# namada-net/masp

Measured on AMD Instinct MI355X. Metric: Spend proofs/sec, higher is better.
Workload: dtype u32; 1 GPU; BASELINE.json configs[3]: batch of 256 distinct Spend proofs per step on one MI355X (throughput mode); proofs_per_gpu=4352, distinct_witnesses_per_gpu=256, ntt_log2=17, batch_cap=256, slots=4, calls_in_flight=4, hw_queues=4, parallelism=proofs sharded over 1 GPU(s), no data-path collective, gather of the proofs

## Files before the change

include/masp_hip.h:

```cpp
#ifndef MASP_HIP_H
#define MASP_HIP_H
#include <stddef.h>
#include <stdint.h>

#ifdef __cplusplus
extern "C" {
#endif

#define MASP_HIP_OK 0
#define MASP_HIP_E_INVALID_ARG 1
#define MASP_HIP_E_PARAMS_FORMAT 2
#define MASP_HIP_E_PARAMS_SHAPE 3
#define MASP_HIP_E_NO_DEVICE 4
#define MASP_HIP_E_HIP 5
#define MASP_HIP_E_UNEXPECTED_IDENTITY 6
#define MASP_HIP_E_NOT_LOADED 7
#define MASP_HIP_E_SCALAR_RANGE 8
#define MASP_HIP_E_POINT_ENCODING 9
#define MASP_HIP_E_CAPACITY 10

#define MASP_HIP_MAX_CIRCUITS 8
#define MASP_HIP_SPEND 0
#define MASP_HIP_OUTPUT 1
#define MASP_HIP_CONVERT 2

typedef struct masp_hip_ctx masp_hip_ctx;

typedef struct {
    uint32_t n_inputs, n_aux, n_constraints;
    const uint32_t* a_rowptr; const uint32_t* a_col; const uint8_t* a_coef;
    const uint32_t* b_rowptr; const uint32_t* b_col; const uint8_t* b_coef;
    const uint32_t* c_rowptr; const uint32_t* c_col; const uint8_t* c_coef;
} masp_hip_r1cs;

typedef struct {
    uint32_t circuit;
    const uint8_t* inputs;
    const uint8_t* aux;
    const uint8_t* a;
    const uint8_t* b;
    const uint8_t* c;
    uint8_t r[32], s[32];
    uint32_t aux_form;
    uint32_t reserved;
} masp_hip_job;
#define MASP_HIP_AUX_CANONICAL 0
#define MASP_HIP_AUX_MONTGOMERY 1

int masp_hip_device_count(void);
int masp_hip_device_pci_bus_id(int device, char* out, size_t cap);

typedef struct {
    uint32_t struct_size;
    int32_t slots;
    int32_t batch_cap;
    int32_t ntt_sub_batch;
    int32_t window_bits_h;
    int32_t window_bits_la;
    int32_t window_bits_b;
    int32_t window_bits_b2_lone;
    int32_t witness_nontrivial_percent;
    int32_t bucket_tree_levels;
    int32_t bucket_tree_sub_batch;
    int32_t bucket_tree_levels_g2;
    int32_t bucket_tree_scratch_mb;
    int32_t bucket_tree_fallback_proofs;
    int32_t lone_proof_graph;
    int32_t hw_queues;
    int32_t window_bits_h_lone;
    int32_t digit_recoding;
    int32_t window_bits_b2;
} masp_hip_options;
void masp_hip_options_default(masp_hip_options* opt);
#define MASP_HIP_MAX_USEFUL_HW_QUEUES 20
int masp_hip_runtime_prepare(int hw_queues, int overwrite);

int masp_hip_ctx_create(int device, masp_hip_ctx** out);
int masp_hip_ctx_create_ex(const int* devices, int n_devices, const masp_hip_options* opt, masp_hip_ctx** out);
int masp_hip_ctx_get_options(const masp_hip_ctx* ctx, masp_hip_options* out);
int masp_hip_ctx_create_multi(const int* devices, int n_devices, masp_hip_ctx** out);
int masp_hip_ctx_set_boolean_block_bits(masp_hip_ctx* ctx, int32_t bits);
int masp_hip_ctx_get_boolean_block_bits(const masp_hip_ctx* ctx, int32_t* out);
int masp_hip_ctx_device_count(const masp_hip_ctx* ctx);
int masp_hip_ctx_device_proofs(const masp_hip_ctx* ctx, uint64_t* counts, int cap);
int masp_hip_ctx_device_status(const masp_hip_ctx* ctx, int32_t* status, int cap, uint64_t* requeued);
int masp_hip_ctx_inject_fault(masp_hip_ctx* ctx, int device, uint32_t nth);
int masp_hip_ctx_stream_concurrency(masp_hip_ctx* ctx, int mains_only, int* n_streams, int* concurrent);
int masp_hip_ctx_lone_graph_launches(const masp_hip_ctx* ctx, uint64_t* out);
void masp_hip_ctx_destroy(masp_hip_ctx* ctx);
const char* masp_hip_strerror(int code);
const char* masp_hip_last_error(const masp_hip_ctx* ctx);

int masp_hip_circuit_load(masp_hip_ctx* ctx, uint32_t slot, const uint8_t* params, size_t params_len, const masp_hip_r1cs* cs);
#define MASP_HIP_CIRCUIT_G1_ENDOMORPHISM 1u
int masp_hip_circuit_flags(const masp_hip_ctx* ctx, uint32_t slot, uint32_t* flags);

int masp_hip_prove(masp_hip_ctx* ctx, uint32_t slot, const uint8_t* inputs, const uint8_t* aux, const uint8_t* a,
                   const uint8_t* b, const uint8_t* c, const uint8_t r[32], const uint8_t s[32], uint8_t proof_out[192]);
int masp_hip_prove_batch(masp_hip_ctx* ctx, size_t n, const masp_hip_job* jobs, uint8_t* proofs_out);

int masp_hip_generate_parameters(masp_hip_ctx* ctx, const masp_hip_r1cs* cs, const uint8_t toxic[160], uint8_t* out, size_t cap,
                                 size_t* out_len);
size_t masp_hip_parameters_max_size(const masp_hip_r1cs* cs);

int masp_hip_msm_g1(masp_hip_ctx* ctx, const uint8_t* bases, const uint8_t* scalars, size_t n, uint8_t out[96]);
int masp_hip_msm_g2(masp_hip_ctx* ctx, const uint8_t* bases, const uint8_t* scalars, size_t n, uint8_t out[192]);
int masp_hip_msm_g1_multi(masp_hip_ctx* ctx, const uint8_t* bases, size_t n, const uint8_t* scalars, size_t np, int window_bits,
                          uint8_t* out);
int masp_hip_msm_g2_multi(masp_hip_ctx* ctx, const uint8_t* bases, size_t n, const uint8_t* scalars, size_t np, int window_bits,
                          uint8_t* out);
int masp_hip_msm_g1_multi_ex(masp_hip_ctx* ctx, const uint8_t* bases, size_t n, const uint8_t* scalars, size_t np, int window_bits,
                             int block_bits, size_t sub_lo, size_t sub_hi, uint8_t* out, uint32_t* bucket0_entries);
int masp_hip_msm_g2_multi_ex(masp_hip_ctx* ctx, const uint8_t* bases, size_t n, const uint8_t* scalars, size_t np, int window_bits,
                             int block_bits, size_t sub_lo, size_t sub_hi, uint8_t* out, uint32_t* bucket0_entries);
int masp_hip_quotient_h(masp_hip_ctx* ctx, const uint8_t* a, const uint8_t* b, const uint8_t* c, size_t nrows,
                        uint32_t logm, uint8_t* h_out);
int masp_hip_ntt(masp_hip_ctx* ctx, uint8_t* data, uint32_t logm, int inverse);

typedef struct masp_hip_vk masp_hip_vk;
int masp_hip_vk_prepare(masp_hip_ctx* ctx, const uint8_t* params, size_t params_len, masp_hip_vk** out);
void masp_hip_vk_free(masp_hip_vk* vk);
int masp_hip_verify_batch(masp_hip_ctx* ctx, masp_hip_vk* vk, size_t n, const uint8_t* proofs, const uint8_t* public_inputs,
                          uint32_t n_public, const uint8_t* z, int* all_valid);

int masp_hip_jubjub_msm(masp_hip_ctx* ctx, size_t n, const uint8_t* points, const uint8_t* scalars, uint8_t out32[32], int64_t* bad_index);
int masp_hip_redjubjub_verify_batch(masp_hip_ctx* ctx, size_t n, const uint8_t* vks, const uint8_t* sigs, const uint8_t* sighashes,
                                    const uint8_t* kinds, const uint8_t* z, int* all_valid);

int masp_hip_sapling_trial_decrypt(masp_hip_ctx* ctx, size_t n_ivk, const uint8_t* ivks, size_t n_out, const uint8_t* epks,
                                   const uint8_t* enc_ciphertexts, uint8_t* epk_status, size_t hit_capacity, uint32_t* hit_output,
                                   uint32_t* hit_ivk, uint8_t* hit_keys, size_t* n_hits);
int masp_hip_note_scan_configure(masp_hip_ctx* ctx, int signed_digits, int inversion);
int masp_hip_note_scan_last_timing(masp_hip_ctx* ctx, double ms[2]);

int masp_hip_sapling_compact_trial_decrypt(masp_hip_ctx* ctx, size_t n_ivk, const uint8_t* ivks, size_t n_out, const uint8_t* epks,
                                           const uint8_t* cmus, const uint8_t* enc_compact, int lead_byte, uint8_t* epk_status,
                                           size_t hit_capacity, uint32_t* hit_output, uint32_t* hit_ivk, uint8_t* hit_plaintexts,
                                           uint8_t* hit_pk_d, size_t* n_hits, size_t* n_candidates);
int masp_hip_note_scan_compact_last_timing(masp_hip_ctx* ctx, double ms[3]);

int masp_hip_sapling_output_recovery_scan(masp_hip_ctx* ctx, size_t n_ovk, const uint8_t* ovks, size_t n_out, const uint8_t* cvs,
                                          const uint8_t* epks, const uint8_t* cmus, const uint8_t* out_ciphertexts, size_t hit_capacity,
                                          uint32_t* hit_output, uint32_t* hit_ovk, uint8_t* hit_ocks, size_t* n_hits);
int masp_hip_out_recovery_last_timing(masp_hip_ctx* ctx, double ms[2]);

int masp_hip_merkle_tree_complete(masp_hip_ctx* ctx, unsigned height0, size_t n, const uint8_t* row, uint8_t* nodes_out, size_t nodes_capacity,
                                  size_t* n_nodes, uint8_t root32[32], size_t n_paths, const uint64_t* positions, uint8_t* paths_out,
                                  int64_t* bad_index);
int masp_hip_merkle_last_timing(masp_hip_ctx* ctx, double ms[3]);
int masp_hip_merkle_tree_append(masp_hip_ctx* ctx, uint64_t start, const uint8_t frontier[32 * 32], size_t n, const uint8_t* row,
                                uint8_t* nodes_out, size_t nodes_capacity, size_t* n_nodes, int64_t* bad_index);

int masp_hip_batch_upload(masp_hip_ctx* ctx, size_t n, const masp_hip_job* jobs);
int masp_hip_batch_prove_resident(masp_hip_ctx* ctx, int handle, uint8_t* proofs_out, float* elapsed_ms);
int masp_hip_batch_prove_resident_steps(masp_hip_ctx* ctx, int handle, size_t steps, const uint8_t* rs, uint8_t* proofs_out,
                                        float* elapsed_ms);
int masp_hip_batch_free(masp_hip_ctx* ctx, int handle);
int masp_hip_bench_msm(masp_hip_ctx* ctx, int handle, size_t job, int which, int iters, float* avg_ms, uint32_t* n_bases);

int masp_hip_profile_enable(masp_hip_ctx* ctx, int on);
int masp_hip_profile_read(masp_hip_ctx* ctx, double* total_ms, uint64_t* launches, uint64_t* alg_bytes);
int masp_hip_profile_read_split(masp_hip_ctx* ctx, double ms[8]);
int masp_hip_profile_read_lone(masp_hip_ctx* ctx, double ms[12]);
void* masp_hip_host_alloc(masp_hip_ctx* ctx, size_t bytes);
void masp_hip_host_free(masp_hip_ctx* ctx, void* ptr);
int masp_hip_sync(masp_hip_ctx* ctx);

#ifdef __cplusplus
}
#endif

#if defined(__cplusplus) && __cplusplus >= 201103L
#define MASP_HIP_STATIC_ASSERT(c, m) static_assert(c, m)
#elif defined(__STDC_VERSION__) && __STDC_VERSION__ >= 201112L
#define MASP_HIP_STATIC_ASSERT(c, m) _Static_assert(c, m)
#else
#define MASP_HIP_SA_CAT2(a, b) a##b
#define MASP_HIP_SA_CAT(a, b) MASP_HIP_SA_CAT2(a, b)
#define MASP_HIP_STATIC_ASSERT(c, m) typedef char MASP_HIP_SA_CAT(masp_hip_static_assert_, __LINE__)[(c) ? 1 : -1]
#endif
#if defined(__LP64__) || defined(_LP64)
MASP_HIP_STATIC_ASSERT(sizeof(masp_hip_job) == 120, "masp_hip_job: 4 + 4 pad + 5 pointers + r[32] + s[32] + aux_form + reserved");
MASP_HIP_STATIC_ASSERT(offsetof(masp_hip_job, inputs) == 8 && offsetof(masp_hip_job, c) == 40, "masp_hip_job pointers");
MASP_HIP_STATIC_ASSERT(offsetof(masp_hip_job, r) == 48 && offsetof(masp_hip_job, s) == 80, "masp_hip_job r | s");
MASP_HIP_STATIC_ASSERT(offsetof(masp_hip_job, aux_form) == 112 && offsetof(masp_hip_job, reserved) == 116, "masp_hip_job tail");
MASP_HIP_STATIC_ASSERT(sizeof(masp_hip_r1cs) == 88 && offsetof(masp_hip_r1cs, a_rowptr) == 16 && offsetof(masp_hip_r1cs, c_coef) == 80,
                       "masp_hip_r1cs: three counts + 4 pad + nine pointers");
MASP_HIP_STATIC_ASSERT(sizeof(masp_hip_options) == 76 && offsetof(masp_hip_options, window_bits_b2) == 72,
                       "masp_hip_options: struct_size + 18 int32 fields (appended-only: struct_size versions it)");
MASP_HIP_STATIC_ASSERT(offsetof(masp_hip_options, hw_queues) == 60 && offsetof(masp_hip_options, digit_recoding) == 68, "masp_hip_options tail");
#endif
#endif
```

masp_amd/csrc/device/ntt.hpp:

```cpp
#pragma once
#include <hip/hip_runtime.h>

#include "field.hpp"
#include "fr_io.hpp"
#include "ntt_geom.h"

namespace masp {


__device__ __forceinline__ uint32_t bitrev(uint32_t k, uint32_t logm) { return __brev(k) >> (32 - logm); }

__global__ void k_fr_powers(Fr* __restrict__ table, uint32_t n, Fr base, Fr scale, int plain) {
    uint32_t k = blockIdx.x * blockDim.x + threadIdx.x;
    if (k >= n) return;
    uint32_t e[1] = {k};
    Fr r = fe_mul(fe_pow(base, e, 1), scale);
    if (plain) r = fe_from_mont(r);
    fr_store(table + k, r);
}

#define NTT_P (blockIdx.y)

__global__ void k_ntt_load_bitrev(const Fr* __restrict__ x, size_t x_stride, uint32_t nrows, Fr* __restrict__ y, uint32_t logm) {
    uint32_t k = blockIdx.x * blockDim.x + threadIdx.x;
    if (k >= (1u << logm)) return;
    x += NTT_P * x_stride;
    y += (size_t)NTT_P << logm;
    Fr v = fe_zero<FrCfg>();
    if (k < nrows) v = fe_to_mont(fr_load(x + k));
    fr_store(y + bitrev(k, logm), v);
}
__global__ void k_ntt_copy_bitrev(const Fr* __restrict__ x, size_t x_stride, uint32_t nrows, Fr* __restrict__ y, uint32_t logm) {
    uint32_t k = blockIdx.x * blockDim.x + threadIdx.x;
    if (k >= (1u << logm)) return;
    x += NTT_P * x_stride;
    y += (size_t)NTT_P << logm;
    Fr v = fe_zero<FrCfg>();
    if (k < nrows) v = fr_load(x + k);
    fr_store(y + bitrev(k, logm), v);
}
__global__ void k_ntt_scale_bitrev(const Fr* __restrict__ x, const Fr* __restrict__ scale, Fr* __restrict__ y, uint32_t logm) {
    uint32_t k = blockIdx.x * blockDim.x + threadIdx.x;
    if (k >= (1u << logm)) return;
    x += (size_t)NTT_P << logm;
    y += (size_t)NTT_P << logm;
    fr_store(y + bitrev(k, logm), fe_mul(fr_load(x + k), fr_load(scale + k)));
}
__global__ void k_ntt_ab_bitrev(const Fr* __restrict__ a, const Fr* __restrict__ b, Fr* __restrict__ y, uint32_t logm) {
    uint32_t k = blockIdx.x * blockDim.x + threadIdx.x;
    if (k >= (1u << logm)) return;
    a += (size_t)NTT_P << logm;
    b += (size_t)NTT_P << logm;
    y += (size_t)NTT_P << logm;
    fr_store(y + bitrev(k, logm), fe_mul(fr_load(a + k), fr_load(b + k)));
}
__global__ void k_fr_scale_sub(const Fr* __restrict__ x, const Fr* __restrict__ scale, const Fr* __restrict__ c, Fr cscale, Fr* __restrict__ y,
                               uint32_t n, size_t y_stride) {
    uint32_t k = blockIdx.x * blockDim.x + threadIdx.x;
    if (k >= n) return;
    x += (size_t)NTT_P * n;
    c += (size_t)NTT_P * n;
    y += (size_t)NTT_P * y_stride;
    fr_store(y + k, fe_sub(fe_mul(fr_load(x + k), fr_load(scale + k)), fe_mul(fr_load(c + k), cscale)));
}
__global__ void k_fr_scale(const Fr* __restrict__ x, const Fr* __restrict__ scale, Fr* __restrict__ y, uint32_t n, size_t y_stride) {
    uint32_t k = blockIdx.x * blockDim.x + threadIdx.x;
    if (k >= n) return;
    x += (size_t)NTT_P * n;
    y += (size_t)NTT_P * y_stride;
    fr_store(y + k, fe_mul(fr_load(x + k), fr_load(scale + k)));
}
__global__ void k_fr_from_mont(const Fr* __restrict__ x, Fr* __restrict__ y, uint32_t n) {
    uint32_t k = blockIdx.x * blockDim.x + threadIdx.x;
    if (k >= n) return;
    fr_store(y + k, fe_from_mont(fr_load(x + k)));
}

__global__ void __launch_bounds__(256) k_ntt_pass(Fr* __restrict__ data, const Fr* __restrict__ tw, uint32_t logm, uint32_t s0,
                                                  uint32_t nst) {
    __shared__ uint4 tile[2 << NTT_LT];
    const uint32_t lt = nst + (NTT_LT - nst < logm - nst ? NTT_LT - nst : logm - nst);
    const uint32_t cols_log = lt - nst;
    const uint32_t cols = 1u << cols_log;
    const uint32_t tsize = 1u << lt;
    const uint32_t col0 = blockIdx.x << cols_log;
    const uint32_t lomask = (1u << s0) - 1u;
    data += (size_t)NTT_P << logm;
    for (uint32_t L = threadIdx.x; L < tsize; L += blockDim.x) {
        uint32_t h = L >> cols_log, col = col0 + (L & (cols - 1));
        uint32_t idx = ((col >> s0) << (s0 + nst)) | (h << s0) | (col & lomask);
        const uint4* q = reinterpret_cast<const uint4*>(data + idx);
        tile[L] = q[0];
        tile[tsize + L] = q[1];
    }
    __syncthreads();
    auto ld = [&](uint32_t L) {
        Fr r;
        uint4 a0 = tile[L], a1 = tile[tsize + L];
        r.v[0] = a0.x; r.v[1] = a0.y; r.v[2] = a0.z; r.v[3] = a0.w; r.v[4] = a1.x; r.v[5] = a1.y; r.v[6] = a1.z; r.v[7] = a1.w;
        return r;
    };
    auto st = [&](uint32_t L, const Fr& x) {
        tile[L] = make_uint4(x.v[0], x.v[1], x.v[2], x.v[3]);
        tile[tsize + L] = make_uint4(x.v[4], x.v[5], x.v[6], x.v[7]);
    };
    uint32_t q = 0;
    for (; q + 1 < nst; q += 2) {
        const uint32_t s = s0 + q;
        for (uint32_t gidx = threadIdx.x; gidx < (tsize >> 2); gidx += blockDim.x) {
            const uint32_t cl = gidx & (cols - 1), r = gidx >> cols_log;
            const uint32_t hj = r & ((1u << q) - 1u), hg = r >> q;
            const uint32_t h00 = (hg << (q + 2)) | hj;
            const uint32_t L0 = (h00 << cols_log) | cl, d = cols << q;
            const uint32_t lo = (col0 + cl) & lomask;
            const uint32_t j1 = (hj << s0) | lo;
            const uint32_t j2a = j1, j2b = ((hj | (1u << q)) << s0) | lo;
            Fr x0 = ld(L0), x1 = ld(L0 + d), x2 = ld(L0 + 2 * d), x3 = ld(L0 + 3 * d);
            if (s == 0) {
                const Fr y0 = fe_add(x0, x1), y1 = fe_sub(x0, x1), y2 = fe_add(x2, x3), y3 = fe_sub(x2, x3);
                st(L0, fe_add(y0, y2));
                st(L0 + 2 * d, fe_sub(y0, y2));
                const Fr t = fe_mul(y3, fr_load(tw + ((size_t)1 << (logm - 2))));
                st(L0 + d, fe_add(y1, t));
                st(L0 + 3 * d, fe_sub(y1, t));
                continue;
            }
            const Fr w1 = fr_load(tw + ((size_t)j1 << (logm - s - 1)));
            const Fr w2a = fr_load(tw + ((size_t)j2a << (logm - s - 2)));
            const Fr w2b = fr_load(tw + ((size_t)j2b << (logm - s - 2)));
            Fr t = fe_mul(x1, w1);
            Fr y0 = fe_add(x0, t), y1 = fe_sub(x0, t);
            t = fe_mul(x3, w1);
            Fr y2 = fe_add(x2, t), y3 = fe_sub(x2, t);
            t = fe_mul(y2, w2a);
            st(L0, fe_add(y0, t));
            st(L0 + 2 * d, fe_sub(y0, t));
            t = fe_mul(y3, w2b);
            st(L0 + d, fe_add(y1, t));
            st(L0 + 3 * d, fe_sub(y1, t));
        }
        __syncthreads();
    }
    for (; q < nst; ++q) {
        const uint32_t s = s0 + q;
        for (uint32_t b = threadIdx.x; b < (tsize >> 1); b += blockDim.x) {
            uint32_t cl = b & (cols - 1), hb = b >> cols_log;
            uint32_t hj = hb & ((1u << q) - 1u), hg = hb >> q;
            uint32_t L0 = (((hg << (q + 1)) | hj) << cols_log) | cl;
            uint32_t L1 = L0 + (cols << q);
            uint32_t col = col0 + cl;
            uint32_t jglob = (hj << s0) | (col & lomask);
            Fr w = fr_load(tw + ((size_t)jglob << (logm - s - 1)));
            Fr u = ld(L0), v = fe_mul(ld(L1), w);
            st(L0, fe_add(u, v));
            st(L1, fe_sub(u, v));
        }
        __syncthreads();
    }
    for (uint32_t L = threadIdx.x; L < tsize; L += blockDim.x) {
        uint32_t h = L >> cols_log, col = col0 + (L & (cols - 1));
        uint32_t idx = ((col >> s0) << (s0 + nst)) | (h << s0) | (col & lomask);
        uint4* q = reinterpret_cast<uint4*>(data + idx);
        q[0] = tile[L];
        q[1] = tile[tsize + L];
    }
}

}
```

masp_amd/csrc/device/r1cs.hpp:

```cpp
#pragma once
#include <hip/hip_runtime.h>

#include "../launch.h"
#include "fr_io.hpp"

namespace masp {

__global__ void k_fr_to_mont(const Fr* __restrict__ x, size_t x_stride, Fr* __restrict__ y, uint32_t n, int* __restrict__ range_err) {
    uint32_t k = blockIdx.x * blockDim.x + threadIdx.x;
    if (k >= n) return;
    x += blockIdx.y * x_stride;
    y += (size_t)blockIdx.y * n;
    Fr v = fr_load(x + k);
    if (fe_canonical_ge_mod(v)) atomicOr(range_err, 1);
    fr_store(y + k, fe_to_mont(v));
}
__global__ void k_fr_split_forms(Fr* __restrict__ x, size_t x_stride, Fr* __restrict__ y, uint32_t n, uint32_t mont_from, int* __restrict__ range_err) {
    uint32_t k = blockIdx.x * blockDim.x + threadIdx.x;
    if (k >= n) return;
    x += blockIdx.y * x_stride;
    y += (size_t)blockIdx.y * n;
    Fr v = fr_load(x + k);
    if (fe_canonical_ge_mod(v)) atomicOr(range_err, 1);
    if (k < mont_from) {
        fr_store(y + k, fe_to_mont(v));
    } else {
        fr_store(y + k, v);
        fr_store(x + k, fe_from_mont(v));
    }
}

__global__ void k_r1cs_eval(R1csMatrices M, const Fr* __restrict__ w, uint32_t n_vars, uint32_t n_constraints, uint32_t n_inputs) {
    const int which = blockIdx.z;
    const uint32_t v = blockIdx.x * blockDim.x + threadIdx.x, nl = M.n_long[which];
    const uint32_t* __restrict__ rowptr = M.rowptr[which];
    const uint32_t* __restrict__ order = M.order[which];
    const uint32_t* __restrict__ col = M.col[which];
    const Fr* __restrict__ coef = M.coef[which];
    Fr* __restrict__ out = M.out[which];
    w += (size_t)blockIdx.y * n_vars;
    out += (size_t)blockIdx.y * (n_constraints + n_inputs);
    if (v < nl * 64u) {
        const uint32_t row = order[v >> 6], lane = v & 63u;
        const uint32_t lo = rowptr[row], hi = rowptr[row + 1];
        Fr acc = fe_zero<FrCfg>();
        for (uint32_t t = lo + lane; t < hi; t += 64) acc = fe_add(acc, fe_mul(fr_load(coef + t), fr_load(w + col[t])));
        for (int d = 32; d >= 1; d >>= 1) {
            Fr other;
#pragma unroll
            for (int i = 0; i < 8; ++i) other.v[i] = (uint32_t)__shfl_down((int)acc.v[i], d, 64);
            acc = fe_add(acc, other);
        }
        if (lane == 0) fr_store(out + row, acc);
        return;
    }
    uint32_t row = v - nl * 64u + nl;
    if (row >= n_constraints + n_inputs) return;
    Fr acc = fe_zero<FrCfg>();
    if (row < n_constraints) {
        row = order[row];
        uint32_t lo = rowptr[row], hi = rowptr[row + 1];
        for (uint32_t t = lo; t < hi; ++t) acc = fe_add(acc, fe_mul(fr_load(coef + t), fr_load(w + col[t])));
    } else if (which == 0) {
        acc = fr_load(w + (row - n_constraints));
    }
    fr_store(out + row, acc);
}

__global__ void k_gather_scalars(const Fr* __restrict__ src, size_t src_stride, const uint32_t* __restrict__ idx, uint32_t n,
                                 Fr* __restrict__ dst) {
    uint32_t k = blockIdx.x * blockDim.x + threadIdx.x;
    if (k >= n) return;
    src += blockIdx.y * src_stride;
    dst += (size_t)blockIdx.y * n;
    fr_store(dst + k, fr_load(src + idx[k]));
}

}
```

masp_amd/csrc/device/setup.hpp:

```cpp
#pragma once
#include <hip/hip_runtime.h>

#include "curve.hpp"
#include "fr_io.hpp"
#include "io.hpp"

namespace masp {

__global__ void k_setup_lagrange(Fr* __restrict__ lag, uint32_t nrows, Fr omega, Fr tau, Fr z_over_m) {
    uint32_t k = blockIdx.x * blockDim.x + threadIdx.x;
    if (k >= nrows) return;
    uint32_t e[1] = {k};
    Fr wk = fe_pow(omega, e, 1);
    Fr den = fe_inv(fe_sub(tau, wk));
    fr_store(lag + k, fe_mul(fe_mul(z_over_m, wk), den));
}
__global__ void k_setup_qap(const uint32_t* __restrict__ colptr, const uint32_t* __restrict__ rowidx, const Fr* __restrict__ coef,
                            const Fr* __restrict__ lag, uint32_t nv, uint32_t n_inputs, uint32_t n_constraints, int is_a,
                            Fr* __restrict__ out) {
    uint32_t v = blockIdx.x * blockDim.x + threadIdx.x;
    if (v >= nv) return;
    Fr acc = fe_zero<FrCfg>();
    for (uint32_t t = colptr[v]; t < colptr[v + 1]; ++t) acc = fe_add(acc, fe_mul(fr_load(coef + t), fr_load(lag + rowidx[t])));
    if (is_a && v < n_inputs) acc = fe_add(acc, fr_load(lag + n_constraints + v));
    fr_store(out + v, acc);
}
__global__ void k_setup_lc(const Fr* __restrict__ at, const Fr* __restrict__ bt, const Fr* __restrict__ ct, uint32_t n, Fr alpha, Fr beta,
                           Fr scale, Fr* __restrict__ out) {
    uint32_t v = blockIdx.x * blockDim.x + threadIdx.x;
    if (v >= n) return;
    Fr x = fe_add(fe_add(fe_mul(beta, fr_load(at + v)), fe_mul(alpha, fr_load(bt + v))), fr_load(ct + v));
    fr_store(out + v, fe_mul(x, scale));
}
__global__ void k_setup_nonzero(const Fr* __restrict__ x, uint32_t n, uint8_t* __restrict__ flags) {
    uint32_t v = blockIdx.x * blockDim.x + threadIdx.x;
    if (v >= n) return;
    flags[v] = fe_is_zero(fr_load(x + v)) ? 0 : 1;
}

template <class O>
__global__ void k_setup_fixed_table(Affine<O> gen, Affine<O>* __restrict__ tab) {
    uint32_t w = blockIdx.x * blockDim.x + threadIdx.x;
    if (w >= 32) return;
    Xyzz<O> base = xyzz_from_affine(gen);
    for (uint32_t k = 0; k < 8 * w; ++k) base = xyzz_dbl(base);
    Affine<O> b = xyzz_to_affine(base);
    Xyzz<O> cur = xyzz_from_affine(b);
    for (uint32_t d = 1; d <= 255; ++d) {
        tab[w * 255 + d - 1] = xyzz_to_affine(cur);
        xyzz_madd_nc(cur, b, false);
    }
}
template <class O, int BYTES>
__global__ void __launch_bounds__(64) k_setup_fixed_mul(const Affine<O>* __restrict__ tab, const Fr* __restrict__ scalars, uint32_t n, int mont,
                                                        uint8_t* __restrict__ out) {
    uint32_t i = blockIdx.x * blockDim.x + threadIdx.x;
    if (i >= n) return;
    Fr k = fr_load(scalars + i);
    if (mont) k = fe_from_mont(k);
    Xyzz<O> acc = xyzz_inf<O>();
    for (int w = 0; w < 32; ++w) {
        uint32_t d = (k.v[w >> 2] >> (8 * (w & 3))) & 0xffu;
        if (d) xyzz_madd_nc(acc, tab[w * 255 + d - 1], false);
    }
    Affine<O> p = xyzz_to_affine(acc);
    if constexpr (BYTES == 96)
        g1_write_uncompressed(p, out + (size_t)i * 96);
    else
        g2_write_uncompressed(p, out + (size_t)i * 192);
}
__global__ void k_setup_gather(const Fr* __restrict__ src, const uint32_t* __restrict__ idx, uint32_t n, Fr* __restrict__ dst) {
    uint32_t k = blockIdx.x * blockDim.x + threadIdx.x;
    if (k >= n) return;
    fr_store(dst + k, fr_load(src + idx[k]));
}
__global__ void k_setup_h_scalars(Fr tau, Fr c, uint32_t n, Fr* __restrict__ out) {
    uint32_t i = blockIdx.x * blockDim.x + threadIdx.x;
    if (i >= n) return;
    uint32_t e[1] = {i};
    fr_store(out + i, fe_mul(fe_pow(tau, e, 1), c));
}

}
```

masp_amd/csrc/internal.h:

```cpp
#pragma once
#include <hip/hip_runtime.h>

#include <algorithm>
#include <array>
#include <condition_variable>
#include <cstring>
#include <deque>
#include <map>
#include <memory>
#include <mutex>
#include <shared_mutex>
#include <string>
#include <thread>
#include <vector>

#include "chunk_pipeline.h"
#include "device/io.hpp"
#include "device/ntt_geom.h"
#include "launch.h"
#include "msm_host.h"
#include <atomic>
#include "util.h"

#ifndef MASP_SUBSET_BITS
#define MASP_SUBSET_BITS 2
#endif
static_assert(MASP_SUBSET_BITS == 0 || MASP_SUBSET_BITS == 2 || MASP_SUBSET_BITS == 3, "subset blocks are 4 or 8 bases wide");


namespace masp {

template <class T>
struct DevBuf {
    T* p = nullptr;
    size_t cap = 0;
    ~DevBuf() { release(); }
    void release() {
        if (p) dev_free(p);
        p = nullptr;
        cap = 0;
    }
    int reserve(size_t n) {
        if (n <= cap) return MASP_HIP_OK;
        release();
        HIP_TRY(dev_malloc(&p, sizeof(T) * std::max<size_t>(n, 1)));
        cap = n;
        return MASP_HIP_OK;
    }
    int upload(const T* h, size_t n, hipStream_t s) {
        int rc = reserve(n);
        if (rc) return rc;
        if (n) HIP_TRY(hipMemcpyAsync(p, h, sizeof(T) * n, hipMemcpyHostToDevice, s));
        return MASP_HIP_OK;
    }
};

static inline Fr fr_from_u64_mont(uint64_t x) {
    Fr v = fe_zero<FrCfg>();
    v.v[0] = (uint32_t)x;
    v.v[1] = (uint32_t)(x >> 32);
    return fe_to_mont(v);
}
static inline Fr fr_const(const uint32_t* limbs) {
    Fr v;
    for (int i = 0; i < 8; ++i) v.v[i] = limbs[i];
    return v;
}

struct NttDomain {
    uint32_t logm = 0;
    size_t m = 0;
    DevBuf<Fr> tw_fwd, tw_inv, coset_scale, h_scale;
    Fr c_scale;
    int init(uint32_t logm_, hipStream_t s) {
        logm = logm_;
        m = (size_t)1 << logm;
        Fr omega = fr_const(FrCfg::ROOT_OF_UNITY);
        for (uint32_t i = logm; i < 32; ++i) omega = fe_sqr(omega);
        Fr omega_inv = fe_inv(omega);
        Fr minv = fe_inv(fr_from_u64_mont(m));
        Fr g = fr_const(FrCfg::GEN), ginv = fr_const(FrCfg::GEN_INV);
        uint32_t e[2] = {(uint32_t)m, (uint32_t)((uint64_t)m >> 32)};
        const Fr zinv = fe_inv(fe_sub(fe_pow(g, e, 2), fe_one<FrCfg>()));
        const Fr mzinv = fe_mul(minv, zinv);
        c_scale = fe_from_mont(mzinv);
        Fr one = fe_one<FrCfg>();
        size_t half = std::max<size_t>(m / 2, 1);
        int rc;
        if ((rc = tw_fwd.reserve(half)) || (rc = tw_inv.reserve(half)) || (rc = coset_scale.reserve(m)) || (rc = h_scale.reserve(m))) return rc;
        launch_fr_powers(s, tw_fwd.p, (uint32_t)half, omega, one, 0);
        launch_fr_powers(s, tw_inv.p, (uint32_t)half, omega_inv, one, 0);
        launch_fr_powers(s, coset_scale.p, (uint32_t)m, g, minv, 0);
        launch_fr_powers(s, h_scale.p, (uint32_t)m, ginv, mzinv, 1);
        HIP_TRY(hipStreamSynchronize(s));
        return MASP_HIP_OK;
    }
    void passes(hipStream_t s, Fr* data, const Fr* tw, uint32_t np = 1) const {
        for (uint32_t s0 = 0; s0 < logm;) {
            uint32_t nst = std::min<uint32_t>(NTT_LT, logm - s0);
            launch_ntt_pass(s, data, tw, logm, s0, nst, np);
            s0 += nst;
        }
    }
};

struct Circuit {
    uint32_t n_inputs = 0, n_aux = 0, n_constraints = 0, nrows = 0, logm = 0;
    size_t m = 0;
    DevBuf<uint32_t> rowptr[3], col[3];
    DevBuf<uint32_t> row_order[3];
    uint32_t n_long_rows[3] = {0, 0, 0};
    DevBuf<Fr> coef[3];
    DevBuf<uint32_t> a_var, b_var;
    uint32_t na = 0, nbq = 0;
    DevBuf<VkDevice> vk;
    DevBuf<G1Xyzz> fb1;
    DevBuf<G2Xyzz> fb2;
    BasesG1 h, l, a, b1;
    BasesG1 hl;
    BasesG2 b2;
    BasesG2 b2_lone;
    bool g1_endo = false;
    NttDomain* dom = nullptr;
};

struct Slot {
    hipStream_t stream = nullptr;
    hipEvent_t done = nullptr;
    MsmWorkspace<FpOps> ws1;
    MsmWorkspace<Fp2Ops> ws2;
    static constexpr int N_AUX = 4;
    hipStream_t aux[N_AUX] = {nullptr, nullptr, nullptr, nullptr};
    hipEvent_t ev_fork = nullptr, ev_sort_b = nullptr, ev_fixed = nullptr, ev_join[N_AUX] = {nullptr, nullptr, nullptr, nullptr};
    hipEvent_t ev_uploaded = nullptr;
    MsmWorkspace<FpOps> ws_l, ws_a, ws_b;
    DevBuf<Fr> w, inp, abc, wm, ev[3], x0, x1, h, hl, sa, sb;
    DevBuf<G1Xyzz> res1, asm1;
    DevBuf<G2Xyzz> res2, asm2;
    DevBuf<uint32_t> rs;
    DevBuf<uint8_t> proof;
    DevBuf<int> flags;
    MsmProfile prof;
    bool profiling = false;
    static constexpr int N_LONE_MARKS = 12;
    hipEvent_t ev_lone[N_LONE_MARKS] = {};
    bool lone_marked = false;
    void lone_mark(hipStream_t st, int id) {
        if (!profiling) return;
        if (!ev_lone[id] && hipEventCreate(&ev_lone[id]) != hipSuccess) return;
        (void)hipEventRecord(ev_lone[id], st);
        if (id == N_LONE_MARKS - 1) lone_marked = true;
    }
    uint32_t ntt_sub = 8;
    uint8_t* h_stage = nullptr;
    size_t h_stage_cap = 0;
    uint8_t* h_proof = nullptr;
    size_t h_proof_cap = 0;
    int* h_flags = nullptr;
    struct LoneGraph {
        const void *circuit, *w, *abc, *rs, *proof;
        size_t w_stride;
        uint32_t np;
        bool mont;
        int runs;
        bool dead;
        hipGraphExec_t exec;
    };
    std::vector<LoneGraph> graphs;
    uint64_t graph_epoch = 0;
    bool lone_graph = false;
    std::atomic<uint64_t> graph_launches{0};
    void drop_graphs() {
        for (auto& g : graphs)
            if (g.exec) hipGraphExecDestroy(g.exec);
        graphs.clear();
    }
    ~Slot() {
        drop_graphs();
        if (done) hipEventDestroy(done);
        for (hipEvent_t e : ev_join)
            if (e) hipEventDestroy(e);
        for (hipEvent_t e : ev_lone)
            if (e) hipEventDestroy(e);
        if (ev_fork) hipEventDestroy(ev_fork);
        if (ev_uploaded) hipEventDestroy(ev_uploaded);
        if (ev_sort_b) hipEventDestroy(ev_sort_b);
        if (ev_fixed) hipEventDestroy(ev_fixed);
        if (h_stage) hipHostFree(h_stage);
        if (h_proof) hipHostFree(h_proof);
        if (h_flags) hipHostFree(h_flags);
    }
    void configure(const masp_hip_options& o) {
        ntt_sub = (uint32_t)o.ntt_sub_batch;
        ws1.tree_levels = o.bucket_tree_levels;
        ws2.tree_levels = o.bucket_tree_levels_g2;
        ws1.tree_levels_shared = o.bucket_tree_levels_g2;
        ws1.tree_sub = ws2.tree_sub = (uint32_t)o.bucket_tree_sub_batch;
        ws2.tree.arena = &ws1.tree.own;
        ws1.tree.own.limit = (size_t)o.bucket_tree_scratch_mb << 20;
        lone_graph = o.lone_proof_graph > 0;
    }
    int init(const std::array<hipStream_t, 5>& streams) {
        stream = streams[0];
        for (int i = 0; i < N_AUX; ++i) aux[i] = streams[1 + i];
        HIP_TRY(hipEventCreateWithFlags(&done, hipEventDisableTiming));
        HIP_TRY(hipEventCreateWithFlags(&ev_fork, hipEventDisableTiming));
        HIP_TRY(hipEventCreateWithFlags(&ev_uploaded, hipEventDisableTiming));
        HIP_TRY(hipEventCreateWithFlags(&ev_sort_b, hipEventDisableTiming));
        HIP_TRY(hipEventCreateWithFlags(&ev_fixed, hipEventDisableTiming));
        for (hipEvent_t& e : ev_join) HIP_TRY(hipEventCreateWithFlags(&e, hipEventDisableTiming));
        HIP_TRY(hipHostMalloc(&h_flags, sizeof(int)));
        int rc;
        if ((rc = flags.reserve(1))) return rc;
        return reserve_batch(1);
    }
    int reserve_batch(size_t np) {
        int rc;
        if ((rc = res1.reserve(4 * np)) || (rc = res2.reserve(np)) || (rc = asm1.reserve(6 * np)) || (rc = asm2.reserve(np)) || (rc = rs.reserve(16 * np)) || (rc = proof.reserve(192 * np))) return rc;
        if (np > h_proof_cap) {
            if (h_proof) hipHostFree(h_proof);
            h_proof = nullptr;
            HIP_TRY(hipHostMalloc(&h_proof, 192 * np));
            h_proof_cap = np;
        }
        return MASP_HIP_OK;
    }
    int stage_reserve(size_t bytes) {
        if (bytes <= h_stage_cap) return MASP_HIP_OK;
        if (h_stage) hipHostFree(h_stage);
        h_stage = nullptr;
        HIP_TRY(hipHostMalloc(&h_stage, bytes));
        h_stage_cap = bytes;
        return MASP_HIP_OK;
    }
};

struct ResidentBatch {
    size_t n = 0;
    std::vector<uint32_t> circuit;
    std::vector<size_t> order;
    std::vector<size_t> w_off;
    DevBuf<Fr> w;
    DevBuf<uint32_t> rs;
};

struct StreamTable {
    hipStream_t main = nullptr;
    std::vector<std::array<hipStream_t, 5>> slot;
    hipStream_t vk[2] = {nullptr, nullptr};
    std::vector<hipStream_t> distinct() const {
        std::vector<hipStream_t> out;
        auto add = [&](hipStream_t s) {
            if (s && std::find(out.begin(), out.end(), s) == out.end()) out.push_back(s);
        };
        add(main);
        for (const auto& row : slot)
            for (hipStream_t s : row) add(s);
        for (hipStream_t s : vk) add(s);
        return out;
    }
    ~StreamTable() {
        for (hipStream_t s : distinct()) (void)hipStreamDestroy(s);
    }
};

}

using masp::Circuit;
using masp::DevBuf;
using masp::Fr;
using masp::G1Affine;
using masp::G1Xyzz;
using masp::G2Affine;
using masp::G2Xyzz;
using masp::NttDomain;
using masp::ResidentBatch;
using masp::Slot;

struct masp_hip_ctx {
    static constexpr size_t MAX_SLOTS = 64;
    int device = 0;
    std::vector<masp_hip_ctx*> children;
    masp_hip_options opt{};
    int boolean_block_bits = MASP_SUBSET_BITS;
    int n_slots = 4;
    size_t batch_cap = 256;
    std::shared_mutex mu;
    mutable std::mutex slot_mu;
    std::condition_variable slot_cv;
    std::vector<char> slot_busy;
    std::string err;
    masp::StreamTable streams;
    std::unique_ptr<Circuit> circ[MASP_HIP_MAX_CIRCUITS];
    std::map<uint32_t, std::unique_ptr<NttDomain>> domains;
    std::vector<std::unique_ptr<Slot>> slots;
    std::vector<std::unique_ptr<ResidentBatch>> batches;
    bool profiling = false;
    std::atomic<uint64_t> proofs_done{0};
    std::unique_ptr<std::atomic<int>[]> dev_status;
    std::atomic<uint64_t> requeued{0};
    std::atomic<uint32_t> fault_countdown{0};
    std::atomic<unsigned> vk_next{0};
    int main_streams_concurrent = 0;
    std::mutex upload_mu;
    hipEvent_t upload_tail = nullptr;
    std::atomic<uint64_t> block_tree_fallbacks{0};
    std::atomic<uint32_t> block_tree_sub{0xffffffffu};
    DevBuf<Fr> tmp_scalars;
    DevBuf<uint8_t> tmp_out;
    DevBuf<G1Xyzz> tmp_g1;
    DevBuf<G2Xyzz> tmp_g2;
    DevBuf<G1Affine> fb_g1;
    DevBuf<G2Affine> fb_g2;
    std::mutex jj_mu;
    DevBuf<uint8_t> jj_points, jj_scalars, jj_partial;
    DevBuf<int> jj_status;
    DevBuf<uint32_t> jj_out;
    struct NoteScanSet {
        DevBuf<uint8_t> epk, raw, ct, pts, status, hit_keys;
        DevBuf<uint32_t> count, hit_idx;
    };
    std::mutex ns_mu;
    NoteScanSet ns[2];
    DevBuf<uint32_t> ns_digits;
    std::atomic<int> ns_signed_digits{1}, ns_inversion{0};
    double ns_last_ms[2] = {0, 0};
    struct NoteScanCompactSet {
        DevBuf<uint8_t> cmu, enc, cand, state, hit_idx, hit_data;
        DevBuf<uint32_t> count, list;
    };
    NoteScanCompactSet nsc[2];
    DevBuf<uint8_t> nsc_ivks;
    DevBuf<uint8_t> nsc_table;
    double nsc_last_ms[3] = {0, 0, 0};
    struct OutRecoverySet {
        DevBuf<uint8_t> cv, cmu, epk, cout, cols, hit_ocks;
        DevBuf<uint32_t> count, hit_idx;
    };
    OutRecoverySet orc[2];
    DevBuf<uint32_t> orc_ovks;
    double orc_last_ms[2] = {0, 0};
    DevBuf<uint32_t> mt_nodes, mt_bad, mt_paths, mt_empties;
    DevBuf<uint64_t> mt_pos;
    double mt_last_ms[3] = {0, 0, 0};
};

namespace masp {

static inline int fail(masp_hip_ctx* ctx, int rc) {
    if (rc == MASP_HIP_E_HIP) {
        std::lock_guard<std::mutex> g(ctx->slot_mu);
        ctx->err = last_hip_error();
    }
    return rc;
}

#define FIRST_DEVICE(ctx) ((ctx) && !(ctx)->children.empty() ? (ctx)->children[0] : (ctx))

static inline int get_domain(masp_hip_ctx* ctx, uint32_t logm, NttDomain** out) {
    auto it = ctx->domains.find(logm);
    if (it == ctx->domains.end()) {
        std::unique_ptr<NttDomain> d(new NttDomain);
        int rc = d->init(logm, ctx->streams.main);
        if (rc) return rc;
        it = ctx->domains.emplace(logm, std::move(d)).first;
    }
    *out = it->second.get();
    return MASP_HIP_OK;
}

constexpr size_t NS_MAX_IVKS = 4096;
constexpr size_t NS_MAX_OUTPUTS = (size_t)1 << 26;
int ns_recode_ivks(std::vector<uint32_t>& digits, size_t n_ivk, const uint8_t* ivks, bool signed_digits);
void launch_ns_decode(hipStream_t s, const uint8_t* epks, uint32_t n, uint8_t* status, uint8_t* pts);

static inline uint32_t log2_ceil(uint32_t n) {
    uint32_t k = 0;
    while ((1ull << k) < n) ++k;
    return k;
}

}
```

masp_amd/csrc/k_ntt.hip:

```cpp
#include <algorithm>
#include "device/ntt.hpp"
#include "device/r1cs.hpp"
#include "launch.h"
#include "util.h"

namespace masp {

void launch_fr_powers(hipStream_t s, Fr* table, uint32_t n, const Fr& base, const Fr& scale, int plain) {
    MASP_LAUNCH(k_fr_powers, dim3((n + 255) / 256), dim3(256), 0, s, table, n, base, scale, plain);
}
void launch_ntt_pass(hipStream_t s, Fr* data, const Fr* tw, uint32_t logm, uint32_t s0, uint32_t nst, uint32_t np) {
    const uint32_t lt = (uint32_t)NTT_LT < logm ? (uint32_t)NTT_LT : logm;
    MASP_LAUNCH(k_ntt_pass, dim3(1u << (logm - lt), np), dim3(256), 0, s, data, tw, logm, s0, nst);
}
void launch_ntt_load_bitrev(hipStream_t s, const Fr* x, size_t x_stride, uint32_t nrows, Fr* y, uint32_t logm, uint32_t np) {
    MASP_LAUNCH(k_ntt_load_bitrev, dim3(((1u << logm) + 255) / 256, np), dim3(256), 0, s, x, x_stride, nrows, y, logm);
}
void launch_ntt_copy_bitrev(hipStream_t s, const Fr* x, size_t x_stride, uint32_t nrows, Fr* y, uint32_t logm, uint32_t np) {
    MASP_LAUNCH(k_ntt_copy_bitrev, dim3(((1u << logm) + 255) / 256, np), dim3(256), 0, s, x, x_stride, nrows, y, logm);
}
void launch_ntt_scale_bitrev(hipStream_t s, const Fr* x, const Fr* scale, Fr* y, uint32_t logm, uint32_t np) {
    MASP_LAUNCH(k_ntt_scale_bitrev, dim3(((1u << logm) + 255) / 256, np), dim3(256), 0, s, x, scale, y, logm);
}
void launch_ntt_ab_bitrev(hipStream_t s, const Fr* a, const Fr* b, Fr* y, uint32_t logm, uint32_t np) {
    MASP_LAUNCH(k_ntt_ab_bitrev, dim3(((1u << logm) + 255) / 256, np), dim3(256), 0, s, a, b, y, logm);
}
void launch_fr_scale_sub(hipStream_t s, const Fr* x, const Fr* scale, const Fr* c, const Fr& cscale, Fr* y, uint32_t n, uint32_t np, size_t y_stride) {
    MASP_LAUNCH(k_fr_scale_sub, dim3((n + 255) / 256, np), dim3(256), 0, s, x, scale, c, cscale, y, n, y_stride ? y_stride : (size_t)n);
}
void launch_fr_scale(hipStream_t s, const Fr* x, const Fr* scale, Fr* y, uint32_t n, uint32_t np, size_t y_stride) {
    MASP_LAUNCH(k_fr_scale, dim3((n + 255) / 256, np), dim3(256), 0, s, x, scale, y, n, y_stride ? y_stride : (size_t)n);
}
void launch_fr_from_mont(hipStream_t s, const Fr* x, Fr* y, uint32_t n) {
    MASP_LAUNCH(k_fr_from_mont, dim3((n + 255) / 256), dim3(256), 0, s, x, y, n);
}
void launch_fr_to_mont(hipStream_t s, const Fr* x, size_t x_stride, Fr* y, uint32_t n, uint32_t np, int* range_err) {
    MASP_LAUNCH(k_fr_to_mont, dim3((n + 255) / 256, np), dim3(256), 0, s, x, x_stride, y, n, range_err);
}
void launch_fr_split_forms(hipStream_t s, Fr* x, size_t x_stride, Fr* y, uint32_t n, uint32_t mont_from, uint32_t np, int* range_err) {
    MASP_LAUNCH(k_fr_split_forms, dim3((n + 255) / 256, np), dim3(256), 0, s, x, x_stride, y, n, mont_from, range_err);
}
void launch_r1cs_eval(hipStream_t s, const R1csMatrices& M, const Fr* w, uint32_t n_vars, uint32_t n_constraints, uint32_t n_inputs, uint32_t np) {
    const uint32_t nl = std::max(M.n_long[0], std::max(M.n_long[1], M.n_long[2])), lanes = n_constraints + n_inputs + nl * 63u;
    MASP_LAUNCH(k_r1cs_eval, dim3((lanes + 127) / 128, np, 3), dim3(128), 0, s, M, w, n_vars, n_constraints, n_inputs);
}
void launch_gather_scalars(hipStream_t s, const Fr* src, size_t src_stride, const uint32_t* idx, uint32_t n, Fr* dst, uint32_t np) {
    MASP_LAUNCH(k_gather_scalars, dim3((n + 255) / 256, np), dim3(256), 0, s, src, src_stride, idx, n, dst);
}

}
```

masp_amd/csrc/k_setup.hip:

```cpp
#include "device/setup.hpp"
#include "internal.h"

using namespace masp;

extern "C" {

size_t masp_hip_parameters_max_size(const masp_hip_r1cs* cs) {
    if (!cs) return 0;
    size_t nv = (size_t)cs->n_inputs + cs->n_aux;
    size_t m = (size_t)1 << log2_ceil(cs->n_constraints + cs->n_inputs);
    return 864 + 6 * 4 + 96 * ((size_t)cs->n_inputs + (m - 1) + cs->n_aux + 2 * nv) + 192 * nv;
}

int masp_hip_generate_parameters(masp_hip_ctx* ctx, const masp_hip_r1cs* cs, const uint8_t toxic[160], uint8_t* out, size_t cap,
                                 size_t* out_len) {
    if (!ctx || !cs || !toxic || !out_len || cs->n_inputs == 0) return MASP_HIP_E_INVALID_ARG;
    const ApiLaunchScope api_scope;
    ctx = FIRST_DEVICE(ctx);
    std::unique_lock<std::shared_mutex> lock(ctx->mu);
    hipSetDevice(ctx->device);
    hipStream_t s = ctx->streams.main;
    Fr tw[5];
    for (int i = 0; i < 5; ++i) {
        Fr v = fe_load_le<FrCfg>(toxic + 32 * i);
        if (fe_canonical_ge_mod(v)) return MASP_HIP_E_SCALAR_RANGE;
        tw[i] = fe_to_mont(v);
    }
    const Fr tau = tw[0], alpha = tw[1], beta = tw[2], gamma = tw[3], delta = tw[4];
    if (fe_is_zero(gamma) || fe_is_zero(delta)) return MASP_HIP_E_UNEXPECTED_IDENTITY;
    const uint32_t n_in = cs->n_inputs, n_aux = cs->n_aux, nc = cs->n_constraints, nv = n_in + n_aux;
    const uint32_t nrows = nc + n_in, logm = log2_ceil(nrows);
    const size_t m = (size_t)1 << logm;
    Fr omega = fr_const(FrCfg::ROOT_OF_UNITY);
    for (uint32_t i = logm; i < 32; ++i) omega = fe_sqr(omega);
    uint32_t em[2] = {(uint32_t)m, (uint32_t)((uint64_t)m >> 32)};
    Fr z = fe_sub(fe_pow(tau, em, 2), fe_one<FrCfg>());
    Fr z_over_m = fe_mul(z, fe_inv(fr_from_u64_mont(m)));
    Fr dinv = fe_inv(delta), ginv = fe_inv(gamma);
    int rc;
    if (!ctx->fb_g1.p) {
        if ((rc = ctx->fb_g1.reserve(32 * 255)) || (rc = ctx->fb_g2.reserve(32 * 255))) return fail(ctx, rc);
        G1Affine g1;
        G2Affine g2;
        for (int i = 0; i < 12; ++i) {
            g1.x.v[i] = FpCfg::G1_X[i];
            g1.y.v[i] = FpCfg::G1_Y[i];
            g2.x.c0.v[i] = FpCfg::G2_X0[i];
            g2.x.c1.v[i] = FpCfg::G2_X1[i];
            g2.y.c0.v[i] = FpCfg::G2_Y0[i];
            g2.y.c1.v[i] = FpCfg::G2_Y1[i];
        }
        MASP_LAUNCH((k_setup_fixed_table<FpOps>), dim3(1), dim3(64), 0, s, g1, ctx->fb_g1.p);
        MASP_LAUNCH((k_setup_fixed_table<Fp2Ops>), dim3(1), dim3(64), 0, s, g2, ctx->fb_g2.p);
    }
    DevBuf<Fr> lag, qt[3];
    if ((rc = lag.reserve(nrows))) return fail(ctx, rc);
    MASP_LAUNCH(k_setup_lagrange, dim3((nrows + 127) / 128), dim3(128), 0, s, lag.p, nrows, omega, tau, z_over_m);
    const uint32_t* rp[3] = {cs->a_rowptr, cs->b_rowptr, cs->c_rowptr};
    const uint32_t* cl[3] = {cs->a_col, cs->b_col, cs->c_col};
    const uint8_t* cf[3] = {cs->a_coef, cs->b_coef, cs->c_coef};
    DevBuf<int> d_flag;
    if ((rc = d_flag.reserve(1))) return fail(ctx, rc);
    hipMemsetAsync(d_flag.p, 0, sizeof(int), s);
    for (int mi = 0; mi < 3; ++mi) {
        const uint32_t nnz = rp[mi][nc];
        std::vector<uint32_t> colptr(nv + 1, 0), rowidx(nnz);
        std::vector<Fr> coefs(nnz);
        for (uint32_t t = 0; t < nnz; ++t) {
            if (cl[mi][t] >= nv) return MASP_HIP_E_INVALID_ARG;
            ++colptr[cl[mi][t] + 1];
        }
        for (uint32_t v = 0; v < nv; ++v) colptr[v + 1] += colptr[v];
        std::vector<uint32_t> fill(colptr.begin(), colptr.end() - 1);
        for (uint32_t row = 0; row < nc; ++row)
            for (uint32_t t = rp[mi][row]; t < rp[mi][row + 1]; ++t) {
                uint32_t pos = fill[cl[mi][t]]++;
                rowidx[pos] = row;
                memcpy(&coefs[pos], cf[mi] + 32 * (size_t)t, 32);
            }
        DevBuf<uint32_t> d_colptr, d_rowidx;
        DevBuf<Fr> d_raw, d_coef;
        if ((rc = d_colptr.upload(colptr.data(), nv + 1, s)) || (rc = d_rowidx.upload(rowidx.data(), nnz, s)) ||
            (rc = d_raw.upload(coefs.data(), nnz, s)) || (rc = d_coef.reserve(nnz)) || (rc = qt[mi].reserve(nv)))
            return fail(ctx, rc);
        if (nnz) launch_fr_to_mont(s, d_raw.p, (size_t)0, d_coef.p, nnz, 1, d_flag.p);
        MASP_LAUNCH(k_setup_qap, dim3((nv + 127) / 128), dim3(128), 0, s, d_colptr.p, d_rowidx.p, d_coef.p, lag.p, nv, n_in, nc,
                           mi == 0 ? 1 : 0, qt[mi].p);
        if (hipStreamSynchronize(s) != hipSuccess) {
            last_hip_error() = std::string("qap evaluation failed: ") + hipGetErrorString(hipGetLastError());
            return fail(ctx, MASP_HIP_E_HIP);
        }
    }
    DevBuf<uint8_t> d_nz;
    if ((rc = d_nz.reserve(2 * (size_t)nv))) return fail(ctx, rc);
    MASP_LAUNCH(k_setup_nonzero, dim3((nv + 255) / 256), dim3(256), 0, s, qt[0].p, nv, d_nz.p);
    MASP_LAUNCH(k_setup_nonzero, dim3((nv + 255) / 256), dim3(256), 0, s, qt[1].p, nv, d_nz.p + nv);
    std::vector<uint8_t> nz(2 * (size_t)nv);
    int hflag = 0;
    if (hipMemcpyAsync(nz.data(), d_nz.p, nz.size(), hipMemcpyDeviceToHost, s) != hipSuccess ||
        hipMemcpyAsync(&hflag, d_flag.p, sizeof(int), hipMemcpyDeviceToHost, s) != hipSuccess || hipStreamSynchronize(s) != hipSuccess)
        return fail(ctx, MASP_HIP_E_HIP);
    if (hflag) return MASP_HIP_E_SCALAR_RANGE;
    std::vector<uint32_t> a_list, b_list;
    for (uint32_t v = 0; v < nv; ++v) {
        if (nz[v]) a_list.push_back(v);
        if (nz[nv + v]) b_list.push_back(v);
    }
    const size_t n_h = m - 1, n_a = a_list.size(), n_b = b_list.size();
    const size_t o_ic = 3, o_h = o_ic + n_in, o_l = o_h + n_h, o_a = o_l + n_aux, o_b = o_a + n_a, n_g1 = o_b + n_b;
    const size_t n_g2 = 3 + n_b;
    const size_t total = 864 + 6 * 4 + 96 * (n_g1 - 3) + 192 * n_b;
    *out_len = total;
    if (!out || cap < total) return MASP_HIP_E_INVALID_ARG;
    DevBuf<Fr> k1, k2, lc;
    DevBuf<uint32_t> d_alist, d_blist;
    if ((rc = k1.reserve(n_g1)) || (rc = k2.reserve(n_g2)) || (rc = lc.reserve(nv)) || (rc = d_alist.upload(a_list.data(), n_a, s)) ||
        (rc = d_blist.upload(b_list.data(), n_b, s)))
        return fail(ctx, rc);
    Fr head1[3] = {alpha, beta, delta}, head2[3] = {beta, gamma, delta};
    if (hipMemcpyAsync(k1.p, head1, sizeof(head1), hipMemcpyHostToDevice, s) != hipSuccess ||
        hipMemcpyAsync(k2.p, head2, sizeof(head2), hipMemcpyHostToDevice, s) != hipSuccess)
        return fail(ctx, MASP_HIP_E_HIP);
    MASP_LAUNCH(k_setup_lc, dim3((n_in + 255) / 256), dim3(256), 0, s, qt[0].p, qt[1].p, qt[2].p, n_in, alpha, beta, ginv, k1.p + o_ic);
    if (n_aux)
        MASP_LAUNCH(k_setup_lc, dim3((n_aux + 255) / 256), dim3(256), 0, s, qt[0].p + n_in, qt[1].p + n_in, qt[2].p + n_in, n_aux, alpha,
                           beta, dinv, k1.p + o_l);
    MASP_LAUNCH(k_setup_h_scalars, dim3((n_h + 255) / 256), dim3(256), 0, s, tau, fe_mul(z, dinv), (uint32_t)n_h, k1.p + o_h);
    if (n_a) MASP_LAUNCH(k_setup_gather, dim3((n_a + 255) / 256), dim3(256), 0, s, qt[0].p, d_alist.p, (uint32_t)n_a, k1.p + o_a);
    if (n_b) {
        MASP_LAUNCH(k_setup_gather, dim3((n_b + 255) / 256), dim3(256), 0, s, qt[1].p, d_blist.p, (uint32_t)n_b, k1.p + o_b);
        MASP_LAUNCH(k_setup_gather, dim3((n_b + 255) / 256), dim3(256), 0, s, qt[1].p, d_blist.p, (uint32_t)n_b, k2.p + 3);
    }
    DevBuf<uint8_t> p1, p2;
    if ((rc = p1.reserve(96 * n_g1)) || (rc = p2.reserve(192 * n_g2))) return fail(ctx, rc);
    MASP_LAUNCH((k_setup_fixed_mul<FpOps, 96>), dim3((n_g1 + 63) / 64), dim3(64), 0, s, ctx->fb_g1.p, k1.p, (uint32_t)n_g1, 1, p1.p);
    MASP_LAUNCH((k_setup_fixed_mul<Fp2Ops, 192>), dim3((n_g2 + 63) / 64), dim3(64), 0, s, ctx->fb_g2.p, k2.p, (uint32_t)n_g2, 1, p2.p);
    std::vector<uint8_t> h1(96 * n_g1), h2(192 * n_g2);
    if (hipMemcpyAsync(h1.data(), p1.p, h1.size(), hipMemcpyDeviceToHost, s) != hipSuccess ||
        hipMemcpyAsync(h2.data(), p2.p, h2.size(), hipMemcpyDeviceToHost, s) != hipSuccess || hipStreamSynchronize(s) != hipSuccess) {
        last_hip_error() = std::string("parameter generation failed: ") + hipGetErrorString(hipGetLastError());
        return fail(ctx, MASP_HIP_E_HIP);
    }
    uint8_t* w = out;
    auto put = [&](const uint8_t* src, size_t n) {
        memcpy(w, src, n);
        w += n;
    };
    auto put_len = [&](size_t n) {
        uint8_t b[4] = {(uint8_t)(n >> 24), (uint8_t)(n >> 16), (uint8_t)(n >> 8), (uint8_t)n};
        put(b, 4);
    };
    put(&h1[0], 96);
    put(&h1[96], 96);
    put(&h2[0], 192);
    put(&h2[192], 192);
    put(&h1[192], 96);
    put(&h2[384], 192);
    put_len(n_in);
    put(&h1[96 * o_ic], 96 * (size_t)n_in);
    put_len(n_h);
    put(&h1[96 * o_h], 96 * n_h);
    put_len(n_aux);
    put(&h1[96 * o_l], 96 * (size_t)n_aux);
    put_len(n_a);
    put(&h1[96 * o_a], 96 * n_a);
    put_len(n_b);
    put(&h1[96 * o_b], 96 * n_b);
    put_len(n_b);
    put(&h2[192 * 3], 192 * n_b);
    if (launch_status() != MASP_HIP_OK) return fail(ctx, MASP_HIP_E_HIP);
    return (size_t)(w - out) == total ? MASP_HIP_OK : MASP_HIP_E_INVALID_ARG;
}

}
```

masp_amd/csrc/launch.h:

```cpp
#pragma once
#include <hip/hip_runtime.h>

#include "device/curve.hpp"

namespace masp {

void launch_fr_powers(hipStream_t s, Fr* table, uint32_t n, const Fr& base, const Fr& scale, int plain);
void launch_ntt_pass(hipStream_t s, Fr* data, const Fr* tw, uint32_t logm, uint32_t s0, uint32_t nst, uint32_t np);
void launch_ntt_load_bitrev(hipStream_t s, const Fr* x, size_t x_stride, uint32_t nrows, Fr* y, uint32_t logm, uint32_t np);
void launch_ntt_copy_bitrev(hipStream_t s, const Fr* x, size_t x_stride, uint32_t nrows, Fr* y, uint32_t logm, uint32_t np);
void launch_ntt_scale_bitrev(hipStream_t s, const Fr* x, const Fr* scale, Fr* y, uint32_t logm, uint32_t np);
void launch_ntt_ab_bitrev(hipStream_t s, const Fr* a, const Fr* b, Fr* y, uint32_t logm, uint32_t np);
void launch_fr_scale_sub(hipStream_t s, const Fr* x, const Fr* scale, const Fr* c, const Fr& cscale, Fr* y, uint32_t n, uint32_t np, size_t y_stride = 0);
void launch_fr_scale(hipStream_t s, const Fr* x, const Fr* scale, Fr* y, uint32_t n, uint32_t np, size_t y_stride = 0);
void launch_fr_from_mont(hipStream_t s, const Fr* x, Fr* y, uint32_t n);
void launch_fr_to_mont(hipStream_t s, const Fr* x, size_t x_stride, Fr* y, uint32_t n, uint32_t np, int* range_err);
void launch_fr_split_forms(hipStream_t s, Fr* x, size_t x_stride, Fr* y, uint32_t n, uint32_t mont_from, uint32_t np, int* range_err);
struct R1csMatrices {
    const uint32_t* rowptr[3];
    const uint32_t* order[3];
    const uint32_t* col[3];
    const Fr* coef[3];
    Fr* out[3];
    uint32_t n_long[3];
};
static constexpr uint32_t R1CS_LONG_ROW = 64;
void launch_r1cs_eval(hipStream_t s, const R1csMatrices& M, const Fr* w, uint32_t n_vars, uint32_t n_constraints, uint32_t n_inputs, uint32_t np);
void launch_gather_scalars(hipStream_t s, const Fr* src, size_t src_stride, const uint32_t* idx, uint32_t n, Fr* dst, uint32_t np);

void launch_groth16_fixed_g1(hipStream_t s, const G1Xyzz* fb1, const uint32_t* rs, size_t rs_stride, G1Xyzz* part, uint32_t np);
void launch_groth16_fixed_g2(hipStream_t s, const G2Xyzz* fb2, const uint32_t* rs, size_t rs_stride, G2Xyzz* part2, uint32_t np);
void launch_groth16_var_mul(hipStream_t s, int which, const G1Xyzz* msm_g1, const uint32_t* rs, size_t rs_stride, G1Xyzz* part, uint32_t np, bool endo);
void launch_g1_subgroup_flag(hipStream_t s, const void* pts, size_t stride_bytes, uint32_t n, int* flag);
void launch_groth16_finish_b(hipStream_t s, const VkDevice* vk, const G2Xyzz* part2, const G2Xyzz* msm_g2, uint8_t* proof, uint32_t np);
void launch_groth16_finish_ac(hipStream_t s, const VkDevice* vk, const G1Xyzz* part, const G1Xyzz* msm_g1, uint8_t* proof, uint32_t np);
void launch_groth16_finish_ac_early(hipStream_t s, const VkDevice* vk, G1Xyzz* part, const G1Xyzz* msm_g1, uint8_t* proof, uint32_t np);
void launch_groth16_finish_c_late(hipStream_t s, const G1Xyzz* part, const G1Xyzz* msm_g1, uint8_t* proof, uint32_t np);
void launch_g1_export(hipStream_t s, const G1Xyzz* p, uint8_t* out);
void launch_g2_export(hipStream_t s, const G2Xyzz* p, uint8_t* out);
void launch_g1_import_one(hipStream_t s, const uint8_t* raw, G1Affine* out, int* status);
void launch_g2_import_one(hipStream_t s, const uint8_t* raw, G2Affine* out, int* status);
void launch_fixed_table_g1(hipStream_t s, const G1Affine* pts, G1Xyzz* tabs, uint32_t npts);
void launch_fixed_table_g2(hipStream_t s, const G2Affine* pts, G2Xyzz* tabs, uint32_t npts);

}
```

masp_amd/csrc/prover.hip:

```cpp
#include <hip/hip_runtime.h>

#include <chrono>
#include <cstring>
#include <map>
#include <memory>
#include <algorithm>
#include <condition_variable>
#include <deque>
#include <mutex>
#include <shared_mutex>
#include <string>
#include <thread>
#include <vector>

#include "internal.h"

using namespace masp;

#ifndef MASP_UPLOAD_CHAIN
#define MASP_UPLOAD_CHAIN 1
#endif

namespace {

static masp_hip_options resolve_options(const masp_hip_options* in) {
    masp_hip_options o;
    memset(&o, 0, sizeof o);
    if (in) memcpy(&o, in, std::min<size_t>(in->struct_size ? in->struct_size : sizeof o, sizeof o));
    o.struct_size = sizeof o;
    o.slots = o.slots > 0 ? std::min<int>(o.slots, (int)masp_hip_ctx::MAX_SLOTS) : 4;
    o.batch_cap = o.batch_cap > 0 ? std::min<int>(o.batch_cap, 256) : 256;
    o.ntt_sub_batch = o.ntt_sub_batch > 0 ? o.ntt_sub_batch : o.ntt_sub_batch < 0 ? 0 : 8;
    o.window_bits_b2_lone = o.window_bits_b2_lone > 0 ? o.window_bits_b2_lone : o.window_bits_b2_lone < 0 ? 0 : 8;
    o.witness_nontrivial_percent = o.witness_nontrivial_percent > 0 ? std::min<int>(o.witness_nontrivial_percent, 100) : 30;
    o.bucket_tree_levels = o.bucket_tree_levels > 0 ? std::min<int>(o.bucket_tree_levels, 12) : o.bucket_tree_levels < 0 ? -1 : 0;
    o.bucket_tree_sub_batch = o.bucket_tree_sub_batch > 0 ? std::min<int>(o.bucket_tree_sub_batch, 256) : 86;
    o.bucket_tree_levels_g2 = o.bucket_tree_levels_g2 > 0 ? std::min<int>(o.bucket_tree_levels_g2, 12) : o.bucket_tree_levels_g2 < 0 ? -1 : o.bucket_tree_levels;
    o.bucket_tree_scratch_mb = std::max(o.bucket_tree_scratch_mb, 0);
    o.bucket_tree_fallback_proofs = 0;
    o.hw_queues = 0;
    o.window_bits_h_lone = o.window_bits_h_lone > 0 ? std::min<int>(o.window_bits_h_lone, 16) : 0;
    o.lone_proof_graph = o.lone_proof_graph > 0 ? 1 : 0;
    o.digit_recoding = 0;
    o.window_bits_b2 = o.window_bits_b2 > 0 ? std::max(2, std::min<int>(o.window_bits_b2, 16)) : o.window_bits_b2 < 0 ? -1 : 0;
    return o;
}
static std::vector<std::pair<size_t, size_t>> even_groups(size_t n, size_t cap) {
    std::vector<std::pair<size_t, size_t>> out;
    if (!n) return out;
    const size_t g = (n + cap - 1) / cap, base = n / g, extra = n % g;
    size_t lo = 0;
    for (size_t i = 0; i < g; ++i) {
        size_t cnt = base + (i < extra ? 1 : 0);
        out.push_back({lo, cnt});
        lo += cnt;
    }
    return out;
}

static int add_slot(masp_hip_ctx* ctx, char busy) {
    std::unique_ptr<Slot> s(new Slot);
    int rc = s->init(ctx->streams.slot[ctx->slots.size()]);
    if (rc) return rc;
    s->profiling = ctx->profiling;
    s->configure(ctx->opt);
    ctx->slots.push_back(std::move(s));
    ctx->slot_busy.push_back(busy);
    return MASP_HIP_OK;
}
static int ensure_slots(masp_hip_ctx* ctx, size_t want) {
    std::lock_guard<std::mutex> g(ctx->slot_mu);
    want = std::min(want, ctx->streams.slot.size());
    while (ctx->slots.size() < want)
        if (int rc = add_slot(ctx, 0)) return rc;
    for (auto& sl : ctx->slots) sl->profiling = ctx->profiling;
    return MASP_HIP_OK;
}
static int slot_try_acquire(masp_hip_ctx* ctx, size_t* si) {
    std::lock_guard<std::mutex> g(ctx->slot_mu);
    for (size_t i = 0; i < ctx->slots.size(); ++i)
        if (!ctx->slot_busy[i]) {
            ctx->slot_busy[i] = 1;
            *si = i;
            return MASP_HIP_OK;
        }
    if (ctx->slots.size() >= (size_t)ctx->n_slots) return -1;
    if (int rc = add_slot(ctx, 1)) return rc;
    *si = ctx->slots.size() - 1;
    return MASP_HIP_OK;
}
static size_t slot_acquire_blocking(masp_hip_ctx* ctx) {
    std::unique_lock<std::mutex> g(ctx->slot_mu);
    size_t found = 0;
    ctx->slot_cv.wait(g, [&] {
        for (size_t i = 0; i < ctx->slots.size(); ++i)
            if (!ctx->slot_busy[i]) {
                found = i;
                return true;
            }
        return false;
    });
    ctx->slot_busy[found] = 1;
    return found;
}
static void slot_release(masp_hip_ctx* ctx, size_t si) {
    bool idle = true;
    {
        std::lock_guard<std::mutex> g(ctx->slot_mu);
        ctx->slot_busy[si] = 0;
        for (char b : ctx->slot_busy) idle = idle && !b;
    }
    ctx->slot_cv.notify_one();
    if (idle) dev_free_drain();
}
static int enqueue_quotient(Slot& sl, const NttDomain& D, const Fr* const in[3], size_t in_stride, uint32_t nrows, bool mont_in, uint32_t np,
                            Fr* h_out = nullptr, size_t h_stride = 0) {
    hipStream_t s = sl.stream;
    const uint32_t m = (uint32_t)D.m, logm = D.logm;
    const uint32_t sub_max = sl.ntt_sub;
    const uint32_t sub = sub_max ? std::min(sub_max, np) : np;
    int rc;
    if ((rc = sl.x0.reserve((size_t)3 * m * sub)) || (rc = sl.x1.reserve((size_t)2 * m * sub))) return rc;
    if (!h_out) {
        if ((rc = sl.h.reserve((size_t)m * np))) return rc;
        h_out = sl.h.p;
        h_stride = m;
    }
    Fr *x0 = sl.x0.p, *x1 = sl.x1.p;
    for (uint32_t p0 = 0; p0 < np; p0 += sub) {
        const uint32_t q = std::min(sub, np - p0);
        const size_t part = (size_t)q * m;
        for (int i = 0; i < 3; ++i) {
            const Fr* src = in[i] + (size_t)p0 * in_stride;
            if (mont_in)
                launch_ntt_copy_bitrev(s, src, in_stride, nrows, x0 + i * part, logm, q);
            else
                launch_ntt_load_bitrev(s, src, in_stride, nrows, x0 + i * part, logm, q);
        }
        D.passes(s, x0, D.tw_inv.p, 3 * q);
        launch_ntt_scale_bitrev(s, x0, D.coset_scale.p, x1, logm, 2 * q);
        D.passes(s, x1, D.tw_fwd.p, 2 * q);
        launch_ntt_ab_bitrev(s, x1, x1 + part, x0, logm, q);
        D.passes(s, x0, D.tw_inv.p, q);
        launch_fr_scale_sub(s, x0, D.h_scale.p, x0 + 2 * part, D.c_scale, h_out + (size_t)p0 * h_stride, m, q, h_stride);
    }
    return MASP_HIP_OK;
}

static int enqueue_proofs(Slot& sl, Circuit& C, uint32_t np, const Fr* d_w, size_t w_stride, const Fr* const d_abc[3], const uint32_t* d_rs,
                          uint8_t* d_proof, bool aux_montgomery = false) {
    hipStream_t s = sl.stream;
    const uint32_t nv = C.n_inputs + C.n_aux;
    int rc;
    if ((rc = sl.reserve_batch(np))) return rc;
    if ((rc = sl.wm.reserve((size_t)nv * np))) return rc;
    const bool lone = np < 8;
    if (aux_montgomery) launch_fr_split_forms(s, const_cast<Fr*>(d_w), w_stride, sl.wm.p, nv, C.n_inputs, np, sl.flags.p);
    if (lone) {
        sl.lone_mark(s, 0);
        HIP_TRY(hipEventRecord(sl.ev_fork, s));
        for (int i = 0; i < Slot::N_AUX; ++i) HIP_TRY(hipStreamWaitEvent(sl.aux[i], sl.ev_fork, 0));
    }
    if (!aux_montgomery) launch_fr_to_mont(s, d_w, w_stride, sl.wm.p, nv, np, sl.flags.p);
    const Fr* in[3];
    bool mont_in;
    if (d_abc[0]) {
        in[0] = d_abc[0];
        in[1] = d_abc[1];
        in[2] = d_abc[2];
        mont_in = false;
    } else {
        R1csMatrices M;
        for (int i = 0; i < 3; ++i) {
            if ((rc = sl.ev[i].reserve((size_t)C.nrows * np))) return rc;
            M.rowptr[i] = C.rowptr[i].p;
            M.order[i] = C.row_order[i].p;
            M.n_long[i] = C.n_long_rows[i];
            M.col[i] = C.col[i].p;
            M.coef[i] = C.coef[i].p;
            M.out[i] = sl.ev[i].p;
            in[i] = sl.ev[i].p;
        }
        launch_r1cs_eval(s, M, sl.wm.p, nv, C.n_constraints, C.n_inputs, np);
        mont_in = true;
    }
    if ((rc = sl.sa.reserve((size_t)C.na * np)) || (rc = sl.sb.reserve((size_t)C.nbq * np))) return rc;
    MsmProfile* prof = sl.profiling ? &sl.prof : nullptr;
    const size_t m8 = C.m * 8;
    const bool share_b = C.nbq && msm_same_sort(C.b1, C.b2);
    if (lone) {
        launch_groth16_fixed_g1(sl.aux[0], C.fb1.p, d_rs, 16, sl.asm1.p, np);
        launch_groth16_fixed_g2(sl.aux[0], C.fb2.p, d_rs, 16, sl.asm2.p, np);
        HIP_TRY(hipEventRecord(sl.ev_fixed, sl.aux[0]));
        const bool own_b2 = C.b2_lone.n != 0;
        auto chain_a = [&]() -> int {
            int r;
            if (C.na) launch_gather_scalars(sl.aux[1], d_w, w_stride, C.a_var.p, C.na, sl.sa.p, np);
            if ((r = msm_enqueue(sl.aux[1], C.a, sl.ws_a, (const uint32_t*)sl.sa.p, (size_t)C.na * 8, sl.res1.p + 2, 4, np))) return r;
            sl.lone_mark(sl.aux[1], 1);
            launch_groth16_var_mul(sl.aux[1], 0, sl.res1.p, d_rs, 16, sl.asm1.p, np, C.g1_endo);
            sl.lone_mark(sl.aux[1], 2);
            return MASP_HIP_OK;
        };
        auto chain_b = [&]() -> int {
            int r;
            if (C.nbq) launch_gather_scalars(sl.aux[2], d_w, w_stride, C.b_var.p, C.nbq, sl.sb.p, np);
            HIP_TRY(hipEventRecord(sl.ev_sort_b, sl.aux[2]));
            if (share_b) {
                if ((r = msm_sort_enqueue(sl.aux[2], C.b1.n, C.b1.g, sl.ws_b.sort, (const uint32_t*)sl.sb.p, (size_t)C.nbq * 8, np, 0, C.b1.subset()))) return r;
                if (!own_b2) HIP_TRY(hipEventRecord(sl.ev_sort_b, sl.aux[2]));
                if ((r = msm_reduce_enqueue(sl.aux[2], C.b1, sl.ws_b.sort, sl.ws_b, sl.res1.p + 3, 4))) return r;
            } else if ((r = msm_enqueue(sl.aux[2], C.b1, sl.ws_b, (const uint32_t*)sl.sb.p, (size_t)C.nbq * 8, sl.res1.p + 3, 4, np))) {
                return r;
            }
            sl.lone_mark(sl.aux[2], 3);
            launch_groth16_var_mul(sl.aux[2], 1, sl.res1.p, d_rs, 16, sl.asm1.p, np, C.g1_endo);
            sl.lone_mark(sl.aux[2], 4);
            HIP_TRY(hipStreamWaitEvent(sl.aux[3], sl.ev_sort_b, 0));
            if (own_b2) {
                if ((r = msm_enqueue(sl.aux[3], C.b2_lone, sl.ws2, (const uint32_t*)sl.sb.p, (size_t)C.nbq * 8, sl.res2.p, 1, np))) return r;
            } else if (share_b) {
                if ((r = msm_reduce_enqueue(sl.aux[3], C.b2, sl.ws_b.sort, sl.ws2, sl.res2.p, 1))) return r;
            } else if ((r = msm_enqueue(sl.aux[3], C.b2, sl.ws2, (const uint32_t*)sl.sb.p, (size_t)C.nbq * 8, sl.res2.p, 1, np))) {
                return r;
            }
            sl.lone_mark(sl.aux[3], 5);
            HIP_TRY(hipStreamWaitEvent(sl.aux[3], sl.ev_fixed, 0));
            launch_groth16_finish_b(sl.aux[3], C.vk.p, sl.asm2.p, sl.res2.p, d_proof, np);
            sl.lone_mark(sl.aux[3], 6);
            return MASP_HIP_OK;
        };
        auto chain_l = [&]() -> int {
            return msm_enqueue(sl.aux[0], C.l, sl.ws_l, (const uint32_t*)(d_w + C.n_inputs), w_stride * 8, sl.res1.p + 1, 4, np);
        };
        if ((rc = chain_a()) || (rc = chain_b())) return rc;
        if ((rc = enqueue_quotient(sl, *C.dom, in, C.nrows, C.nrows, mont_in, np))) return rc;
        sl.lone_mark(s, 7);
        if ((rc = msm_enqueue(s, C.h, sl.ws1, (const uint32_t*)sl.h.p, m8, sl.res1.p + 0, 4, np, prof))) return rc;
        sl.lone_mark(s, 8);
        if ((rc = chain_l())) return rc;
        sl.lone_mark(sl.aux[0], 9);
        for (int i = 1; i < Slot::N_AUX - 1; ++i) {
            HIP_TRY(hipEventRecord(sl.ev_join[i], sl.aux[i]));
            HIP_TRY(hipStreamWaitEvent(sl.aux[0], sl.ev_join[i], 0));
        }
        launch_groth16_finish_ac_early(sl.aux[0], C.vk.p, sl.asm1.p, sl.res1.p, d_proof, np);
        HIP_TRY(hipEventRecord(sl.ev_join[0], sl.aux[0]));
        HIP_TRY(hipStreamWaitEvent(s, sl.ev_join[0], 0));
    } else {
        const size_t hl_stride = C.hl.n;
        if ((rc = sl.hl.reserve(hl_stride * np + 1))) return rc;
        if ((rc = enqueue_quotient(sl, *C.dom, in, C.nrows, C.nrows, mont_in, np, sl.hl.p, hl_stride))) return rc;
        HIP_TRY(hipMemcpy2DAsync(sl.hl.p + (C.m - 1), hl_stride * sizeof(Fr), d_w + C.n_inputs, w_stride * sizeof(Fr), (size_t)C.n_aux * sizeof(Fr), np,
                                 hipMemcpyDeviceToDevice, s));
        if (C.na) launch_gather_scalars(s, d_w, w_stride, C.a_var.p, C.na, sl.sa.p, np);
        if (C.nbq) launch_gather_scalars(s, d_w, w_stride, C.b_var.p, C.nbq, sl.sb.p, np);
        if ((rc = msm_enqueue(s, C.hl, sl.ws1, (const uint32_t*)sl.hl.p, hl_stride * 8, sl.res1.p + 0, 4, np, prof))) return rc;
        HIP_TRY(hipMemset2DAsync(sl.res1.p + 1, 4 * sizeof(G1Xyzz), 0, sizeof(G1Xyzz), np, s));
        const BasesG1 &Aq = C.a, &B1q = C.b1;
        const BasesG2& B2q = C.b2;
        const bool share_bq = share_b;
        if ((rc = msm_enqueue(s, Aq, sl.ws1, (const uint32_t*)sl.sa.p, (size_t)C.na * 8, sl.res1.p + 2, 4, np, prof))) return rc;
        if ((rc = msm_enqueue(s, B1q, sl.ws1, (const uint32_t*)sl.sb.p, (size_t)C.nbq * 8, sl.res1.p + 3, 4, np, prof))) return rc;
        if (share_bq) {
            if ((rc = msm_reduce_enqueue(s, B2q, sl.ws1.sort, sl.ws2, sl.res2.p, 1))) return rc;
        } else if ((rc = msm_enqueue(s, B2q, sl.ws2, (const uint32_t*)sl.sb.p, (size_t)C.nbq * 8, sl.res2.p, 1, np))) {
            return rc;
        }
    }
    if (!lone) {
        launch_groth16_fixed_g1(s, C.fb1.p, d_rs, 16, sl.asm1.p, np);
        launch_groth16_fixed_g2(s, C.fb2.p, d_rs, 16, sl.asm2.p, np);
                launch_groth16_var_mul(s, 2, sl.res1.p, d_rs, 16, sl.asm1.p, np, C.g1_endo);
        launch_groth16_finish_b(s, C.vk.p, sl.asm2.p, sl.res2.p, d_proof, np);
    }
    if (lone)
        launch_groth16_finish_c_late(s, sl.asm1.p, sl.res1.p, d_proof, np);
    else
        launch_groth16_finish_ac(s, C.vk.p, sl.asm1.p, sl.res1.p, d_proof, np);
    if (lone) {
        sl.lone_mark(s, 10);
        HIP_TRY(hipEventRecord(sl.ev_join[Slot::N_AUX - 1], sl.aux[Slot::N_AUX - 1]));
        HIP_TRY(hipStreamWaitEvent(s, sl.ev_join[Slot::N_AUX - 1], 0));
        sl.lone_mark(s, 11);
    }
    return MASP_HIP_OK;
}

static int enqueue_proofs_graphed(Slot& sl, Circuit& C, uint32_t np, const Fr* d_w, size_t w_stride, const Fr* const d_abc[3], const uint32_t* d_rs,
                                  uint8_t* d_proof, bool aux_montgomery) {
    if (np >= 8 || !sl.lone_graph || sl.profiling) return enqueue_proofs(sl, C, np, d_w, w_stride, d_abc, d_rs, d_proof, aux_montgomery);
    const uint64_t epoch = device_alloc_epoch().load(std::memory_order_relaxed);
    if (epoch != sl.graph_epoch) {
        sl.drop_graphs();
        sl.graph_epoch = epoch;
    }
    Slot::LoneGraph* e = nullptr;
    for (auto& g : sl.graphs)
        if (g.circuit == &C && g.np == np && g.w == d_w && g.w_stride == w_stride && g.abc == d_abc[0] && g.rs == d_rs && g.proof == d_proof &&
            g.mont == aux_montgomery)
            e = &g;
    if (!e) {
        if (sl.graphs.size() >= 16) sl.drop_graphs();
        sl.graphs.push_back(Slot::LoneGraph{&C, d_w, d_abc[0], d_rs, d_proof, w_stride, np, aux_montgomery, 0, false, nullptr});
        e = &sl.graphs.back();
    }
    if (e->exec) {
        HIP_TRY(hipGraphLaunch(e->exec, sl.stream));
        ++sl.graph_launches;
        return MASP_HIP_OK;
    }
    if (e->dead || e->runs == 0) {
        ++e->runs;
        return enqueue_proofs(sl, C, np, d_w, w_stride, d_abc, d_rs, d_proof, aux_montgomery);
    }
    bool ok = hipStreamBeginCapture(sl.stream, hipStreamCaptureModeThreadLocal) == hipSuccess;
    if (ok) {
        const int rc = enqueue_proofs(sl, C, np, d_w, w_stride, d_abc, d_rs, d_proof, aux_montgomery);
        hipGraph_t g = nullptr;
        const hipError_t ce = hipStreamEndCapture(sl.stream, &g);
        ok = rc == MASP_HIP_OK && ce == hipSuccess && g != nullptr && device_alloc_epoch().load(std::memory_order_relaxed) == epoch;
        if (ok) ok = hipGraphInstantiate(&e->exec, g, nullptr, nullptr, 0) == hipSuccess && e->exec != nullptr;
        if (g) hipGraphDestroy(g);
    }
    if (!ok) {
        (void)hipGetLastError();
        launch_error().clear();
        e->exec = nullptr;
        e->dead = true;
        sl.graph_epoch = device_alloc_epoch().load(std::memory_order_relaxed);
        return enqueue_proofs(sl, C, np, d_w, w_stride, d_abc, d_rs, d_proof, aux_montgomery);
    }
    HIP_TRY(hipGraphLaunch(e->exec, sl.stream));
    ++sl.graph_launches;
    return MASP_HIP_OK;
}

static bool rs_in_range(const uint8_t* x) {
    Fr v = fe_load_le<FrCfg>(x);
    return !fe_canonical_ge_mod(v);
}

struct ParamsLayout {
    const uint8_t *alpha_g1, *beta_g1, *beta_g2, *gamma_g2, *delta_g1, *delta_g2;
    const uint8_t *ic, *h, *l, *a, *b_g1, *b_g2;
    uint32_t n_ic, n_h, n_l, n_a, n_b1, n_b2;
};
static bool read_u32be(const uint8_t*& p, const uint8_t* end, uint32_t& v) {
    if (end - p < 4) return false;
    v = ((uint32_t)p[0] << 24) | ((uint32_t)p[1] << 16) | ((uint32_t)p[2] << 8) | p[3];
    p += 4;
    return true;
}
static bool parse_params(const uint8_t* buf, size_t len, ParamsLayout& L) {
    const uint8_t *p = buf, *end = buf + len;
    if (len < 864) return false;
    L.alpha_g1 = p; p += 96;
    L.beta_g1 = p;  p += 96;
    L.beta_g2 = p;  p += 192;
    L.gamma_g2 = p; p += 192;
    L.delta_g1 = p; p += 96;
    L.delta_g2 = p; p += 192;
    struct { const uint8_t** ptr; uint32_t* n; size_t sz; } secs[6] = {
        {&L.ic, &L.n_ic, 96}, {&L.h, &L.n_h, 96}, {&L.l, &L.n_l, 96}, {&L.a, &L.n_a, 96}, {&L.b_g1, &L.n_b1, 96}, {&L.b_g2, &L.n_b2, 192}};
    for (auto& sec : secs) {
        if (!read_u32be(p, end, *sec.n)) return false;
        if ((size_t)(end - p) < (size_t)*sec.n * sec.sz) return false;
        *sec.ptr = p;
        p += (size_t)*sec.n * sec.sz;
    }
    return true;
}

}

extern "C" {

const char* masp_hip_strerror(int code) {
    switch (code) {
        case MASP_HIP_OK: return "ok";
        case MASP_HIP_E_INVALID_ARG: return "invalid argument";
        case MASP_HIP_E_PARAMS_FORMAT: return "Parameters bytes are malformed";
        case MASP_HIP_E_PARAMS_SHAPE: return "Parameters do not match the circuit shape";
        case MASP_HIP_E_NO_DEVICE: return "no usable HIP device (there is no CPU fallback)";
        case MASP_HIP_E_HIP: return "HIP runtime error";
        case MASP_HIP_E_UNEXPECTED_IDENTITY: return "delta is the identity (UnexpectedIdentity)";
        case MASP_HIP_E_NOT_LOADED: return "circuit slot is empty";
        case MASP_HIP_E_SCALAR_RANGE: return "scalar is not a canonical field element";
        case MASP_HIP_E_POINT_ENCODING: return "a Jubjub point encoding does not decode";
        case MASP_HIP_E_CAPACITY: return "an output buffer is too small";
        default: return "unknown error";
    }
}

const char* masp_hip_last_error(const masp_hip_ctx* ctx) {
    static thread_local std::string copy;
    if (!ctx) return "";
    if (!ctx->children.empty()) {
        for (const masp_hip_ctx* ch : ctx->children) {
            const char* e = masp_hip_last_error(ch);
            if (e[0]) return e;
        }
        return "";
    }
    std::lock_guard<std::mutex> g(ctx->slot_mu);
    copy = ctx->err;
    return copy.c_str();
}

int masp_hip_device_count(void) {
    int count = 0;
    return hipGetDeviceCount(&count) == hipSuccess && count > 0 ? count : 0;
}

int masp_hip_device_pci_bus_id(int device, char* out, size_t cap) {
    if (!out || cap < 13) return MASP_HIP_E_INVALID_ARG;
    int count = 0;
    if (hipGetDeviceCount(&count) != hipSuccess || device < 0 || device >= count) return MASP_HIP_E_NO_DEVICE;
    return hipDeviceGetPCIBusId(out, (int)std::min<size_t>(cap, 64), device) == hipSuccess ? MASP_HIP_OK : MASP_HIP_E_HIP;
}

int masp_hip_runtime_prepare(int hw_queues, int overwrite) {
    char v[16];
    snprintf(v, sizeof v, "%d", hw_queues > 0 ? std::min(hw_queues, (int)MASP_HIP_MAX_USEFUL_HW_QUEUES) : 16);
    setenv("GPU_MAX_HW_QUEUES", v, overwrite ? 1 : 0);
    const char* e = getenv("GPU_MAX_HW_QUEUES");
    return e ? atoi(e) : 0;
}
__attribute__((constructor)) static void masp_hip_on_load() { setenv("GPU_MAX_HW_QUEUES", "16", 0); }

void masp_hip_options_default(masp_hip_options* opt) {
    if (!opt) return;
    memset(opt, 0, sizeof *opt);
    opt->struct_size = sizeof *opt;
}

static __global__ void k_hwq_spin(unsigned long long* out, int idx, long long ticks) {
    const long long t0 = wall_clock64();
    for (int it = 0; it < (1 << 22) && wall_clock64() - t0 < ticks; ++it) {
    }
    out[2 * idx] = (unsigned long long)t0;
    out[2 * idx + 1] = (unsigned long long)wall_clock64();
}
static long long wall_clock_per_ms() {
    int dev = 0, khz = 0;
    if (hipGetDevice(&dev) != hipSuccess || hipDeviceGetAttribute(&khz, hipDeviceAttributeWallClockRate, dev) != hipSuccess) return 0;
    return khz;
}
static int measure_streams(const std::vector<hipStream_t>& ss, int* concurrent, std::vector<unsigned long long>* intervals = nullptr) {
    const int n = (int)ss.size();
    const long long ms = wall_clock_per_ms();
    unsigned long long* d = nullptr;
    HIP_TRY(dev_malloc(&d, 16 * n));
    (void)hipGetLastError();
    bool ok = ms > 0;
    for (int r = 0; r < 2 && ok; ++r) {
        for (int i = 0; i < n; ++i) hipLaunchKernelGGL(k_hwq_spin, dim3(1), dim3(64), 0, ss[i], d, i, r ? 2 * ms : ms / 100);
        for (int i = 0; i < n; ++i) ok = hipStreamSynchronize(ss[i]) == hipSuccess && ok;
    }
    std::vector<unsigned long long> h(2 * n);
    ok = ok && hipGetLastError() == hipSuccess && hipMemcpyAsync(h.data(), d, 16 * n, hipMemcpyDeviceToHost, ss[0]) == hipSuccess &&
         hipStreamSynchronize(ss[0]) == hipSuccess;
    (void)dev_free(d);
    if (!ok) {
        last_hip_error() = "stream concurrency probe failed";
        return MASP_HIP_E_HIP;
    }
    int best = 0;
    for (int i = 0; i < n; ++i) {
        int c = 0;
        for (int j = 0; j < n; ++j) c += h[2 * j] <= h[2 * i] && h[2 * i] < h[2 * j + 1];
        best = std::max(best, c);
    }
    *concurrent = best;
    if (intervals) *intervals = std::move(h);
    return MASP_HIP_OK;
}
static int measure_hw_queues(int device, int streams) {
    static std::mutex mu;
    static std::map<int, int> known;
    std::lock_guard<std::mutex> lock(mu);
    auto it = known.find(device);
    if (it != known.end()) return it->second;
    const int n = std::max(1, std::min(streams, (int)MASP_HIP_MAX_USEFUL_HW_QUEUES + 1));
    std::vector<hipStream_t> ss;
    for (int i = 0; i < n; ++i) {
        hipStream_t s = nullptr;
        if (hipStreamCreateWithFlags(&s, hipStreamNonBlocking) != hipSuccess) break;
        ss.push_back(s);
    }
    int best = 0;
    if ((int)ss.size() == n) (void)measure_streams(ss, &best);
    for (hipStream_t s : ss) (void)hipStreamDestroy(s);
    (void)hipGetLastError();
    if (best > 0) known[device] = best;
    return best;
}

static std::vector<hipStream_t*> main_streams_of(StreamTable& t) {
    std::vector<hipStream_t*> at{&t.main};
    for (auto& row : t.slot) at.push_back(&row[0]);
    for (hipStream_t& v : t.vk) at.push_back(&v);
    return at;
}
static int measure_own_streams(masp_hip_ctx* ctx, bool mains_only, int* n_streams, int* concurrent) {
    std::vector<hipStream_t> ss;
    if (mains_only)
        for (hipStream_t* p : main_streams_of(ctx->streams)) ss.push_back(*p);
    else
        ss = ctx->streams.distinct();
    const int rc = measure_streams(ss, concurrent);
    if (rc == MASP_HIP_OK) *n_streams = (int)ss.size();
    return rc;
}

static int separate_main_streams(masp_hip_ctx* ctx) {
    const unsigned long long ms = (unsigned long long)wall_clock_per_ms();
    for (int attempt = 0; attempt < 8; ++attempt) {
        const std::vector<hipStream_t*> at = main_streams_of(ctx->streams);
        std::vector<hipStream_t> ss;
        for (hipStream_t* p : at) ss.push_back(*p);
        const int n = (int)ss.size();
        int conc = 0;
        std::vector<unsigned long long> h;
        if (int rc = measure_streams(ss, &conc, &h)) return rc;
        ctx->main_streams_concurrent = conc;
        if (conc >= n) return MASP_HIP_OK;
        unsigned long long t0 = ~0ull;
        for (int i = 0; i < n; ++i) t0 = std::min(t0, h[2 * i]);
        bool replaced = false;
        for (int i = 0; i < n; ++i) {
            if (h[2 * i] - t0 < ms) continue;
            int partner = -1;
            unsigned long long bestd = ~0ull;
            for (int j = 0; j < n; ++j) {
                if (j == i) continue;
                const unsigned long long d = h[2 * j + 1] > h[2 * i] ? h[2 * j + 1] - h[2 * i] : h[2 * i] - h[2 * j + 1];
                if (d < bestd) bestd = d, partner = j;
            }
            const int victim = i == 1 && partner >= 0 ? partner : i;
            if (victim == 1) continue;
            hipStream_t fresh = nullptr;
            if (hipStreamCreateWithFlags(&fresh, hipStreamNonBlocking) != hipSuccess) return MASP_HIP_E_HIP;
            (void)hipStreamDestroy(*at[victim]);
            *at[victim] = fresh;
            replaced = true;
        }
        if (!replaced) return MASP_HIP_OK;
    }
    return MASP_HIP_OK;
}

static int create_single(int device, const masp_hip_options& opt, masp_hip_ctx** out) {
    *out = nullptr;
    int count = 0;
    if (hipGetDeviceCount(&count) != hipSuccess || count <= 0 || device < 0 || device >= count) return MASP_HIP_E_NO_DEVICE;
    if (hipSetDevice(device) != hipSuccess) return MASP_HIP_E_NO_DEVICE;
    std::unique_ptr<masp_hip_ctx> ctx(new masp_hip_ctx);
    ctx->device = device;
    ctx->opt = opt;
    ctx->n_slots = opt.slots;
    ctx->batch_cap = (size_t)opt.batch_cap;
    ctx->slots.reserve(masp_hip_ctx::MAX_SLOTS);
    ctx->slot_busy.reserve(masp_hip_ctx::MAX_SLOTS);
    ctx->opt.hw_queues = measure_hw_queues(device, 5 * opt.slots);
    StreamTable& t = ctx->streams;
    bool ok = hipStreamCreateWithFlags(&t.main, hipStreamNonBlocking) == hipSuccess;
    t.slot.assign((size_t)opt.slots, std::array<hipStream_t, 5>{});
    for (size_t si = 0; si < t.slot.size(); ++si)
        for (int j = 0; j < 5; ++j) {
            if (j > 0 && si >= 2 && !opt.lone_proof_graph)
                t.slot[si][j] = t.slot[1][j];
            else
                ok = ok && hipStreamCreateWithFlags(&t.slot[si][j], hipStreamNonBlocking) == hipSuccess;
        }
    for (hipStream_t& v : t.vk) ok = ok && hipStreamCreateWithFlags(&v, hipStreamNonBlocking) == hipSuccess;
    if (!ok || separate_main_streams(ctx.get()) != MASP_HIP_OK) return MASP_HIP_E_NO_DEVICE;
    *out = ctx.release();
    return MASP_HIP_OK;
}

static int create_front(const int* devices, int n_devices, const masp_hip_options& opt, masp_hip_ctx** out) {
    std::unique_ptr<masp_hip_ctx> front(new masp_hip_ctx);
    front->device = devices[0];
    front->opt = opt;
    front->n_slots = opt.slots;
    front->batch_cap = (size_t)opt.batch_cap;
    for (int i = 0; i < n_devices; ++i) {
        masp_hip_ctx* ch = nullptr;
        if (int rc = create_single(devices[i], opt, &ch)) {
            for (masp_hip_ctx* c : front->children) masp_hip_ctx_destroy(c);
            return rc;
        }
        front->children.push_back(ch);
    }
    front->dev_status.reset(new std::atomic<int>[n_devices]);
    for (int i = 0; i < n_devices; ++i) front->dev_status[i] = MASP_HIP_OK;
    *out = front.release();
    return MASP_HIP_OK;
}

int masp_hip_ctx_create_ex(const int* devices, int n_devices, const masp_hip_options* opt_in, masp_hip_ctx** out) {
    if (!out || !devices || n_devices <= 0 || n_devices > 64) return MASP_HIP_E_INVALID_ARG;
    if (opt_in && opt_in->struct_size != 0 && opt_in->struct_size < 4 * sizeof(int32_t)) return MASP_HIP_E_INVALID_ARG;
    *out = nullptr;
    const masp_hip_options opt = resolve_options(opt_in);
    return n_devices == 1 ? create_single(devices[0], opt, out) : create_front(devices, n_devices, opt, out);
}

int masp_hip_ctx_get_options(const masp_hip_ctx* ctx, masp_hip_options* out) {
    if (!ctx || !out) return MASP_HIP_E_INVALID_ARG;
    const masp_hip_ctx* c = ctx->children.empty() ? ctx : ctx->children[0];
    const size_t room = out->struct_size ? std::min<size_t>(out->struct_size, sizeof(masp_hip_options)) : sizeof(masp_hip_options);
    if (room < 4 * sizeof(int32_t)) return MASP_HIP_E_INVALID_ARG;
    masp_hip_options full = c->opt, *const caller_out = out;
    out = &full;
    uint64_t fb = 0;
    int sub = out->bucket_tree_sub_batch;
    auto scan = [&](const masp_hip_ctx* d) {
        std::lock_guard<std::mutex> g(d->slot_mu);
        for (const auto& sl : d->slots) {
            fb += sl->ws1.tree_fallbacks + sl->ws2.tree_fallbacks;
            sub = std::min<int>(sub, (int)std::min(sl->ws1.tree_sub, sl->ws2.tree_sub));
        }
    };
    if (ctx->children.empty())
        scan(ctx);
    else
        for (const masp_hip_ctx* d : ctx->children) scan(d);
    fb += c->block_tree_fallbacks.load();
    if (c->block_tree_sub.load() != 0xffffffffu) sub = std::min<int>(sub, (int)c->block_tree_sub.load());
    out->bucket_tree_sub_batch = sub;
    out->bucket_tree_fallback_proofs = (int32_t)std::min<uint64_t>(fb, 0x7fffffff);
    full.struct_size = (uint32_t)room;
    memcpy(caller_out, &full, room);
    return MASP_HIP_OK;
}

int masp_hip_ctx_set_boolean_block_bits(masp_hip_ctx* ctx, int32_t bits) {
    if (!ctx || (bits != 0 && bits != -1 && bits != 2 && bits != 3)) return MASP_HIP_E_INVALID_ARG;
    const int resolved = bits == 0 ? (int)(MASP_SUBSET_BITS) : bits < 0 ? 0 : bits;
    auto set = [&](masp_hip_ctx* c) {
        std::unique_lock<std::shared_mutex> lock(c->mu);
        c->boolean_block_bits = resolved;
    };
    set(ctx);
    for (masp_hip_ctx* c : ctx->children) set(c);
    return MASP_HIP_OK;
}
int masp_hip_ctx_get_boolean_block_bits(const masp_hip_ctx* ctx, int32_t* out) {
    if (!ctx || !out) return MASP_HIP_E_INVALID_ARG;
    *out = (ctx->children.empty() ? ctx : ctx->children[0])->boolean_block_bits;
    return MASP_HIP_OK;
}

int masp_hip_ctx_create(int device, masp_hip_ctx** out) {
    if (!out) return MASP_HIP_E_INVALID_ARG;
    return masp_hip_ctx_create_ex(&device, 1, nullptr, out);
}

int masp_hip_ctx_create_multi(const int* devices, int n_devices, masp_hip_ctx** out) {
    if (!out || !devices || n_devices <= 0 || n_devices > 64) return MASP_HIP_E_INVALID_ARG;
    *out = nullptr;
    return create_front(devices, n_devices, resolve_options(nullptr), out);
}

int masp_hip_ctx_device_proofs(const masp_hip_ctx* ctx, uint64_t* counts, int cap) {
    if (!ctx || !counts || cap < 0) return MASP_HIP_E_INVALID_ARG;
    if (ctx->children.empty()) {
        if (cap >= 1) counts[0] = ctx->proofs_done.load();
        return MASP_HIP_OK;
    }
    for (size_t d = 0; d < ctx->children.size() && (int)d < cap; ++d) counts[d] = ctx->children[d]->proofs_done.load();
    return MASP_HIP_OK;
}
int masp_hip_ctx_device_status(const masp_hip_ctx* ctx, int32_t* status, int cap, uint64_t* requeued) {
    if (!ctx || !status || cap < 0) return MASP_HIP_E_INVALID_ARG;
    if (requeued) *requeued = ctx->requeued.load();
    if (ctx->children.empty()) {
        if (cap >= 1) status[0] = MASP_HIP_OK;
        return MASP_HIP_OK;
    }
    for (size_t d = 0; d < ctx->children.size() && (int)d < cap; ++d) status[d] = ctx->dev_status[d].load();
    return MASP_HIP_OK;
}
int masp_hip_ctx_inject_fault(masp_hip_ctx* ctx, int device, uint32_t nth) {
    if (!ctx || device < 0) return MASP_HIP_E_INVALID_ARG;
    if (ctx->children.empty()) {
        if (device != 0) return MASP_HIP_E_INVALID_ARG;
        ctx->fault_countdown = nth;
        return MASP_HIP_OK;
    }
    if ((size_t)device >= ctx->children.size()) return MASP_HIP_E_INVALID_ARG;
    ctx->children[device]->fault_countdown = nth;
    return MASP_HIP_OK;
}
int masp_hip_ctx_stream_concurrency(masp_hip_ctx* ctx, int mains_only, int* n_streams, int* concurrent) {
    if (!ctx || !n_streams || !concurrent) return MASP_HIP_E_INVALID_ARG;
    if (!ctx->children.empty()) ctx = ctx->children[0];
    std::unique_lock<std::shared_mutex> lock(ctx->mu);
    hipSetDevice(ctx->device);
    if (hipDeviceSynchronize() != hipSuccess) return fail(ctx, MASP_HIP_E_HIP);
    return fail(ctx, measure_own_streams(ctx, mains_only != 0, n_streams, concurrent));
}
int masp_hip_ctx_lone_graph_launches(const masp_hip_ctx* ctx, uint64_t* out) {
    if (!ctx || !out) return MASP_HIP_E_INVALID_ARG;
    *out = 0;
    if (!ctx->children.empty()) {
        for (const masp_hip_ctx* ch : ctx->children) {
            uint64_t v = 0;
            masp_hip_ctx_lone_graph_launches(ch, &v);
            *out += v;
        }
        return MASP_HIP_OK;
    }
    std::lock_guard<std::mutex> g(ctx->slot_mu);
    for (const auto& sl : ctx->slots) *out += sl->graph_launches.load();
    return MASP_HIP_OK;
}
int masp_hip_ctx_device_count(const masp_hip_ctx* ctx) { return !ctx ? 0 : ctx->children.empty() ? 1 : (int)ctx->children.size(); }

void masp_hip_ctx_destroy(masp_hip_ctx* ctx) {
    if (!ctx) return;
    if (!ctx->children.empty()) {
        for (masp_hip_ctx* c : ctx->children) masp_hip_ctx_destroy(c);
        delete ctx;
        return;
    }
    hipSetDevice(ctx->device);
    hipDeviceSynchronize();
    ctx->batches.clear();
    ctx->slots.clear();
    for (auto& c : ctx->circ) c.reset();
    ctx->domains.clear();
    delete ctx;
    dev_free_drain();
}

int masp_hip_circuit_load(masp_hip_ctx* ctx, uint32_t slot, const uint8_t* params, size_t params_len, const masp_hip_r1cs* cs) {
    const ApiLaunchScope api_scope;
    if (!ctx || !params || !cs || slot >= MASP_HIP_MAX_CIRCUITS || cs->n_inputs == 0) return MASP_HIP_E_INVALID_ARG;
    if (!ctx->children.empty()) {
        std::vector<int> rcs(ctx->children.size(), MASP_HIP_OK);
        std::vector<std::thread> th;
        for (size_t d = 0; d < ctx->children.size(); ++d)
            th.emplace_back([&, d] { rcs[d] = masp_hip_circuit_load(ctx->children[d], slot, params, params_len, cs); });
        for (auto& t : th) t.join();
        for (int rc : rcs)
            if (rc) return rc;
        return MASP_HIP_OK;
    }
    std::unique_lock<std::shared_mutex> lock(ctx->mu);
    hipSetDevice(ctx->device);
    hipStream_t s = ctx->streams.main;
    ParamsLayout L;
    if (!parse_params(params, params_len, L)) return MASP_HIP_E_PARAMS_FORMAT;
    std::unique_ptr<Circuit> C(new Circuit);
    C->n_inputs = cs->n_inputs;
    C->n_aux = cs->n_aux;
    C->n_constraints = cs->n_constraints;
    C->nrows = cs->n_constraints + cs->n_inputs;
    C->logm = log2_ceil(C->nrows);
    C->m = (size_t)1 << C->logm;
    const uint32_t nv = cs->n_inputs + cs->n_aux;
    std::vector<uint8_t> a_dense(nv, 0), b_dense(nv, 0);
    const uint32_t* rp[3] = {cs->a_rowptr, cs->b_rowptr, cs->c_rowptr};
    const uint32_t* cl[3] = {cs->a_col, cs->b_col, cs->c_col};
    const uint8_t* cf[3] = {cs->a_coef, cs->b_coef, cs->c_coef};
    for (int mi = 0; mi < 3; ++mi) {
        uint32_t nnz = rp[mi][cs->n_constraints];
        for (uint32_t t = 0; t < nnz; ++t) {
            if (cl[mi][t] >= nv) return MASP_HIP_E_INVALID_ARG;
            if (mi == 0) a_dense[cl[mi][t]] = 1;
            if (mi == 1) b_dense[cl[mi][t]] = 1;
        }
    }
    std::vector<uint32_t> a_var, b_var;
    for (uint32_t i = 0; i < cs->n_inputs; ++i) a_var.push_back(i);
    for (uint32_t v = cs->n_inputs; v < nv; ++v)
        if (a_dense[v]) a_var.push_back(v);
    for (uint32_t v = 0; v < nv; ++v)
        if (b_dense[v]) b_var.push_back(v);
    C->na = a_var.size();
    C->nbq = b_var.size();
    if (L.n_ic != cs->n_inputs || L.n_h < C->m - 1 || L.n_l != cs->n_aux || L.n_a != C->na || L.n_b1 != C->nbq || L.n_b2 != C->nbq)
        return MASP_HIP_E_PARAMS_SHAPE;
    int rc;
    if ((rc = C->a_var.upload(a_var.data(), a_var.size(), s)) || (rc = C->b_var.upload(b_var.data(), b_var.size(), s))) return fail(ctx, rc);
    DevBuf<int> d_flag;
    if ((rc = d_flag.reserve(1))) return fail(ctx, rc);
    hipMemsetAsync(d_flag.p, 0, sizeof(int), s);
    for (int mi = 0; mi < 3; ++mi) {
        uint32_t nnz = rp[mi][cs->n_constraints];
        DevBuf<Fr> raw;
        std::vector<uint32_t> order(cs->n_constraints);
        for (uint32_t r = 0; r < cs->n_constraints; ++r) order[r] = r;
        std::stable_sort(order.begin(), order.end(),
                         [&](uint32_t x, uint32_t y) { return rp[mi][x + 1] - rp[mi][x] > rp[mi][y + 1] - rp[mi][y]; });
        if ((rc = C->row_order[mi].upload(order.data(), order.size(), s))) return fail(ctx, rc);
        C->n_long_rows[mi] = 0;
        for (uint32_t r : order) {
            if (rp[mi][r + 1] - rp[mi][r] < R1CS_LONG_ROW) break;
            ++C->n_long_rows[mi];
        }
        if ((rc = C->rowptr[mi].upload(rp[mi], cs->n_constraints + 1, s)) || (rc = C->col[mi].upload(cl[mi], nnz, s)) ||
            (rc = raw.upload((const Fr*)cf[mi], nnz, s)) || (rc = C->coef[mi].reserve(nnz)))
            return fail(ctx, rc);
        if (nnz) launch_fr_to_mont(s, raw.p, (size_t)0, C->coef[mi].p, nnz, 1, d_flag.p);
        if (hipStreamSynchronize(s) != hipSuccess) return fail(ctx, MASP_HIP_E_HIP);
    }
    if ((rc = C->vk.reserve(1))) return fail(ctx, rc);
    {
        DevBuf<uint8_t> raw;
        if ((rc = raw.upload(params, 864, s))) return fail(ctx, rc);
        DevBuf<int> st;
        if ((rc = st.reserve(1))) return fail(ctx, rc);
        hipMemsetAsync(st.p, 0, sizeof(int), s);
        VkDevice* v = C->vk.p;
        launch_g1_import_one(s, raw.p + 0, &v->alpha_g1, st.p);
        launch_g1_import_one(s, raw.p + 96, &v->beta_g1, st.p);
        launch_g2_import_one(s, raw.p + 192, &v->beta_g2, st.p);
        launch_g1_import_one(s, raw.p + 576, &v->delta_g1, st.p);
        launch_g2_import_one(s, raw.p + 672, &v->delta_g2, st.p);
        int hst = 0, hflag = 0;
        if (hipMemcpyAsync(&hst, st.p, sizeof(int), hipMemcpyDeviceToHost, s) != hipSuccess ||
            hipMemcpyAsync(&hflag, d_flag.p, sizeof(int), hipMemcpyDeviceToHost, s) != hipSuccess || hipStreamSynchronize(s) != hipSuccess) {
            last_hip_error() = "vk import failed";
            return fail(ctx, MASP_HIP_E_HIP);
        }
        if (hflag) return MASP_HIP_E_SCALAR_RANGE;
        if (hst & (PT_BAD_FLAGS | PT_NOT_CANONICAL)) return MASP_HIP_E_PARAMS_FORMAT;
        DevBuf<G1Affine> p1;
        DevBuf<G2Affine> p2;
        if ((rc = p1.reserve(3)) || (rc = p2.reserve(1)) || (rc = C->fb1.reserve(3 * 32 * 255)) || (rc = C->fb2.reserve(32 * 255))) return fail(ctx, rc);
        hipMemcpyAsync(p1.p + 0, &v->delta_g1, sizeof(G1Affine), hipMemcpyDeviceToDevice, s);
        hipMemcpyAsync(p1.p + 1, &v->alpha_g1, sizeof(G1Affine), hipMemcpyDeviceToDevice, s);
        hipMemcpyAsync(p1.p + 2, &v->beta_g1, sizeof(G1Affine), hipMemcpyDeviceToDevice, s);
        hipMemcpyAsync(p2.p, &v->delta_g2, sizeof(G2Affine), hipMemcpyDeviceToDevice, s);
        launch_fixed_table_g1(s, p1.p, C->fb1.p, 3);
        launch_fixed_table_g2(s, p2.p, C->fb2.p, 1);
        if (hipStreamSynchronize(s) != hipSuccess) {
            last_hip_error() = std::string("fixed-base tables failed: ") + hipGetErrorString(hipGetLastError());
            return fail(ctx, MASP_HIP_E_HIP);
        }
        if ((params[576] & 0x40) || (params[672] & 0x40)) return MASP_HIP_E_UNEXPECTED_IDENTITY;
    }
    const uint32_t pct = (uint32_t)ctx->opt.witness_nontrivial_percent;
    auto eff = [&](uint32_t n) { return (uint32_t)((uint64_t)n * pct / 100); };
    const int c_la = ctx->opt.window_bits_la, c_b = ctx->opt.window_bits_b;
    const int c_b2 = ctx->opt.window_bits_b2 > 0 ? ctx->opt.window_bits_b2 : c_b;
    const uint32_t n_h = (uint32_t)(C->m - 1);
    const int c_h = ctx->opt.window_bits_h ? ctx->opt.window_bits_h : n_h >= 49152 ? 16 : n_h >= 16384 ? 15 : 0;
    const int c_h_lone = ctx->opt.window_bits_h_lone ? ctx->opt.window_bits_h_lone : c_h;
    const int sub_bits = ctx->boolean_block_bits;
    if ((rc = C->h.load_host(L.h, (uint32_t)(C->m - 1), s, 0xffffffffu, c_h_lone)) || (rc = C->l.load_host(L.l, L.n_l, s, eff(L.n_l), c_la)) ||
        (rc = C->a.load_host(L.a, L.n_a, s, eff(L.n_a), c_la, sub_bits)) || (rc = C->b1.load_host(L.b_g1, L.n_b1, s, eff(L.n_b1), c_b, sub_bits)) ||
        (rc = C->b2.load_host(L.b_g2, L.n_b2, s, eff(L.n_b2), c_b2, sub_bits)))
        return fail(ctx, rc);
    if (C->b1.sub.bits && C->b2.sub.bits && msm_same_sort(C->b1, C->b2)) {
        const uint32_t words = C->b1.sub.bad_words();
        std::vector<uint32_t> w1(words), w2(words);
        if (hipMemcpyAsync(w1.data(), C->b1.sub.bad, 4 * (size_t)words, hipMemcpyDeviceToHost, s) != hipSuccess ||
            hipMemcpyAsync(w2.data(), C->b2.sub.bad, 4 * (size_t)words, hipMemcpyDeviceToHost, s) != hipSuccess || hipStreamSynchronize(s) != hipSuccess)
            return fail(ctx, MASP_HIP_E_HIP);
        for (uint32_t i = 0; i < words; ++i) w1[i] |= w2[i];
        if (hipMemcpyAsync(C->b1.sub.bad, w1.data(), 4 * (size_t)words, hipMemcpyHostToDevice, s) != hipSuccess ||
            hipMemcpyAsync(C->b2.sub.bad, w1.data(), 4 * (size_t)words, hipMemcpyHostToDevice, s) != hipSuccess || hipStreamSynchronize(s) != hipSuccess)
            return fail(ctx, MASP_HIP_E_HIP);
    }
    {
        const int c_lone = ctx->opt.window_bits_b2_lone;
        if (c_lone > 0 && L.n_b2 && (rc = C->b2_lone.load_host(L.b_g2, L.n_b2, s, eff(L.n_b2), c_lone))) return fail(ctx, rc);
    }
    {
        const size_t nh = C->m - 1;
        std::vector<uint8_t> cat(96 * (nh + L.n_l));
        memcpy(cat.data(), L.h, 96 * nh);
        memcpy(cat.data() + 96 * nh, L.l, 96 * (size_t)L.n_l);
        const int c_hl = c_h ? c_h : ctx->opt.window_bits_h_lone ? 0 : C->h.g.c;
        if ((rc = C->hl.load_host(cat.data(), (uint32_t)(nh + L.n_l), s, 0xffffffffu, c_hl, sub_bits, (uint32_t)nh))) return fail(ctx, rc);
    }
    int st = C->h.import_status | C->l.import_status | C->a.import_status | C->b1.import_status | C->b2.import_status;
    if (st) return MASP_HIP_E_PARAMS_FORMAT;
    {
        DevBuf<int> out;
        if ((rc = out.reserve(1))) return fail(ctx, rc);
        hipMemsetAsync(out.p, 0, sizeof(int), s);
        launch_g1_subgroup_flag(s, C->a.tab, sizeof(*C->a.tab), C->a.n, out.p);
        launch_g1_subgroup_flag(s, C->b1.tab, sizeof(*C->b1.tab), C->b1.n, out.p);
        launch_g1_subgroup_flag(s, &C->vk.p->alpha_g1, 0, 1, out.p);
        launch_g1_subgroup_flag(s, &C->vk.p->beta_g1, 0, 1, out.p);
        launch_g1_subgroup_flag(s, &C->vk.p->delta_g1, 0, 1, out.p);
        int outside = 1;
        if (hipMemcpyAsync(&outside, out.p, sizeof(int), hipMemcpyDeviceToHost, s) != hipSuccess || hipStreamSynchronize(s) != hipSuccess ||
            launch_status() != MASP_HIP_OK)
            return fail(ctx, MASP_HIP_E_HIP);
        C->g1_endo = outside == 0;
    }
    if ((rc = get_domain(ctx, C->logm, &C->dom))) return fail(ctx, rc);
    ctx->circ[slot] = std::move(C);
    return MASP_HIP_OK;
}

int masp_hip_circuit_flags(const masp_hip_ctx* ctx, uint32_t slot, uint32_t* flags) {
    if (!ctx || !flags) return MASP_HIP_E_INVALID_ARG;
    if (!ctx->children.empty()) return masp_hip_circuit_flags(ctx->children[0], slot, flags);
    std::shared_lock<std::shared_mutex> lock(const_cast<masp_hip_ctx*>(ctx)->mu);
    if (slot >= MASP_HIP_MAX_CIRCUITS || !ctx->circ[slot]) return MASP_HIP_E_NOT_LOADED;
    *flags = ctx->circ[slot]->g1_endo ? MASP_HIP_CIRCUIT_G1_ENDOMORPHISM : 0u;
    return MASP_HIP_OK;
}

static int validate_jobs(const masp_hip_ctx* dev_ctx, size_t n, const masp_hip_job* jobs) {
    for (size_t j = 0; j < n; ++j) {
        const masp_hip_job& J = jobs[j];
        if (J.circuit >= MASP_HIP_MAX_CIRCUITS || !J.inputs || !J.aux) return MASP_HIP_E_INVALID_ARG;
        if (!dev_ctx->circ[J.circuit]) return MASP_HIP_E_NOT_LOADED;
        if ((J.a || J.b || J.c) && !(J.a && J.b && J.c)) return MASP_HIP_E_INVALID_ARG;
        if (J.reserved != 0) return MASP_HIP_E_INVALID_ARG;
        if (J.aux_form > MASP_HIP_AUX_MONTGOMERY || (J.aux_form && J.a)) return MASP_HIP_E_INVALID_ARG;
        if (!rs_in_range(J.r) || !rs_in_range(J.s)) return MASP_HIP_E_SCALAR_RANGE;
    }
    return MASP_HIP_OK;
}

static int prove_batch_multi(masp_hip_ctx* ctx, size_t n, const masp_hip_job* jobs, uint8_t* proofs_out) {
    const size_t nd = ctx->children.size();
    auto alive = [&](size_t d) { return ctx->dev_status[d].load() == MASP_HIP_OK; };
    size_t n_alive = 0, first_alive = nd;
    for (size_t d = 0; d < nd; ++d)
        if (alive(d)) {
            ++n_alive;
            if (first_alive == nd) first_alive = d;
        }
    if (!n_alive) return MASP_HIP_E_HIP;
    {
        std::shared_lock<std::shared_mutex> lock(ctx->children[first_alive]->mu);
        if (int rc = validate_jobs(ctx->children[first_alive], n, jobs)) return rc;
    }
    struct Block {
        std::vector<size_t> idx;
        uint64_t cost;
    };
    std::deque<Block> queue;
    {
        std::map<std::pair<uint32_t, bool>, std::vector<size_t>> by_kind;
        for (size_t j = 0; j < n; ++j) by_kind[{jobs[j].circuit | (jobs[j].aux_form ? 0x100u : 0u), jobs[j].a != nullptr}].push_back(j);
        std::vector<Block> blocks;
        for (auto& kv : by_kind) {
            const size_t cap = std::min(ctx->batch_cap, std::max<size_t>((kv.second.size() + n_alive - 1) / n_alive, 8));
            const Circuit& C = *ctx->children[first_alive]->circ[kv.first.first & 0xffu];
            for (auto& g : even_groups(kv.second.size(), cap)) {
                Block b;
                b.idx.assign(kv.second.begin() + g.first, kv.second.begin() + g.first + g.second);
                b.cost = (uint64_t)C.nrows * g.second;
                blocks.push_back(std::move(b));
            }
        }
        std::stable_sort(blocks.begin(), blocks.end(), [](const Block& x, const Block& y) { return x.cost > y.cost; });
        for (auto& b : blocks) queue.push_back(std::move(b));
    }
    std::mutex mu;
    std::condition_variable cv;
    size_t pending = queue.size();
    int fatal = MASP_HIP_OK;
    auto worker = [&](size_t d) {
        masp_hip_ctx* ch = ctx->children[d];
        std::vector<masp_hip_job> mine;
        std::vector<uint8_t> out;
        for (;;) {
            Block b;
            {
                std::unique_lock<std::mutex> g(mu);
                cv.wait(g, [&] { return !queue.empty() || pending == 0 || fatal || !alive(d); });
                if (pending == 0 || fatal || !alive(d)) return;
                b = std::move(queue.front());
                queue.pop_front();
            }
            mine.resize(b.idx.size());
            for (size_t k = 0; k < mine.size(); ++k) mine[k] = jobs[b.idx[k]];
            out.resize(192 * mine.size());
            const int rc = masp_hip_prove_batch(ch, mine.size(), mine.data(), out.data());
            std::unique_lock<std::mutex> g(mu);
            if (rc == MASP_HIP_OK) {
                for (size_t k = 0; k < b.idx.size(); ++k) memcpy(proofs_out + 192 * b.idx[k], out.data() + 192 * k, 192);
                --pending;
            } else if (rc == MASP_HIP_E_HIP || rc == MASP_HIP_E_NO_DEVICE) {
                int ok = MASP_HIP_OK;
                ctx->dev_status[d].compare_exchange_strong(ok, rc);
                ctx->requeued += b.idx.size();
                queue.push_front(std::move(b));
                bool any = false;
                for (size_t e = 0; e < nd; ++e) any = any || alive(e);
                if (!any) fatal = rc;
            } else {
                fatal = rc;
            }
            cv.notify_all();
            if (rc != MASP_HIP_OK) return;
        }
    };
    std::vector<std::thread> th;
    for (size_t d = 0; d < nd; ++d) {
        if (!alive(d)) continue;
        const size_t w = std::min<size_t>(std::max(ctx->children[d]->n_slots, 1), std::max<size_t>((queue.size() + n_alive - 1) / n_alive, 1));
        for (size_t k = 0; k < w; ++k) th.emplace_back(worker, d);
    }
    for (auto& t : th) t.join();
    if (fatal) return fatal;
    return pending == 0 ? MASP_HIP_OK : MASP_HIP_E_HIP;
}

int masp_hip_prove_batch(masp_hip_ctx* ctx, size_t n, const masp_hip_job* jobs, uint8_t* proofs_out) {
    const ApiLaunchScope api_scope;
    if (!ctx || (n && (!jobs || !proofs_out))) return MASP_HIP_E_INVALID_ARG;
    if (!ctx->children.empty()) return prove_batch_multi(ctx, n, jobs, proofs_out);
    std::shared_lock<std::shared_mutex> lock(ctx->mu);
    if (int rc = validate_jobs(ctx, n, jobs)) return rc;
    for (uint32_t left = ctx->fault_countdown.load(); left != 0;) {
        if (!ctx->fault_countdown.compare_exchange_weak(left, left - 1)) continue;
        if (left == 1) {
            last_hip_error() = "injected fault (masp_hip_ctx_inject_fault): this device context's call fails as a lost GPU's would";
            return fail(ctx, MASP_HIP_E_HIP);
        }
        break;
    }
    hipSetDevice(ctx->device);
    struct Group {
        std::vector<size_t> idx;
    };
    std::vector<Group> groups;
    {
        std::map<std::pair<uint32_t, bool>, std::vector<size_t>> by_kind;
        for (size_t j = 0; j < n; ++j) by_kind[{jobs[j].circuit | (jobs[j].aux_form ? 0x100u : 0u), jobs[j].a != nullptr}].push_back(j);
        for (auto& kv : by_kind)
            for (auto& eg : even_groups(kv.second.size(), ctx->batch_cap)) {
                Group g;
                g.idx.assign(kv.second.begin() + eg.first, kv.second.begin() + eg.first + eg.second);
                groups.push_back(std::move(g));
            }
    }
    struct Owned {
        size_t si, gi;
    };
    std::deque<Owned> owned;
    int result = MASP_HIP_OK, rc;
    auto retire_oldest = [&]() -> size_t {
        Owned o = owned.front();
        owned.pop_front();
        Slot& sl = *ctx->slots[o.si];
        const Group& G = groups[o.gi];
        if (hipEventSynchronize(sl.done) != hipSuccess) {
            last_hip_error() = "event sync failed";
            result = fail(ctx, MASP_HIP_E_HIP);
        } else if (*sl.h_flags) {
            result = MASP_HIP_E_SCALAR_RANGE;
        } else if (result == MASP_HIP_OK) {
            for (size_t p = 0; p < G.idx.size(); ++p) memcpy(proofs_out + 192 * G.idx[p], sl.h_proof + 192 * p, 192);
        }
        return o.si;
    };
#ifdef MASP_ENQ_TIMING
    const auto tcall = std::chrono::steady_clock::now();
    auto ms_since = [&](std::chrono::steady_clock::time_point t0) { return std::chrono::duration<double, std::milli>(std::chrono::steady_clock::now() - t0).count(); };
#endif
    for (size_t gi = 0; gi < groups.size() && result == MASP_HIP_OK; ++gi) {
        size_t si = 0;
#ifdef MASP_ENQ_TIMING
        const auto tg0 = std::chrono::steady_clock::now();
#endif
        rc = slot_try_acquire(ctx, &si);
        if (rc > 0) {
            result = fail(ctx, rc);
            break;
        }
        if (rc < 0) si = owned.empty() ? slot_acquire_blocking(ctx) : retire_oldest();
        if (result) {
            slot_release(ctx, si);
            break;
        }
        const Group& G = groups[gi];
        Slot& sl = *ctx->slots[si];
        Circuit& C = *ctx->circ[jobs[G.idx[0]].circuit];
        const size_t nv = (size_t)C.n_inputs + C.n_aux, np = G.idx.size();
        const bool has_abc = jobs[G.idx[0]].a != nullptr;
#ifdef MASP_ENQ_TIMING
        const double t_wait = ms_since(tg0);
        const auto tg1 = std::chrono::steady_clock::now();
#endif
        const size_t w_bytes = 32 * nv * np, abc_bytes = has_abc ? 3 * 32 * (size_t)C.nrows * np : 0, rs_bytes = 64 * np;
        const size_t in_bytes = 32 * (size_t)C.n_inputs * np;
        bool ok = true;
        if ((rc = sl.stage_reserve(w_bytes + abc_bytes + rs_bytes + in_bytes)) || (rc = sl.w.reserve(nv * np)) || (rc = sl.inp.reserve((size_t)C.n_inputs * np)) ||
            (rc = sl.abc.reserve(has_abc ? 3 * (size_t)C.nrows * np : 1)) || (rc = sl.reserve_batch(np))) {
            result = fail(ctx, rc);
            ok = false;
        }
        if (ok) {
            uint8_t* hs = sl.h_stage;
            std::vector<char> direct(np, 0);
            bool any_staged = false;
            for (size_t p = 0; p < np; ++p) {
                hipPointerAttribute_t attr;
                direct[p] = hipPointerGetAttributes(&attr, jobs[G.idx[p]].aux) == hipSuccess && attr.type == hipMemoryTypeHost;
                any_staged = any_staged || !direct[p];
            }
            (void)hipGetLastError();
            for (size_t p = 0; p < np; ++p) {
                const masp_hip_job& J = jobs[G.idx[p]];
                memcpy(hs + 32 * nv * p, J.inputs, 32 * (size_t)C.n_inputs);
                memcpy(hs + w_bytes + abc_bytes + rs_bytes + 32 * (size_t)C.n_inputs * p, J.inputs, 32 * (size_t)C.n_inputs);
                if (!direct[p]) memcpy(hs + 32 * nv * p + 32 * (size_t)C.n_inputs, J.aux, 32 * (size_t)C.n_aux);
                if (has_abc) {
                    const uint8_t* src[3] = {J.a, J.b, J.c};
                    for (int i = 0; i < 3; ++i) memcpy(hs + w_bytes + 32 * (size_t)C.nrows * (np * i + p), src[i], 32 * (size_t)C.nrows);
                }
                memcpy(hs + w_bytes + abc_bytes + 64 * p, J.r, 32);
                memcpy(hs + w_bytes + abc_bytes + 64 * p + 32, J.s, 32);
            }
            hipStream_t s = sl.stream;
#if MASP_UPLOAD_CHAIN
            const bool chain = ctx->opt.lone_proof_graph == 0;
            std::unique_lock<std::mutex> upload_turn(ctx->upload_mu, std::defer_lock);
            if (chain) upload_turn.lock();
            if (chain && ctx->upload_tail && ctx->upload_tail != sl.ev_uploaded) ok = hipStreamWaitEvent(s, ctx->upload_tail, 0) == hipSuccess;
#endif
            if (!ok) {
            } else if (any_staged) {
                ok = hipMemcpyAsync(sl.w.p, hs, w_bytes, hipMemcpyHostToDevice, s) == hipSuccess;
            } else {
                ok = hipMemcpyAsync(sl.inp.p, hs + w_bytes + abc_bytes + rs_bytes, in_bytes, hipMemcpyHostToDevice, s) == hipSuccess &&
                     hipMemcpy2DAsync(sl.w.p, 32 * nv, sl.inp.p, 32 * (size_t)C.n_inputs, 32 * (size_t)C.n_inputs, np, hipMemcpyDeviceToDevice, s) ==
                         hipSuccess;
            }
            for (size_t p = 0; p < np && ok; ++p)
                if (direct[p])
                    ok = hipMemcpyAsync(sl.w.p + nv * p + C.n_inputs, jobs[G.idx[p]].aux, 32 * (size_t)C.n_aux, hipMemcpyHostToDevice, s) ==
                         hipSuccess;
            ok = ok && (!has_abc || hipMemcpyAsync(sl.abc.p, hs + w_bytes, abc_bytes, hipMemcpyHostToDevice, s) == hipSuccess) &&
                 hipMemcpyAsync(sl.rs.p, hs + w_bytes + abc_bytes, rs_bytes, hipMemcpyHostToDevice, s) == hipSuccess;
#if MASP_UPLOAD_CHAIN
            if (chain && ok && hipEventRecord(sl.ev_uploaded, s) == hipSuccess) ctx->upload_tail = sl.ev_uploaded;
#endif
            if (!ok) {
                last_hip_error() = std::string("H2D copy failed: ") + hipGetErrorString(hipGetLastError());
                result = fail(ctx, MASP_HIP_E_HIP);
            }
        }
        if (ok) {
            const Fr* abc[3] = {nullptr, nullptr, nullptr};
            if (has_abc)
                for (int i = 0; i < 3; ++i) abc[i] = sl.abc.p + (size_t)C.nrows * np * i;
            if (hipMemsetAsync(sl.flags.p, 0, sizeof(int), sl.stream) != hipSuccess) {
                last_hip_error() = "memset failed";
                result = fail(ctx, MASP_HIP_E_HIP);
                ok = false;
            } else {
#ifdef MASP_ENQ_TIMING
                const auto tq0 = std::chrono::steady_clock::now();
#endif
                if ((rc = enqueue_proofs_graphed(sl, C, (uint32_t)np, sl.w.p, nv, abc, sl.rs.p, sl.proof.p, jobs[G.idx[0]].aux_form == MASP_HIP_AUX_MONTGOMERY))) {
                    result = fail(ctx, rc);
                    ok = false;
                }
#ifdef MASP_ENQ_TIMING
                fprintf(stderr, "[enq] %zu proofs: %.3f ms\n", np, std::chrono::duration<double, std::milli>(std::chrono::steady_clock::now() - tq0).count());
#endif
            }
        }
        if (ok) {
            hipStream_t s = sl.stream;
            ok = hipMemcpyAsync(sl.h_proof, sl.proof.p, 192 * np, hipMemcpyDeviceToHost, s) == hipSuccess &&
                 hipMemcpyAsync(sl.h_flags, sl.flags.p, sizeof(int), hipMemcpyDeviceToHost, s) == hipSuccess &&
                 hipEventRecord(sl.done, s) == hipSuccess;
            if (!ok) {
                last_hip_error() = "D2H copy failed";
                result = fail(ctx, MASP_HIP_E_HIP);
            }
        }
        if (!ok) {
            for (int i = 0; i < Slot::N_AUX; ++i) hipStreamSynchronize(sl.aux[i]);
            hipStreamSynchronize(sl.stream);
            slot_release(ctx, si);
            break;
        }
        owned.push_back({si, gi});
#ifdef MASP_ENQ_TIMING
        fprintf(stderr, "[grp] call %p t=%8.2f ms group %zu circuit %u np %zu slot %zu: waited %.2f ms for the slot, staged + enqueued in %.2f ms\n", (void*)jobs,
                ms_since(tcall), gi, jobs[G.idx[0]].circuit, np, si, t_wait, ms_since(tg1));
#endif
    }
    while (!owned.empty()) slot_release(ctx, retire_oldest());
#ifdef MASP_ENQ_TIMING
    fprintf(stderr, "[call] %p done after %.2f ms (%zu jobs)\n", (void*)jobs, ms_since(tcall), n);
#endif
    if (result == MASP_HIP_OK) ctx->proofs_done += n;
    const int launch_rc = launch_status();
    if (launch_rc && result == MASP_HIP_OK) result = fail(ctx, launch_rc);
    if (hipGetLastError() != hipSuccess && result == MASP_HIP_OK) {
        last_hip_error() = "kernel launch failed";
        result = fail(ctx, MASP_HIP_E_HIP);
    }
    return result;
}

int masp_hip_prove(masp_hip_ctx* ctx, uint32_t slot, const uint8_t* inputs, const uint8_t* aux, const uint8_t* a, const uint8_t* b,
                   const uint8_t* c, const uint8_t r[32], const uint8_t s[32], uint8_t proof_out[192]) {
    if (!r || !s || !proof_out) return MASP_HIP_E_INVALID_ARG;
    masp_hip_job J;
    J.circuit = slot;
    J.inputs = inputs;
    J.aux = aux;
// ... 460 lines not shown
```

masp_amd/hip.py:

```python
import ctypes as C
import os

import numpy as np

_HERE = os.path.dirname(os.path.abspath(__file__))
_lib = None

ERRORS = {1: "invalid argument", 2: "Parameters bytes are malformed", 3: "Parameters do not match the circuit shape",
          4: "no usable HIP device (there is no CPU fallback)", 5: "HIP runtime error", 6: "UnexpectedIdentity",
          7: "circuit slot is empty", 8: "scalar is not a canonical field element", 9: "a Jubjub point encoding does not decode",
          10: "an output buffer is too small"}
E_POINT_ENCODING = 9
E_CAPACITY = 10
SPEND_AUTH, BINDING = 0, 1

SPEND, OUTPUT, CONVERT = 0, 1, 2


class MaspHipError(RuntimeError):
    def __init__(self, code, detail=""):
        self.code = code
        super().__init__("masp_hip error %d: %s%s" % (code, ERRORS.get(code, "?"), (" — " + detail) if detail else ""))


OPTION_FIELDS = ("slots", "batch_cap", "ntt_sub_batch", "window_bits_h", "window_bits_la", "window_bits_b", "window_bits_b2_lone",
                 "witness_nontrivial_percent", "bucket_tree_levels", "bucket_tree_sub_batch", "bucket_tree_levels_g2", "bucket_tree_scratch_mb", "lone_proof_graph", "window_bits_h_lone",
                 "window_bits_b2")


class OptionsStruct(C.Structure):
    _fields_ = ([("struct_size", C.c_uint32)] + [(f, C.c_int32) for f in OPTION_FIELDS[:OPTION_FIELDS.index("lone_proof_graph")]] +
                [("bucket_tree_fallback_proofs", C.c_int32), ("lone_proof_graph", C.c_int32), ("hw_queues", C.c_int32), ("window_bits_h_lone", C.c_int32),
                 ("digit_recoding", C.c_int32),
                 ("window_bits_b2", C.c_int32)])


assert C.sizeof(OptionsStruct) == 76 and OptionsStruct.window_bits_b2.offset == 72


class JobStruct(C.Structure):
    _fields_ = [("circuit", C.c_uint32), ("inputs", C.c_void_p), ("aux", C.c_void_p), ("a", C.c_void_p),
                ("b", C.c_void_p), ("c", C.c_void_p), ("r", C.c_uint8 * 32), ("s", C.c_uint8 * 32), ("aux_form", C.c_uint32),
                ("reserved", C.c_uint32)]


assert C.sizeof(JobStruct) == 120 and JobStruct.r.offset == 48 and JobStruct.aux_form.offset == 112
AUX_CANONICAL, AUX_MONTGOMERY = 0, 1


def library_path():
    return os.environ.get("MASP_HIP_LIBRARY") or os.path.join(_HERE, "libmasp_hip.so")


def load_library():
    global _lib
    if _lib is not None:
        return _lib
    path = library_path()
    if not os.path.exists(path):
        raise ImportError("libmasp_hip.so is not built: run `python -c 'import __graft_entry__ as g; g.build()'` "
                          "or `make -C masp_amd/csrc` (hipcc, --offload-arch=gfx950)")
    os.environ.setdefault("GPU_MAX_HW_QUEUES", "16")
    L = C.CDLL(path)
    if hasattr(L, "masp_hip_runtime_prepare"):
        L.masp_hip_runtime_prepare.argtypes = [C.c_int, C.c_int]
        q = L.masp_hip_runtime_prepare(0, 0)
        if q > 20:
            import warnings
            warnings.warn("masp_amd: GPU_MAX_HW_QUEUES=%d: once this process holds more than 20 hardware queues every kernel dispatch gets "
                          "slower (24: -7 %%, 32: -21 %% proofs/s; profiles/r06_second_context_root_cause.txt) — use 16" % q)
    vp, sz, u32 = C.c_void_p, C.c_size_t, C.c_uint32
    L.masp_hip_ctx_create.argtypes = [C.c_int, C.POINTER(vp)]
    L.masp_hip_ctx_create_multi.argtypes = [C.POINTER(C.c_int), C.c_int, C.POINTER(vp)]
    L.masp_hip_ctx_create_ex.argtypes = [C.POINTER(C.c_int), C.c_int, C.POINTER(OptionsStruct), C.POINTER(vp)]
    L.masp_hip_ctx_get_options.argtypes = [vp, C.POINTER(OptionsStruct)]
    L.masp_hip_device_count.argtypes = []
    L.masp_hip_options_default.argtypes = [C.POINTER(OptionsStruct)]
    L.masp_hip_options_default.restype = None
    L.masp_hip_ctx_device_count.argtypes = [vp]
    L.masp_hip_ctx_device_proofs.argtypes = [vp, C.POINTER(C.c_uint64), C.c_int]
    if hasattr(L, "masp_hip_ctx_stream_concurrency"):
        L.masp_hip_ctx_stream_concurrency.argtypes = [vp, C.c_int, C.POINTER(C.c_int), C.POINTER(C.c_int)]
    if hasattr(L, "masp_hip_ctx_device_status"):
        L.masp_hip_ctx_device_status.argtypes = [vp, C.POINTER(C.c_int32), C.c_int, C.POINTER(C.c_uint64)]
        L.masp_hip_ctx_inject_fault.argtypes = [vp, C.c_int, C.c_uint32]
    if hasattr(L, "masp_hip_ctx_lone_graph_launches"):
        L.masp_hip_ctx_lone_graph_launches.argtypes = [vp, C.POINTER(C.c_uint64)]
    if hasattr(L, "masp_hip_circuit_flags"):
        L.masp_hip_circuit_flags.argtypes = [vp, u32, C.POINTER(C.c_uint32)]
    L.masp_hip_ctx_destroy.argtypes = [vp]
    L.masp_hip_ctx_destroy.restype = None
    L.masp_hip_strerror.restype = C.c_char_p
    L.masp_hip_last_error.argtypes = [vp]
    L.masp_hip_last_error.restype = C.c_char_p
    L.masp_hip_circuit_load.argtypes = [vp, u32, vp, sz, vp]
    L.masp_hip_prove.argtypes = [vp, u32, vp, vp, vp, vp, vp, C.c_char_p, C.c_char_p, vp]
    L.masp_hip_prove_batch.argtypes = [vp, sz, vp, vp]
    L.masp_hip_generate_parameters.argtypes = [vp, vp, C.c_char_p, vp, sz, C.POINTER(sz)]
    L.masp_hip_parameters_max_size.argtypes = [vp]
    L.masp_hip_parameters_max_size.restype = sz
    L.masp_hip_msm_g1.argtypes = [vp, vp, vp, sz, vp]
    L.masp_hip_msm_g2.argtypes = [vp, vp, vp, sz, vp]
    L.masp_hip_msm_g1_multi.argtypes = [vp, vp, sz, vp, sz, C.c_int, vp]
    L.masp_hip_msm_g2_multi.argtypes = [vp, vp, sz, vp, sz, C.c_int, vp]
    if hasattr(L, "masp_hip_msm_g1_multi_ex"):
        L.masp_hip_msm_g1_multi_ex.argtypes = [vp, vp, sz, vp, sz, C.c_int, C.c_int, sz, sz, vp, vp]
        L.masp_hip_msm_g2_multi_ex.argtypes = [vp, vp, sz, vp, sz, C.c_int, C.c_int, sz, sz, vp, vp]
        L.masp_hip_ctx_set_boolean_block_bits.argtypes = [vp, C.c_int32]
        L.masp_hip_ctx_get_boolean_block_bits.argtypes = [vp, C.POINTER(C.c_int32)]
    L.masp_hip_quotient_h.argtypes = [vp, vp, vp, vp, sz, u32, vp]
    L.masp_hip_ntt.argtypes = [vp, vp, u32, C.c_int]
    L.masp_hip_vk_prepare.argtypes = [vp, vp, sz, C.POINTER(vp)]
    L.masp_hip_vk_free.argtypes = [vp]
    L.masp_hip_vk_free.restype = None
    L.masp_hip_verify_batch.argtypes = [vp, vp, sz, vp, vp, u32, vp, C.POINTER(C.c_int)]
    if hasattr(L, "masp_hip_redjubjub_verify_batch"):
        L.masp_hip_jubjub_msm.argtypes = [vp, sz, vp, vp, vp, C.POINTER(C.c_int64)]
        L.masp_hip_redjubjub_verify_batch.argtypes = [vp, sz, C.c_char_p, C.c_char_p, C.c_char_p, C.c_char_p, C.c_char_p, C.POINTER(C.c_int)]
    if hasattr(L, "masp_hip_sapling_trial_decrypt"):
        L.masp_hip_sapling_trial_decrypt.argtypes = [vp, sz, vp, sz, vp, vp, vp, sz, vp, vp, vp, C.POINTER(sz)]
        L.masp_hip_note_scan_configure.argtypes = [vp, C.c_int, C.c_int]
        L.masp_hip_note_scan_last_timing.argtypes = [vp, C.POINTER(C.c_double)]
    if hasattr(L, "masp_hip_sapling_compact_trial_decrypt"):
        L.masp_hip_sapling_compact_trial_decrypt.argtypes = [vp, sz, vp, sz, vp, vp, vp, C.c_int, vp, sz, vp, vp, vp, vp, C.POINTER(sz), C.POINTER(sz)]
        L.masp_hip_note_scan_compact_last_timing.argtypes = [vp, C.POINTER(C.c_double)]
    if hasattr(L, "masp_hip_sapling_output_recovery_scan"):
        L.masp_hip_sapling_output_recovery_scan.argtypes = [vp, sz, vp, sz, vp, vp, vp, vp, sz, vp, vp, vp, C.POINTER(sz)]
        L.masp_hip_out_recovery_last_timing.argtypes = [vp, C.POINTER(C.c_double)]
    if hasattr(L, "masp_hip_merkle_tree_complete"):
        L.masp_hip_merkle_tree_complete.argtypes = [vp, C.c_uint, sz, vp, vp, sz, C.POINTER(sz), vp, sz, vp, vp, C.POINTER(C.c_int64)]
        L.masp_hip_merkle_last_timing.argtypes = [vp, C.POINTER(C.c_double)]
    if hasattr(L, "masp_hip_merkle_tree_append"):
        L.masp_hip_merkle_tree_append.argtypes = [vp, C.c_uint64, vp, sz, vp, vp, sz, C.POINTER(sz), C.POINTER(C.c_int64)]
    L.masp_hip_batch_upload.argtypes = [vp, sz, vp]
    L.masp_hip_batch_prove_resident.argtypes = [vp, C.c_int, vp, C.POINTER(C.c_float)]
    L.masp_hip_batch_prove_resident_steps.argtypes = [vp, C.c_int, sz, vp, vp, C.POINTER(C.c_float)]
    L.masp_hip_batch_free.argtypes = [vp, C.c_int]
    L.masp_hip_bench_msm.argtypes = [vp, C.c_int, sz, C.c_int, C.c_int, C.POINTER(C.c_float), C.POINTER(u32)]
    L.masp_hip_profile_enable.argtypes = [vp, C.c_int]
    L.masp_hip_profile_read.argtypes = [vp, C.POINTER(C.c_double), C.POINTER(C.c_uint64), C.POINTER(C.c_uint64)]
    L.masp_hip_profile_read_split.argtypes = [vp, C.POINTER(C.c_double)]
    if hasattr(L, "masp_hip_profile_read_lone"):
        L.masp_hip_profile_read_lone.argtypes = [vp, C.POINTER(C.c_double)]
    L.masp_hip_sync.argtypes = [vp]
    L.masp_hip_host_alloc.argtypes = [vp, sz]
    L.masp_hip_host_alloc.restype = vp
    L.masp_hip_host_free.argtypes = [vp, vp]
    L.masp_hip_host_free.restype = None
    _lib = L
    return L


def device_pci_bus_id(device=0):
    L = load_library()
    if not hasattr(L, "masp_hip_device_pci_bus_id"):
        return None
    buf = C.create_string_buffer(64)
    L.masp_hip_device_pci_bus_id.argtypes = [C.c_int, C.c_char_p, C.c_size_t]
    return buf.value.decode().lower() if L.masp_hip_device_pci_bus_id(int(device), buf, 64) == 0 else None


def device_count():
    return int(load_library().masp_hip_device_count())


def _p(a):
    return a.ctypes.data_as(C.c_void_p) if a is not None else None


def _u8(a, shape_last=None):
    if a is None:
        return None
    if isinstance(a, (bytes, bytearray, memoryview)):
        a = np.frombuffer(a, dtype=np.uint8)
    a = np.ascontiguousarray(a, dtype=np.uint8)
    if shape_last is not None:
        a = a.reshape(-1, shape_last)
    return a


def _scalar32(x):
    if isinstance(x, int):
        return x.to_bytes(32, "little")
    b = bytes(x)
    assert len(b) == 32
    return b


class Context:

    def __init__(self, device=0, **options):
        self._L = load_library()
        h = C.c_void_p()
        unknown = set(options) - set(OPTION_FIELDS)
        if unknown:
            raise TypeError("unknown context option(s): %s" % ", ".join(sorted(unknown)))
        opt = OptionsStruct()
        self._L.masp_hip_options_default(C.byref(opt))
        for k, v in options.items():
            if v is not None:
                setattr(opt, k, int(v))
        if isinstance(device, (list, tuple)):
            arr = (C.c_int * len(device))(*[int(d) for d in device])
            if options or len(device) > 1:
                rc = self._L.masp_hip_ctx_create_ex(arr, len(device), C.byref(opt), C.byref(h))
            else:
                rc = self._L.masp_hip_ctx_create_multi(arr, len(device), C.byref(h))
        else:
            arr = (C.c_int * 1)(int(device))
            rc = self._L.masp_hip_ctx_create_ex(arr, 1, C.byref(opt), C.byref(h))
        if rc:
            raise MaspHipError(rc)
        got = OptionsStruct()
        got.struct_size = C.sizeof(OptionsStruct)
        self._L.masp_hip_ctx_get_options(h, C.byref(got))
        self.options = {f: int(getattr(got, f)) for f in OPTION_FIELDS}
        self.options["hw_queues"] = int(got.hw_queues)
        want = min(5 * self.options["slots"], 15)
        if 0 < self.options["hw_queues"] < want:
            import warnings
            warnings.warn("masp_amd: the HIP runtime gives this process %d hardware queue(s) for %d slots x 5 streams: set GPU_MAX_HW_QUEUES=16 "
                          "before the process's first HIP call (masp_hip_runtime_prepare)" % (self.options["hw_queues"], self.options["slots"]))

        self._h = h
        self._keep = []
        self._pinned = {}

    def close(self):
        if getattr(self, "_h", None):
            for p in list(getattr(self, "_pinned", {}).values()):
                self._L.masp_hip_host_free(self._h, p)
            self._pinned = {}
            self._L.masp_hip_ctx_destroy(self._h)
            self._h = None

    def __del__(self):
        try:
            self.close()
        except Exception:
            pass

    def _check(self, rc):
        if rc:
            raise MaspHipError(rc, self._L.masp_hip_last_error(self._h).decode(errors="replace"))

    def host_alloc(self, rows, cols=32):
        p = self._L.masp_hip_host_alloc(self._h, rows * cols)
        if not p:
            raise MemoryError("masp_hip_host_alloc(%d bytes) failed" % (rows * cols))
        buf = (C.c_uint8 * (rows * cols)).from_address(p)
        a = np.frombuffer(buf, dtype=np.uint8).reshape(rows, cols)
        self._pinned[a.ctypes.data] = p
        return a

    def host_free(self, a):
        p = self._pinned.pop(a.ctypes.data, None)
        if p and getattr(self, "_h", None):
            self._L.masp_hip_host_free(self._h, p)

    def load_circuit(self, slot, params, cs):
        params = _u8(params)
        self._check(self._L.masp_hip_circuit_load(self._h, slot, _p(params), params.size, cs.ref))

    def _job(self, slot, inputs, aux, r, s, abc=None, aux_form=AUX_CANONICAL):
        j = JobStruct()
        j.circuit = slot
        j.aux_form = int(aux_form)
        inputs, aux = _u8(inputs, 32), _u8(aux, 32)
        keep = [inputs, aux]
        j.inputs, j.aux = inputs.ctypes.data, aux.ctypes.data
        if abc is not None:
            a, b, c = (_u8(x, 32) for x in abc)
            keep += [a, b, c]
            j.a, j.b, j.c = a.ctypes.data, b.ctypes.data, c.ctypes.data
        j.r[:] = _scalar32(r)
        j.s[:] = _scalar32(s)
        return j, keep

    def prove(self, slot, inputs, aux, r, s, abc=None):
        return self.prove_batch([(slot, inputs, aux, r, s, abc)])[0]

    def marshal_jobs(self, jobs):
        jobs = list(jobs)
        arr = (JobStruct * len(jobs))()
        keep = []
        for i, job in enumerate(jobs):
            slot, inputs, aux, r, s = job[:5]
            abc = job[5] if len(job) > 5 else None
            arr[i], k = self._job(slot, inputs, aux, r, s, abc, job[6] if len(job) > 6 else AUX_CANONICAL)
            keep.append(k)
        return arr, len(jobs), keep

    def prove_marshalled(self, arr, n, out=None):
        if out is None:
            out = np.zeros((n, 192), dtype=np.uint8)
        self._check(self._L.masp_hip_prove_batch(self._h, n, arr, _p(out)))
        return out

    def prove_batch(self, jobs):
        arr, n, keep = self.marshal_jobs(jobs)
        out = self.prove_marshalled(arr, n)
        return [out[i].tobytes() for i in range(n)]

    def generate_parameters(self, cs, toxic):
        t = b"".join(_scalar32(x) for x in toxic)
        cap = self._L.masp_hip_parameters_max_size(cs.ref)
        out = np.zeros(cap, dtype=np.uint8)
        n = C.c_size_t(0)
        self._check(self._L.masp_hip_generate_parameters(self._h, cs.ref, t, _p(out), cap, C.byref(n)))
        return out[:n.value].copy()

    def prepare_verifying_key(self, params):
        return GpuVerifyingKey(self, params)

    def redjubjub_verify_batch(self, items, randomness=None):
        import secrets
        items = list(items)
        n = len(items)
        if n == 0:
            return True
        vks, sigs, sighashes = (b"".join(bytes(it[k]) for it in items) for k in range(3))
        if len(vks) != 32 * n or len(sigs) != 64 * n or len(sighashes) != 32 * n:
            return False
        kinds = bytes(int(it[3]) for it in items)
        z = randomness if randomness is not None else secrets.token_bytes(16 * n)
        assert len(z) == 16 * n
        ok = C.c_int(0)
        self._check(self._L.masp_hip_redjubjub_verify_batch(self._h, n, vks, sigs, sighashes, kinds, bytes(z), C.byref(ok)))
        return ok.value == 1

    def jubjub_msm(self, points, scalars):
        n = len(points)
        assert len(scalars) == n
        pts = np.frombuffer(b"".join(bytes(p) for p in points), dtype=np.uint8)
        sc = np.frombuffer(b"".join(_scalar32(s) for s in scalars), dtype=np.uint8)
        assert pts.size == 32 * n and sc.size == 32 * n
        out = np.zeros(32, dtype=np.uint8)
        bad = C.c_int64(-1)
        rc = self._L.masp_hip_jubjub_msm(self._h, n, _p(pts), _p(sc), _p(out), C.byref(bad))
        if rc == E_POINT_ENCODING:
            e = MaspHipError(rc, "point %d" % bad.value)
            e.bad_index = bad.value
            raise e
        self._check(rc)
        return out.tobytes()

    def _scan_with_room(self, fn, args, widths, n_out, hit_capacity, tail=()):
        cap = max(16, n_out // 64) if hit_capacity is None else int(hit_capacity)
        while True:
            hits = [np.zeros(cap, np.uint32), np.zeros(cap, np.uint32)] + [np.zeros((cap, w), np.uint8) for w in widths]
            nh = C.c_size_t(0)
            rc = fn(self._h, *args, cap, *[_p(h) for h in hits], C.byref(nh), *tail)
            if rc == E_CAPACITY and hit_capacity is None:
                cap = nh.value
                continue
            if rc == E_CAPACITY:
                e = MaspHipError(rc, "%d hits" % nh.value)
                e.needed = nh.value
                raise e
            self._check(rc)
            return [h[:nh.value] for h in hits]

    def sapling_trial_decrypt(self, ivks, epks, enc_ciphertexts, hit_capacity=None):
        ivks, epks, encs = _u8(ivks, 32), _u8(epks, 32), _u8(enc_ciphertexts, 612)
        n_ivk, n_out = ivks.shape[0], epks.shape[0]
        assert encs.shape[0] == n_out
        status = np.zeros(n_out, dtype=np.uint8)
        ho, hi, hk = self._scan_with_room(self._L.masp_hip_sapling_trial_decrypt, (n_ivk, _p(ivks), n_out, _p(epks), _p(encs), _p(status)), (32,),
                                          n_out, hit_capacity)
        return status, ho, hi, hk

    def note_scan_configure(self, signed_digits=1, inversion=0):
        self._check(self._L.masp_hip_note_scan_configure(self._h, int(signed_digits), int(inversion)))

    def note_scan_last_timing(self):
        ms = (C.c_double * 2)()
        self._check(self._L.masp_hip_note_scan_last_timing(self._h, ms))
        return ms[0], ms[1]

    def sapling_compact_trial_decrypt(self, ivks, epks, cmus, enc_compact, lead_byte=2, hit_capacity=None, count_candidates=True):
        ivks, epks, cmus, encs = _u8(ivks, 32), _u8(epks, 32), _u8(cmus, 32), _u8(enc_compact, 84)
        n_ivk, n_out = ivks.shape[0], epks.shape[0]
        assert encs.shape[0] == n_out and cmus.shape[0] == n_out
        status = np.zeros(n_out, dtype=np.uint8)
        nc = C.c_size_t(0)
        ho, hi, hp, hk = self._scan_with_room(self._L.masp_hip_sapling_compact_trial_decrypt,
                                              (n_ivk, _p(ivks), n_out, _p(epks), _p(cmus), _p(encs), int(lead_byte), _p(status)), (84, 32), n_out,
                                              hit_capacity, tail=(C.byref(nc) if count_candidates else None,))
        return status, ho, hi, hp, hk, (nc.value if count_candidates else None)

    def note_scan_compact_last_timing(self):
        ms = (C.c_double * 3)()
        self._check(self._L.masp_hip_note_scan_compact_last_timing(self._h, ms))
        return ms[0], ms[1], ms[2]

    def sapling_output_recovery_scan(self, ovks, cvs, epks, cmus, c_outs, hit_capacity=None):
        ovks, cvs, epks, cmus, couts = _u8(ovks, 32), _u8(cvs, 32), _u8(epks, 32), _u8(cmus, 32), _u8(c_outs, 80)
        n_ovk, n_out = ovks.shape[0], epks.shape[0]
        assert cvs.shape[0] == n_out and cmus.shape[0] == n_out and couts.shape[0] == n_out
        return tuple(self._scan_with_room(self._L.masp_hip_sapling_output_recovery_scan,
                                          (n_ovk, _p(ovks), n_out, _p(cvs), _p(epks), _p(cmus), _p(couts)), (32,), n_out, hit_capacity))

    def out_recovery_last_timing(self):
        ms = (C.c_double * 2)()
        self._check(self._L.masp_hip_out_recovery_last_timing(self._h, ms))
        return ms[0], ms[1]

    def merkle_tree_complete(self, row, height0=0, positions=(), want_nodes=True, nodes_capacity=None):
        row = _u8(row, 32)
        pos = np.ascontiguousarray(positions, dtype=np.uint64).reshape(-1)
        n, depth = row.shape[0], max(0, 32 - int(height0))
        paths = np.zeros((pos.shape[0], depth, 32), np.uint8)
        root = np.zeros(32, np.uint8)
        nn, bad = C.c_size_t(0), C.c_int64(-1)
        if want_nodes and nodes_capacity is None:
            from .host import merkle_node_count
            nodes_capacity = merkle_node_count(n, int(height0))
        nodes = np.zeros((int(nodes_capacity), 32), np.uint8) if want_nodes else None
        rc = self._L.masp_hip_merkle_tree_complete(self._h, int(height0), n, _p(row) if n else None, _p(nodes), int(nodes_capacity or 0),
                                                   C.byref(nn), _p(root), pos.shape[0], _p(pos) if pos.shape[0] else None, _p(paths),
                                                   C.byref(bad))
        if rc:
            detail = "node %d is not canonical" % bad.value if bad.value >= 0 else \
                "%d nodes" % nn.value if rc == E_CAPACITY else self._L.masp_hip_last_error(self._h).decode(errors="replace")
            e = MaspHipError(rc, detail)
            e.bad_index, e.needed = bad.value, nn.value
            raise e
        return (nodes[:nn.value] if want_nodes else None), root.tobytes(), paths

    def merkle_tree_append(self, start, frontier, row, nodes_capacity=None):
        from .host import merkle_append_args, merkle_append_error, merkle_append_node_count
        row, frontier = merkle_append_args(start, frontier, row)
        n = row.shape[0]
        if nodes_capacity is None:
            nodes_capacity = merkle_append_node_count(int(start), n)
        nodes = np.zeros((max(1, int(nodes_capacity)), 32), np.uint8)
        nn, bad = C.c_size_t(0), C.c_int64(-1)
        rc = self._L.masp_hip_merkle_tree_append(self._h, int(start), _p(frontier), n, _p(row) if n else None, _p(nodes), int(nodes_capacity),
                                                 C.byref(nn), C.byref(bad))
        if rc:
            detail = merkle_append_error("merkle_tree_append", bad.value) if bad.value != -1 else \
                "%d nodes" % nn.value if rc == E_CAPACITY else self._L.masp_hip_last_error(self._h).decode(errors="replace")
            e = MaspHipError(rc, detail)
            e.bad_index, e.needed = bad.value, nn.value
            raise e
        return nodes[:nn.value]

    def merkle_last_timing(self):
        ms = (C.c_double * 3)()
        self._check(self._L.masp_hip_merkle_last_timing(self._h, ms))
        return ms[0], ms[1], ms[2]

    def msm_g1(self, bases, scalars):
        bases, scalars = _u8(bases, 96), _u8(scalars, 32)
        out = np.zeros(96, dtype=np.uint8)
        self._check(self._L.masp_hip_msm_g1(self._h, _p(bases), _p(scalars), scalars.shape[0], _p(out)))
        return out.tobytes()

    def msm_g2(self, bases, scalars):
        bases, scalars = _u8(bases, 192), _u8(scalars, 32)
        out = np.zeros(192, dtype=np.uint8)
        self._check(self._L.masp_hip_msm_g2(self._h, _p(bases), _p(scalars), scalars.shape[0], _p(out)))
        return out.tobytes()

    def msm_g1_multi(self, bases, scalars, window_bits=0):
        bases = _u8(bases, 96)
        scalars = np.ascontiguousarray(scalars, dtype=np.uint8)
        npf, n = scalars.shape[0], scalars.shape[1]
        assert scalars.shape == (npf, n, 32) and bases.shape[0] == n
        out = np.zeros((npf, 96), dtype=np.uint8)
        self._check(self._L.masp_hip_msm_g1_multi(self._h, _p(bases), n, _p(scalars), npf, int(window_bits), _p(out)))
        return [out[i].tobytes() for i in range(npf)]

    def msm_g2_multi(self, bases, scalars, window_bits=0):
        bases = _u8(bases, 192)
        scalars = np.ascontiguousarray(scalars, dtype=np.uint8)
        npf, n = scalars.shape[0], scalars.shape[1]
        assert scalars.shape == (npf, n, 32) and bases.shape[0] == n
        out = np.zeros((npf, 192), dtype=np.uint8)
        self._check(self._L.masp_hip_msm_g2_multi(self._h, _p(bases), n, _p(scalars), npf, int(window_bits), _p(out)))
        return [out[i].tobytes() for i in range(npf)]

    def _msm_multi_ex(self, fn, size, bases, scalars, window_bits, block_bits, sub_lo, sub_hi):
        bases = _u8(bases, size)
        scalars = np.ascontiguousarray(scalars, dtype=np.uint8)
        npf, n = scalars.shape[0], scalars.shape[1]
        assert scalars.shape == (npf, n, 32) and bases.shape[0] == n
        out = np.zeros((npf, size), dtype=np.uint8)
        cnt = np.zeros(npf, dtype=np.uint32)
        self._check(fn(self._h, _p(bases), n, _p(scalars), npf, int(window_bits), int(block_bits), int(sub_lo), int(n if sub_hi is None else sub_hi),
                       _p(out), _p(cnt)))
        return [out[i].tobytes() for i in range(npf)], [int(c) for c in cnt]

    def msm_g1_multi_ex(self, bases, scalars, window_bits=0, block_bits=0, sub_lo=0, sub_hi=None):
        return self._msm_multi_ex(self._L.masp_hip_msm_g1_multi_ex, 96, bases, scalars, window_bits, block_bits, sub_lo, sub_hi)

    def msm_g2_multi_ex(self, bases, scalars, window_bits=0, block_bits=0, sub_lo=0, sub_hi=None):
        return self._msm_multi_ex(self._L.masp_hip_msm_g2_multi_ex, 192, bases, scalars, window_bits, block_bits, sub_lo, sub_hi)

    def set_boolean_block_bits(self, bits):
        self._check(self._L.masp_hip_ctx_set_boolean_block_bits(self._h, int(bits)))

    @property
    def boolean_block_bits(self):
        v = C.c_int32(0)
        self._check(self._L.masp_hip_ctx_get_boolean_block_bits(self._h, C.byref(v)))
        return int(v.value)

    def current_options(self):
        got = OptionsStruct()
        got.struct_size = C.sizeof(OptionsStruct)
        self._check(self._L.masp_hip_ctx_get_options(self._h, C.byref(got)))
        d = {f: int(getattr(got, f)) for f in OPTION_FIELDS}
        d["bucket_tree_fallback_proofs"] = int(got.bucket_tree_fallback_proofs)
        d["hw_queues"] = int(got.hw_queues)
        return d

    @property
    def device_count(self):
        return self._L.masp_hip_ctx_device_count(self._h)

    def circuit_uses_endomorphism(self, slot):
        f = C.c_uint32(0)
        self._check(self._L.masp_hip_circuit_flags(self._h, int(slot), C.byref(f)))
        return bool(f.value & 1)

    def lone_graph_launches(self):
        v = C.c_uint64(0)
        self._check(self._L.masp_hip_ctx_lone_graph_launches(self._h, C.byref(v)))
        return int(v.value)

    def device_proofs(self):
        n = self.device_count
        counts = (C.c_uint64 * n)()
        self._check(self._L.masp_hip_ctx_device_proofs(self._h, counts, n))
        return list(counts)

    def stream_concurrency(self, mains_only=False):
        n, c = C.c_int(0), C.c_int(0)
        self._check(self._L.masp_hip_ctx_stream_concurrency(self._h, 1 if mains_only else 0, C.byref(n), C.byref(c)))
        return int(n.value), int(c.value)

    def device_status(self):
        n = self.device_count
        st, rq = (C.c_int32 * n)(), C.c_uint64(0)
        self._check(self._L.masp_hip_ctx_device_status(self._h, st, n, C.byref(rq)))
        return list(st), int(rq.value)

    def inject_fault(self, device, nth):
        self._check(self._L.masp_hip_ctx_inject_fault(self._h, int(device), int(nth)))

    def quotient_h(self, a, b, c, logm):
        a, b, c = _u8(a, 32), _u8(b, 32), _u8(c, 32)
        out = np.zeros(((1 << logm) - 1, 32), dtype=np.uint8)
        self._check(self._L.masp_hip_quotient_h(self._h, _p(a), _p(b), _p(c), a.shape[0], logm, _p(out)))
        return out

    def ntt(self, data, logm, inverse=False):
        d = _u8(data, 32).copy()
        self._check(self._L.masp_hip_ntt(self._h, _p(d), logm, 1 if inverse else 0))
        return d

    def batch_upload(self, jobs):
        jobs = list(jobs)
        arr = (JobStruct * len(jobs))()
        keep = []
        for i, job in enumerate(jobs):
            slot, inputs, aux, r, s = job[:5]
            arr[i], k = self._job(slot, inputs, aux, r, s, None, job[6] if len(job) > 6 else AUX_CANONICAL)
            keep.append(k)
        h = self._L.masp_hip_batch_upload(self._h, len(jobs), arr)
        if h < 0:
            raise MaspHipError(-h, self._L.masp_hip_last_error(self._h).decode(errors="replace"))
        return h, len(jobs)

    def batch_prove_resident(self, handle, n):
        out = np.zeros((n, 192), dtype=np.uint8)
        ms = C.c_float(0)
        self._check(self._L.masp_hip_batch_prove_resident(self._h, handle, _p(out), C.byref(ms)))
        return [out[i].tobytes() for i in range(n)], ms.value

    def batch_prove_resident_steps(self, handle, n, steps, rs=None):
        out = np.zeros((steps, n, 192), dtype=np.uint8)
        ms = C.c_float(0)
        if rs is not None:
            rs = np.ascontiguousarray(rs, dtype=np.uint8)
            assert rs.shape == (steps, n, 64)
        self._check(self._L.masp_hip_batch_prove_resident_steps(self._h, handle, steps, _p(rs), _p(out), C.byref(ms)))
        return out, ms.value

    def batch_free(self, handle):
        self._check(self._L.masp_hip_batch_free(self._h, handle))

    def profile_enable(self, on=True):
        self._check(self._L.masp_hip_profile_enable(self._h, 1 if on else 0))

    def profile_read_split(self):
        ms = (C.c_double * 8)()
        self._check(self._L.masp_hip_profile_read_split(self._h, ms))
        return dict(zip(("plan_records_copies", "k_tree_pass1", "k_binv", "k_tree_pass2", "k_msm_accumulate_pts"), [float(x) for x in ms[:5]]))

    LONE_MARKS = ("start", "msm_a", "s_A", "msm_b1", "r_B1", "msm_b2", "g_b", "quotient", "msm_h", "msm_l", "g_a_g_c", "complete")

    def profile_read_lone(self):
        ms = (C.c_double * 12)()
        self._check(self._L.masp_hip_profile_read_lone(self._h, ms))
        return {k: round(float(v), 3) for k, v in zip(self.LONE_MARKS, ms)}

    def profile_read(self):
        t, l, b = C.c_double(0), C.c_uint64(0), C.c_uint64(0)
        self._check(self._L.masp_hip_profile_read(self._h, C.byref(t), C.byref(l), C.byref(b)))
        return t.value, l.value, b.value

    def sync(self):
        self._check(self._L.masp_hip_sync(self._h))

    def bench_msm(self, handle, job, which, iters):
        ms, nb = C.c_float(0), C.c_uint32(0)
        self._check(self._L.masp_hip_bench_msm(self._h, handle, job, which, iters, C.byref(ms), C.byref(nb)))
        return ms.value, nb.value


class GpuVerifyingKey:

    def __init__(self, ctx, params):
        self._ctx = ctx
        buf = _u8(params)
        n_ic = int.from_bytes(buf[864:868].tobytes(), "big")
        self._buf = buf[:868 + 96 * n_ic].copy()
        self.n_public = n_ic - 1
        h = C.c_void_p()
        ctx._check(ctx._L.masp_hip_vk_prepare(ctx._h, _p(self._buf), self._buf.size, C.byref(h)))
        self._h = h

    def verify_batch(self, proofs, public_inputs, randomness=None):
        import secrets
        n = len(proofs)
        if n == 0:
            return True
        if len(public_inputs) != n or any(len(pi) != self.n_public for pi in public_inputs):
            return False
        pr = np.frombuffer(b"".join(bytes(p) for p in proofs), dtype=np.uint8)
        if pr.size != 192 * n:
            return False
        pi = np.frombuffer(b"".join(_scalar32(x) for row in public_inputs for x in row), dtype=np.uint8) if self.n_public else None
        z = randomness if randomness is not None else secrets.token_bytes(16 * n)
        assert len(z) == 16 * n
        zb = np.frombuffer(z, dtype=np.uint8)
        ok = C.c_int(0)
        rc = self._ctx._L.masp_hip_verify_batch(self._ctx._h, self._h, n, _p(pr), _p(pi), self.n_public, _p(zb), C.byref(ok))
        if rc == 8:
            return False
        self._ctx._check(rc)
        return ok.value == 1

    def close(self):
        if getattr(self, "_h", None) and getattr(self._ctx, "_h", None):
            self._ctx._L.masp_hip_vk_free(self._h)
        self._h = None

    def __del__(self):
        try:
            self.close()
        except Exception:
            pass
```

Measured before the change: 1406 proofs/s.

## Compute quotient MSM in evaluation form using precomputed transformed H/L bases

At circuit load, builds a new set of G1 bases by running a group-element NTT over the H query points and folding in the C-matrix columns, so the quotient polynomial can be committed directly from evaluations. Per proof, the inverse/coset NTT round-trips for h are replaced by a pointwise A*B product scaled by a constant, and C's contribution is absorbed into per-witness bases. This makes evaluation form the default and removes most per-proof NTT work, at the cost of a heavy one-time setup (scalar multiplications of curve points) and a larger base table that includes extra slots for aux and used inputs.

```diff
diff --git a/include/masp_hip.h b/include/masp_hip.h
--- a/include/masp_hip.h
+++ b/include/masp_hip.h
@@ -81,6 +81,10 @@
 int masp_hip_ctx_create_multi(const int* devices, int n_devices, masp_hip_ctx** out);
 int masp_hip_ctx_set_boolean_block_bits(masp_hip_ctx* ctx, int32_t bits);
 int masp_hip_ctx_get_boolean_block_bits(const masp_hip_ctx* ctx, int32_t* out);
+#define MASP_HIP_QUOTIENT_EVALUATION 0
+#define MASP_HIP_QUOTIENT_COEFFICIENT 1
+int masp_hip_ctx_set_quotient_form(masp_hip_ctx* ctx, int32_t form);
+int masp_hip_ctx_get_quotient_form(const masp_hip_ctx* ctx, int32_t* out);
 int masp_hip_ctx_device_count(const masp_hip_ctx* ctx);
 int masp_hip_ctx_device_proofs(const masp_hip_ctx* ctx, uint64_t* counts, int cap);
 int masp_hip_ctx_device_status(const masp_hip_ctx* ctx, int32_t* status, int cap, uint64_t* requeued);
@@ -94,6 +98,10 @@
 int masp_hip_circuit_load(masp_hip_ctx* ctx, uint32_t slot, const uint8_t* params, size_t params_len, const masp_hip_r1cs* cs);
 #define MASP_HIP_CIRCUIT_G1_ENDOMORPHISM 1u
 int masp_hip_circuit_flags(const masp_hip_ctx* ctx, uint32_t slot, uint32_t* flags);
+
+int masp_hip_circuit_quotient_form(const masp_hip_ctx* ctx, uint32_t slot, int32_t* form);
+int masp_hip_circuit_eval_bases(const masp_hip_ctx* ctx, uint32_t slot, uint8_t* bases, size_t cap_points, size_t* n_points, uint32_t* input_cols,
+                                size_t cap_inputs, size_t* n_input_cols);
 
 int masp_hip_prove(masp_hip_ctx* ctx, uint32_t slot, const uint8_t* inputs, const uint8_t* aux, const uint8_t* a,
                    const uint8_t* b, const uint8_t* c, const uint8_t r[32], const uint8_t s[32], uint8_t proof_out[192]);
diff --git a/masp_amd/csrc/device/ntt.hpp b/masp_amd/csrc/device/ntt.hpp
--- a/masp_amd/csrc/device/ntt.hpp
+++ b/masp_amd/csrc/device/ntt.hpp
@@ -53,6 +53,14 @@
     b += (size_t)NTT_P << logm;
     y += (size_t)NTT_P << logm;
     fr_store(y + bitrev(k, logm), fe_mul(fr_load(a + k), fr_load(b + k)));
+}
+__global__ void k_ntt_ab_eval(const Fr* __restrict__ a, const Fr* __restrict__ b, Fr scale, Fr* __restrict__ y, uint32_t n, size_t y_stride) {
+    uint32_t k = blockIdx.x * blockDim.x + threadIdx.x;
+    if (k >= n) return;
+    a += (size_t)NTT_P * n;
+    b += (size_t)NTT_P * n;
+    y += (size_t)NTT_P * y_stride;
+    fr_store(y + k, fe_mul(fe_mul(fr_load(a + k), fr_load(b + k)), scale));
 }
 __global__ void k_fr_scale_sub(const Fr* __restrict__ x, const Fr* __restrict__ scale, const Fr* __restrict__ c, Fr cscale, Fr* __restrict__ y,
                                uint32_t n, size_t y_stride) {
diff --git a/masp_amd/csrc/device/r1cs.hpp b/masp_amd/csrc/device/r1cs.hpp
--- a/masp_amd/csrc/device/r1cs.hpp
+++ b/masp_amd/csrc/device/r1cs.hpp
@@ -68,11 +68,11 @@
 }
 
 __global__ void k_gather_scalars(const Fr* __restrict__ src, size_t src_stride, const uint32_t* __restrict__ idx, uint32_t n,
-                                 Fr* __restrict__ dst) {
+                                 Fr* __restrict__ dst, size_t dst_stride) {
     uint32_t k = blockIdx.x * blockDim.x + threadIdx.x;
     if (k >= n) return;
     src += blockIdx.y * src_stride;
-    dst += (size_t)blockIdx.y * n;
+    dst += (size_t)blockIdx.y * dst_stride;
     fr_store(dst + k, fr_load(src + idx[k]));
 }
 
diff --git a/masp_amd/csrc/device/setup.hpp b/masp_amd/csrc/device/setup.hpp
--- a/masp_amd/csrc/device/setup.hpp
+++ b/masp_amd/csrc/device/setup.hpp
@@ -81,4 +81,99 @@
     fr_store(out + i, fe_mul(fe_pow(tau, e, 1), c));
 }
 
+
+
+__global__ void __launch_bounds__(64) k_g1ntt_load(const uint8_t* __restrict__ h_raw, uint32_t n_h, const Fr* __restrict__ scale_tab, Fr scale_const,
+                                                   uint32_t logm, G1Xyzz* __restrict__ X) {
+    const uint32_t k = blockIdx.x * blockDim.x + threadIdx.x;
+    if (k >= (1u << logm)) return;
+    X += (size_t)blockIdx.y << logm;
+    G1Xyzz r = xyzz_inf<FpOps>();
+    if (k < n_h) {
+        G1Affine p;
+        g1_read_uncompressed(h_raw + (size_t)96 * k, p);
+        const Fr sc = blockIdx.y == 0 ? fr_load(scale_tab + k) : scale_const;
+        r = xyzz_mul_scalar(xyzz_from_affine(p), sc.v);
+    }
+    X[__brev(k) >> (32 - logm)] = r;
 }
+__global__ void __launch_bounds__(64) k_g1ntt_stage(G1Xyzz* __restrict__ X, const Fr* __restrict__ tw, uint32_t logm, uint32_t st) {
+    const uint32_t b = blockIdx.x * blockDim.x + threadIdx.x;
+    if (b >= (1u << (logm - 1))) return;
+    X += (size_t)blockIdx.y << logm;
+    const uint32_t j = b & ((1u << st) - 1u), i0 = ((b >> st) << (st + 1)) | j, i1 = i0 + (1u << st);
+    G1Xyzz u = X[i0], t = X[i1];
+    if (j) {
+        const Fr w = fe_from_mont(fr_load(tw + ((size_t)j << (logm - st - 1))));
+        t = xyzz_mul_scalar(t, w.v);
+    }
+    G1Xyzz v = u;
+    xyzz_add_nc(v, t);
+    xyzz_add_nc(u, xyzz_neg(t));
+    X[i0] = v;
+    X[i1] = u;
+}
+__global__ void __launch_bounds__(64) k_g1_xyzz_to_bytes(const G1Xyzz* __restrict__ X, uint32_t n, uint8_t* __restrict__ out, int* __restrict__ any_inf) {
+    const uint32_t i = blockIdx.x * blockDim.x + threadIdx.x;
+    if (i >= n) return;
+    const G1Affine p = xyzz_to_affine(X[i]);
+    if (aff_is_inf(p)) atomicOr(any_inf, 1);
+    g1_write_uncompressed(p, out + (size_t)96 * i);
+}
+
+__device__ __forceinline__ void eval_combine_term(G1Xyzz& acc, const G1Xyzz& p, const Fr& c, const Fr& minus_one) {
+    Fr one = fe_zero<FrCfg>();
+    one.v[0] = 1;
+    if (fe_eq(c, one))
+        xyzz_add_nc(acc, p);
+    else if (fe_eq(c, minus_one))
+        xyzz_add_nc(acc, xyzz_neg(p));
+    else
+        xyzz_add_nc(acc, xyzz_mul_scalar(p, c.v));
+}
+__device__ __forceinline__ void eval_combine_finish(G1Xyzz acc, uint32_t o, uint32_t n_aux, const uint8_t* __restrict__ l_raw, uint8_t* __restrict__ out,
+                                                    int* __restrict__ any_inf) {
+    if (o < n_aux) {
+        G1Affine l;
+        g1_read_uncompressed(l_raw + (size_t)96 * o, l);
+        xyzz_madd_nc(acc, l, false);
+    }
+    const G1Affine p = xyzz_to_affine(acc);
+    if (aff_is_inf(p)) atomicOr(any_inf, 1);
+    g1_write_uncompressed(p, out + (size_t)96 * o);
+}
+__global__ void __launch_bounds__(64) k_eval_combine(const uint32_t* __restrict__ colptr, const uint32_t* __restrict__ rowidx, const Fr* __restrict__ coef,
+                                                     const G1Xyzz* __restrict__ T, const uint32_t* __restrict__ slot_cols, uint32_t n_slots, uint32_t n_aux,
+                                                     uint32_t long_col, Fr minus_one, const uint8_t* __restrict__ l_raw, uint8_t* __restrict__ out,
+                                                     int* __restrict__ any_inf) {
+    const uint32_t o = blockIdx.x * blockDim.x + threadIdx.x;
+    if (o >= n_slots) return;
+    const uint32_t v = slot_cols[o], lo = colptr[v], hi = colptr[v + 1];
+    if (hi - lo >= long_col) return;
+    G1Xyzz acc = xyzz_inf<FpOps>();
+    for (uint32_t t = lo; t < hi; ++t) eval_combine_term(acc, T[rowidx[t]], fr_load(coef + t), minus_one);
+    eval_combine_finish(acc, o, n_aux, l_raw, out, any_inf);
+}
+__global__ void __launch_bounds__(64) k_eval_combine_long(const uint32_t* __restrict__ colptr, const uint32_t* __restrict__ rowidx, const Fr* __restrict__ coef,
+                                                          const G1Xyzz* __restrict__ T, const uint32_t* __restrict__ slot_cols,
+                                                          const uint32_t* __restrict__ long_slots, uint32_t n_aux, Fr minus_one,
+                                                          const uint8_t* __restrict__ l_raw, uint8_t* __restrict__ out, int* __restrict__ any_inf) {
+    const uint32_t o = long_slots[blockIdx.x], lane = threadIdx.x;
+    const uint32_t v = slot_cols[o], lo = colptr[v], hi = colptr[v + 1];
+    G1Xyzz acc = xyzz_inf<FpOps>();
+    for (uint32_t t = lo + lane; t < hi; t += 64) eval_combine_term(acc, T[rowidx[t]], fr_load(coef + t), minus_one);
+    for (int d = 32; d >= 1; d >>= 1) {
+        G1Xyzz other;
+#pragma unroll
+        for (int i = 0; i < 12; ++i) {
+            other.X.v[i] = (uint32_t)__shfl_down((int)acc.X.v[i], d, 64);
+            other.Y.v[i] = (uint32_t)__shfl_down((int)acc.Y.v[i], d, 64);
+            other.ZZ.v[i] = (uint32_t)__shfl_down((int)acc.ZZ.v[i], d, 64);
+            other.ZZZ.v[i] = (uint32_t)__shfl_down((int)acc.ZZZ.v[i], d, 64);
+        }
+        xyzz_add_nc(acc, other);
+    }
+    if (lane == 0) eval_combine_finish(acc, o, n_aux, l_raw, out, any_inf);
+}
+
+}
diff --git a/masp_amd/csrc/host/eval_form.h b/masp_amd/csrc/host/eval_form.h
--- /dev/null
+++ b/masp_amd/csrc/host/eval_form.h
@@ -0,0 +1,58 @@
+#pragma once
+#include <cstddef>
+#include <cstdint>
+#include <cstring>
+#include <vector>
+
+namespace masp {
+
+struct CscMatrix {
+    std::vector<uint32_t> colptr, rowidx;
+    std::vector<uint8_t> coef;
+    uint32_t len(uint32_t v) const { return colptr[v + 1] - colptr[v]; }
+};
+static inline bool csc_from_csr(uint32_t n_rows, uint32_t n_cols, const uint32_t* rowptr, const uint32_t* col, const uint8_t* coef, CscMatrix& out) {
+    const uint32_t nnz = rowptr[n_rows];
+    out.colptr.assign((size_t)n_cols + 1, 0);
+    out.rowidx.assign(nnz, 0);
+    out.coef.assign((size_t)32 * nnz, 0);
+    for (uint32_t t = 0; t < nnz; ++t) {
+        if (col[t] >= n_cols) return false;
+        ++out.colptr[col[t] + 1];
+    }
+    for (uint32_t v = 0; v < n_cols; ++v) out.colptr[v + 1] += out.colptr[v];
+    std::vector<uint32_t> fill(out.colptr.begin(), out.colptr.end() - 1);
+    for (uint32_t row = 0; row < n_rows; ++row)
+        for (uint32_t t = rowptr[row]; t < rowptr[row + 1]; ++t) {
+            const uint32_t pos = fill[col[t]]++;
+            out.rowidx[pos] = row;
+            memcpy(&out.coef[(size_t)32 * pos], coef + (size_t)32 * t, 32);
+        }
+    return true;
+}
+
+struct EvalLayout {
+    size_t m = 0;
+    uint32_t n_inputs = 0, n_aux = 0;
+    std::vector<uint32_t> used_inputs;
+    std::vector<uint32_t> long_slots;
+    static constexpr uint32_t LONG_COL = 64;
+    size_t aux_off() const { return m; }
+    size_t in_off() const { return m + n_aux; }
+    size_t n() const { return m + n_aux + used_inputs.size(); }
+    uint32_t n_slots() const { return n_aux + (uint32_t)used_inputs.size(); }
+    uint32_t slot_col(uint32_t o) const { return o < n_aux ? n_inputs + o : used_inputs[o - n_aux]; }
+};
+static inline EvalLayout eval_layout(const CscMatrix& c, uint32_t n_inputs, uint32_t n_aux, size_t m) {
+    EvalLayout L;
+    L.m = m;
+    L.n_inputs = n_inputs;
+    L.n_aux = n_aux;
+    for (uint32_t v = 0; v < n_inputs; ++v)
+        if (c.len(v)) L.used_inputs.push_back(v);
+    for (uint32_t o = 0; o < L.n_slots(); ++o)
+        if (c.len(L.slot_col(o)) >= EvalLayout::LONG_COL) L.long_slots.push_back(o);
+    return L;
+}
+
+}
diff --git a/masp_amd/csrc/internal.h b/masp_amd/csrc/internal.h
--- a/masp_amd/csrc/internal.h
+++ b/masp_amd/csrc/internal.h
@@ -15,6 +15,7 @@
 #include <vector>
 
 #include "chunk_pipeline.h"
+#include "host/eval_form.h"
 #include "device/io.hpp"
 #include "device/ntt_geom.h"
 #include "launch.h"
@@ -72,6 +73,7 @@
     size_t m = 0;
     DevBuf<Fr> tw_fwd, tw_inv, coset_scale, h_scale;
     Fr c_scale;
+    Fr e_scale;
     int init(uint32_t logm_, hipStream_t s) {
         logm = logm_;
         m = (size_t)1 << logm;
@@ -84,6 +86,7 @@
         const Fr zinv = fe_inv(fe_sub(fe_pow(g, e, 2), fe_one<FrCfg>()));
         const Fr mzinv = fe_mul(minv, zinv);
         c_scale = fe_from_mont(mzinv);
+        e_scale = fe_from_mont(zinv);
         Fr one = fe_one<FrCfg>();
         size_t half = std::max<size_t>(m / 2, 1);
         int rc;
@@ -118,6 +121,10 @@
     DevBuf<G2Xyzz> fb2;
     BasesG1 h, l, a, b1;
     BasesG1 hl;
+    BasesG1 hl_eval;
+    DevBuf<uint32_t> eval_in_var;
+    uint32_t n_eval_in = 0;
+    std::vector<uint32_t> eval_inputs;
     BasesG2 b2;
     BasesG2 b2_lone;
     bool g1_endo = false;
@@ -283,6 +290,7 @@
     std::vector<masp_hip_ctx*> children;
     masp_hip_options opt{};
     int boolean_block_bits = MASP_SUBSET_BITS;
+    int quotient_form = 0;
     int n_slots = 4;
     size_t batch_cap = 256;
     std::shared_mutex mu;
@@ -369,6 +377,13 @@
     return MASP_HIP_OK;
 }
 
+struct EvalBases {
+    DevBuf<uint8_t> d_raw;
+    EvalLayout lay;
+    bool usable = false;
+};
+int build_eval_bases(masp_hip_ctx* ctx, const NttDomain& D, const uint8_t* h_raw, const uint8_t* l_raw, const masp_hip_r1cs* cs, EvalBases& out);
+
 constexpr size_t NS_MAX_IVKS = 4096;
 constexpr size_t NS_MAX_OUTPUTS = (size_t)1 << 26;
 int ns_recode_ivks(std::vector<uint32_t>& digits, size_t n_ivk, const uint8_t* ivks, bool signed_digits);
diff --git a/masp_amd/csrc/k_ntt.hip b/masp_amd/csrc/k_ntt.hip
--- a/masp_amd/csrc/k_ntt.hip
+++ b/masp_amd/csrc/k_ntt.hip
@@ -25,6 +25,9 @@
 void launch_ntt_ab_bitrev(hipStream_t s, const Fr* a, const Fr* b, Fr* y, uint32_t logm, uint32_t np) {
     MASP_LAUNCH(k_ntt_ab_bitrev, dim3(((1u << logm) + 255) / 256, np), dim3(256), 0, s, a, b, y, logm);
 }
+void launch_ntt_ab_eval(hipStream_t s, const Fr* a, const Fr* b, const Fr& scale, Fr* y, uint32_t n, uint32_t np, size_t y_stride) {
+    MASP_LAUNCH(k_ntt_ab_eval, dim3((n + 255) / 256, np), dim3(256), 0, s, a, b, scale, y, n, y_stride);
+}
 void launch_fr_scale_sub(hipStream_t s, const Fr* x, const Fr* scale, const Fr* c, const Fr& cscale, Fr* y, uint32_t n, uint32_t np, size_t y_stride) {
     MASP_LAUNCH(k_fr_scale_sub, dim3((n + 255) / 256, np), dim3(256), 0, s, x, scale, c, cscale, y, n, y_stride ? y_stride : (size_t)n);
 }
@@ -40,12 +43,13 @@
 void launch_fr_split_forms(hipStream_t s, Fr* x, size_t x_stride, Fr* y, uint32_t n, uint32_t mont_from, uint32_t np, int* range_err) {
     MASP_LAUNCH(k_fr_split_forms, dim3((n + 255) / 256, np), dim3(256), 0, s, x, x_stride, y, n, mont_from, range_err);
 }
-void launch_r1cs_eval(hipStream_t s, const R1csMatrices& M, const Fr* w, uint32_t n_vars, uint32_t n_constraints, uint32_t n_inputs, uint32_t np) {
-    const uint32_t nl = std::max(M.n_long[0], std::max(M.n_long[1], M.n_long[2])), lanes = n_constraints + n_inputs + nl * 63u;
-    MASP_LAUNCH(k_r1cs_eval, dim3((lanes + 127) / 128, np, 3), dim3(128), 0, s, M, w, n_vars, n_constraints, n_inputs);
+void launch_r1cs_eval(hipStream_t s, const R1csMatrices& M, const Fr* w, uint32_t n_vars, uint32_t n_constraints, uint32_t n_inputs, uint32_t np,
+                      uint32_t n_mat) {
+    const uint32_t nl = std::max(M.n_long[0], std::max(M.n_long[1], n_mat > 2 ? M.n_long[2] : 0u)), lanes = n_constraints + n_inputs + nl * 63u;
+    MASP_LAUNCH(k_r1cs_eval, dim3((lanes + 127) / 128, np, n_mat), dim3(128), 0, s, M, w, n_vars, n_constraints, n_inputs);
 }
-void launch_gather_scalars(hipStream_t s, const Fr* src, size_t src_stride, const uint32_t* idx, uint32_t n, Fr* dst, uint32_t np) {
-    MASP_LAUNCH(k_gather_scalars, dim3((n + 255) / 256, np), dim3(256), 0, s, src, src_stride, idx, n, dst);
+void launch_gather_scalars(hipStream_t s, const Fr* src, size_t src_stride, const uint32_t* idx, uint32_t n, Fr* dst, uint32_t np, size_t dst_stride) {
+    MASP_LAUNCH(k_gather_scalars, dim3((n + 255) / 256, np), dim3(256), 0, s, src, src_stride, idx, n, dst, dst_stride ? dst_stride : (size_t)n);
 }
 
 }
diff --git a/masp_amd/csrc/k_setup.hip b/masp_amd/csrc/k_setup.hip
--- a/masp_amd/csrc/k_setup.hip
+++ b/masp_amd/csrc/k_setup.hip
@@ -2,6 +2,57 @@
 #include "internal.h"
 
 using namespace masp;
+
+int masp::build_eval_bases(masp_hip_ctx* ctx, const NttDomain& D, const uint8_t* h_raw, const uint8_t* l_raw, const masp_hip_r1cs* cs, EvalBases& out) {
+    hipStream_t s = ctx->streams.main;
+    const uint32_t logm = D.logm, n_in = cs->n_inputs, n_aux = cs->n_aux, nv = n_in + n_aux;
+    const size_t m = D.m;
+    out.usable = false;
+    if (logm < 1 || m > ((size_t)1 << 30)) return MASP_HIP_OK;
+    const uint32_t n_h = (uint32_t)(m - 1);
+    CscMatrix csc;
+    if (!csc_from_csr(cs->n_constraints, nv, cs->c_rowptr, cs->c_col, cs->c_coef, csc)) return MASP_HIP_E_INVALID_ARG;
+    out.lay = eval_layout(csc, n_in, n_aux, m);
+    const EvalLayout& lay = out.lay;
+    std::vector<uint32_t> slot_cols(lay.n_slots());
+    for (uint32_t o = 0; o < lay.n_slots(); ++o) slot_cols[o] = lay.slot_col(o);
+    const Fr minv = fe_inv(fr_from_u64_mont(m)), ginv = fr_const(FrCfg::GEN_INV);
+    const Fr neg_mzinv = fe_from_mont(fe_neg(fe_to_mont(D.c_scale))), minus_one = fe_from_mont(fe_neg(fe_one<FrCfg>()));
+    DevBuf<uint8_t> d_h, d_l;
+    DevBuf<Fr> scale, d_coef;
+    DevBuf<G1Xyzz> X;
+    DevBuf<uint32_t> d_colptr, d_rowidx, d_slot_cols, d_long;
+    DevBuf<int> d_inf;
+    int rc;
+    if ((rc = d_h.upload(h_raw, (size_t)96 * n_h, s)) || (rc = d_l.upload(l_raw, (size_t)96 * n_aux, s)) || (rc = scale.reserve(m)) ||
+        (rc = X.reserve(2 * m)) || (rc = out.d_raw.reserve((size_t)96 * lay.n())) || (rc = d_inf.reserve(1)) ||
+        (rc = d_colptr.upload(csc.colptr.data(), csc.colptr.size(), s)) || (rc = d_rowidx.upload(csc.rowidx.data(), csc.rowidx.size(), s)) ||
+        (rc = d_coef.upload((const Fr*)csc.coef.data(), csc.rowidx.size(), s)) || (rc = d_slot_cols.upload(slot_cols.data(), slot_cols.size(), s)) ||
+        (rc = d_long.upload(lay.long_slots.data(), lay.long_slots.size(), s)))
+        return rc;
+    HIP_TRY(hipMemsetAsync(d_inf.p, 0, sizeof(int), s));
+    launch_fr_powers(s, scale.p, (uint32_t)m, ginv, minv, 1);
+    const dim3 block(64);
+    MASP_LAUNCH(k_g1ntt_load, dim3((uint32_t)((m + 63) / 64), 2), block, 0, s, d_h.p, n_h, scale.p, neg_mzinv, logm, X.p);
+    for (uint32_t st = 0; st < logm; ++st)
+        MASP_LAUNCH(k_g1ntt_stage, dim3((uint32_t)((m / 2 + 63) / 64), 2), block, 0, s, X.p, D.tw_inv.p, logm, st);
+    MASP_LAUNCH(k_g1_xyzz_to_bytes, dim3((uint32_t)((m + 63) / 64)), block, 0, s, X.p, (uint32_t)m, out.d_raw.p, d_inf.p);
+    uint8_t* d_slots = out.d_raw.p + (size_t)96 * m;
+    if (lay.n_slots())
+        MASP_LAUNCH(k_eval_combine, dim3((lay.n_slots() + 63) / 64), block, 0, s, d_colptr.p, d_rowidx.p, d_coef.p, X.p + m, d_slot_cols.p, lay.n_slots(),
+                    n_aux, EvalLayout::LONG_COL, minus_one, d_l.p, d_slots, d_inf.p);
+    if (!lay.long_slots.empty())
+        MASP_LAUNCH(k_eval_combine_long, dim3((uint32_t)lay.long_slots.size()), block, 0, s, d_colptr.p, d_rowidx.p, d_coef.p, X.p + m, d_slot_cols.p,
+                    d_long.p, n_aux, minus_one, d_l.p, d_slots, d_inf.p);
+    int any_inf = 1;
+    if (hipMemcpyAsync(&any_inf, d_inf.p, sizeof(int), hipMemcpyDeviceToHost, s) != hipSuccess || hipStreamSynchronize(s) != hipSuccess ||
+        launch_status() != MASP_HIP_OK) {
+        last_hip_error() = std::string("evaluation-form bases failed: ") + hipGetErrorString(hipGetLastError());
+        return MASP_HIP_E_HIP;
+    }
+    out.usable = any_inf == 0;
+    return MASP_HIP_OK;
+}
 
 extern "C" {
 
diff --git a/masp_amd/csrc/launch.h b/masp_amd/csrc/launch.h
--- a/masp_amd/csrc/launch.h
+++ b/masp_amd/csrc/launch.h
@@ -11,6 +11,7 @@
 void launch_ntt_copy_bitrev(hipStream_t s, const Fr* x, size_t x_stride, uint32_t nrows, Fr* y, uint32_t logm, uint32_t np);
 void launch_ntt_scale_bitrev(hipStream_t s, const Fr* x, const Fr* scale, Fr* y, uint32_t logm, uint32_t np);
 void launch_ntt_ab_bitrev(hipStream_t s, const Fr* a, const Fr* b, Fr* y, uint32_t logm, uint32_t np);
+void launch_ntt_ab_eval(hipStream_t s, const Fr* a, const Fr* b, const Fr& scale, Fr* y, uint32_t n, uint32_t np, size_t y_stride);
 void launch_fr_scale_sub(hipStream_t s, const Fr* x, const Fr* scale, const Fr* c, const Fr& cscale, Fr* y, uint32_t n, uint32_t np, size_t y_stride = 0);
 void launch_fr_scale(hipStream_t s, const Fr* x, const Fr* scale, Fr* y, uint32_t n, uint32_t np, size_t y_stride = 0);
 void launch_fr_from_mont(hipStream_t s, const Fr* x, Fr* y, uint32_t n);
@@ -25,8 +26,9 @@
     uint32_t n_long[3];
 };
 static constexpr uint32_t R1CS_LONG_ROW = 64;
-void launch_r1cs_eval(hipStream_t s, const R1csMatrices& M, const Fr* w, uint32_t n_vars, uint32_t n_constraints, uint32_t n_inputs, uint32_t np);
-void launch_gather_scalars(hipStream_t s, const Fr* src, size_t src_stride, const uint32_t* idx, uint32_t n, Fr* dst, uint32_t np);
+void launch_r1cs_eval(hipStream_t s, const R1csMatrices& M, const Fr* w, uint32_t n_vars, uint32_t n_constraints, uint32_t n_inputs, uint32_t np,
+                      uint32_t n_mat = 3);
+void launch_gather_scalars(hipStream_t s, const Fr* src, size_t src_stride, const uint32_t* idx, uint32_t n, Fr* dst, uint32_t np, size_t dst_stride = 0);
 
 void launch_groth16_fixed_g1(hipStream_t s, const G1Xyzz* fb1, const uint32_t* rs, size_t rs_stride, G1Xyzz* part, uint32_t np);
 void launch_groth16_fixed_g2(hipStream_t s, const G2Xyzz* fb2, const uint32_t* rs, size_t rs_stride, G2Xyzz* part2, uint32_t np);
diff --git a/masp_amd/csrc/prover.hip b/masp_amd/csrc/prover.hip
--- a/masp_amd/csrc/prover.hip
+++ b/masp_amd/csrc/prover.hip
@@ -147,6 +147,27 @@
     return MASP_HIP_OK;
 }
 
+static int enqueue_quotient_eval(Slot& sl, const NttDomain& D, const Fr* const in[2], size_t in_stride, uint32_t nrows, uint32_t np, Fr* e_out,
+                                 size_t e_stride) {
+    hipStream_t s = sl.stream;
+    const uint32_t m = (uint32_t)D.m, logm = D.logm;
+    const uint32_t sub_max = sl.ntt_sub;
+    const uint32_t sub = sub_max ? std::min(sub_max, np) : np;
+    int rc;
+    if ((rc = sl.x0.reserve((size_t)2 * m * sub)) || (rc = sl.x1.reserve((size_t)2 * m * sub))) return rc;
+    Fr *x0 = sl.x0.p, *x1 = sl.x1.p;
+    for (uint32_t p0 = 0; p0 < np; p0 += sub) {
+        const uint32_t q = std::min(sub, np - p0);
+        const size_t part = (size_t)q * m;
+        for (int i = 0; i < 2; ++i) launch_ntt_copy_bitrev(s, in[i] + (size_t)p0 * in_stride, in_stride, nrows, x0 + i * part, logm, q);
+        D.passes(s, x0, D.tw_inv.p, 2 * q);
+        launch_ntt_scale_bitrev(s, x0, D.coset_scale.p, x1, logm, 2 * q);
+        D.passes(s, x1, D.tw_fwd.p, 2 * q);
+        launch_ntt_ab_eval(s, x1, x1 + part, D.e_scale, e_out + (size_t)p0 * e_stride, m, q, e_stride);
+    }
+    return MASP_HIP_OK;
+}
+
 static int enqueue_proofs(Slot& sl, Circuit& C, uint32_t np, const Fr* d_w, size_t w_stride, const Fr* const d_abc[3], const uint32_t* d_rs,
                           uint8_t* d_proof, bool aux_montgomery = false) {
     hipStream_t s = sl.stream;
@@ -162,8 +183,9 @@
         for (int i = 0; i < Slot::N_AUX; ++i) HIP_TRY(hipStreamWaitEvent(sl.aux[i], sl.ev_fork, 0));
     }
     if (!aux_montgomery) launch_fr_to_mont(s, d_w, w_stride, sl.wm.p, nv, np, sl.flags.p);
-    const Fr* in[3];
+    const Fr* in[3] = {nullptr, nullptr, nullptr};
     bool mont_in;
+    const bool eval_form = !lone && !d_abc[0] && C.hl_eval.n != 0;
     if (d_abc[0]) {
         in[0] = d_abc[0];
         in[1] = d_abc[1];
@@ -171,7 +193,8 @@
         mont_in = false;
     } else {
         R1csMatrices M;
-        for (int i = 0; i < 3; ++i) {
+        const int n_mat = eval_form ? 2 : 3;
+        for (int i = 0; i < n_mat; ++i) {
             if ((rc = sl.ev[i].reserve((size_t)C.nrows * np))) return rc;
             M.rowptr[i] = C.rowptr[i].p;
             M.order[i] = C.row_order[i].p;
@@ -181,7 +204,13 @@
             M.out[i] = sl.ev[i].p;
             in[i] = sl.ev[i].p;
         }
-        launch_r1cs_eval(s, M, sl.wm.p, nv, C.n_constraints, C.n_inputs, np);
+        for (int i = n_mat; i < 3; ++i) {
+            M.rowptr[i] = M.order[i] = M.col[i] = nullptr;
+            M.coef[i] = nullptr;
+            M.out[i] = nullptr;
+            M.n_long[i] = 0;
+        }
+        launch_r1cs_eval(s, M, sl.wm.p, nv, C.n_constraints, C.n_inputs, np, (uint32_t)n_mat);
         mont_in = true;
     }
     if ((rc = sl.sa.reserve((size_t)C.na * np)) || (rc = sl.sb.reserve((size_t)C.nbq * np))) return rc;
@@ -248,14 +277,21 @@
         HIP_TRY(hipEventRecord(sl.ev_join[0], sl.aux[0]));
         HIP_TRY(hipStreamWaitEvent(s, sl.ev_join[0], 0));
     } else {
-        const size_t hl_stride = C.hl.n;
+        const BasesG1& HL = eval_form ? C.hl_eval : C.hl;
+        const size_t hl_stride = HL.n, aux_at = eval_form ? C.m : C.m - 1;
         if ((rc = sl.hl.reserve(hl_stride * np + 1))) return rc;
-        if ((rc = enqueue_quotient(sl, *C.dom, in, C.nrows, C.nrows, mont_in, np, sl.hl.p, hl_stride))) return rc;
-        HIP_TRY(hipMemcpy2DAsync(sl.hl.p + (C.m - 1), hl_stride * sizeof(Fr), d_w + C.n_inputs, w_stride * sizeof(Fr), (size_t)C.n_aux * sizeof(Fr), np,
-                                 hipMemcpyDeviceToDevice, s));
+        if (eval_form) {
+            if ((rc = enqueue_quotient_eval(sl, *C.dom, in, C.nrows, C.nrows, np, sl.hl.p, hl_stride))) return rc;
+            if (C.n_eval_in) launch_gather_scalars(s, d_w, w_stride, C.eval_in_var.p, C.n_eval_in, sl.hl.p + C.m + C.n_aux, np, hl_stride);
+        } else if ((rc = enqueue_quotient(sl, *C.dom, in, C.nrows, C.nrows, mont_in, np, sl.hl.p, hl_stride))) {
+            return rc;
+        }
+        if (C.n_aux)
+            HIP_TRY(hipMemcpy2DAsync(sl.hl.p + aux_at, hl_stride * sizeof(Fr), d_w + C.n_inputs, w_stride * sizeof(Fr), (size_t)C.n_aux * sizeof(Fr), np,
+                                     hipMemcpyDeviceToDevice, s));
         if (C.na) launch_gather_scalars(s, d_w, w_stride, C.a_var.p, C.na, sl.sa.p, np);
         if (C.nbq) launch_gather_scalars(s, d_w, w_stride, C.b_var.p, C.nbq, sl.sb.p, np);
-        if ((rc = msm_enqueue(s, C.hl, sl.ws1, (const uint32_t*)sl.hl.p, hl_stride * 8, sl.res1.p + 0, 4, np, prof))) return rc;
+        if ((rc = msm_enqueue(s, HL, sl.ws1, (const uint32_t*)sl.hl.p, hl_stride * 8, sl.res1.p + 0, 4, np, prof))) return rc;
         HIP_TRY(hipMemset2DAsync(sl.res1.p + 1, 4 * sizeof(G1Xyzz), 0, sizeof(G1Xyzz), np, s));
         const BasesG1 &Aq = C.a, &B1q = C.b1;
         const BasesG2& B2q = C.b2;
@@ -654,6 +690,22 @@
     return MASP_HIP_OK;
 }
 
+int masp_hip_ctx_set_quotient_form(masp_hip_ctx* ctx, int32_t form) {
+    if (!ctx || (form != MASP_HIP_QUOTIENT_EVALUATION && form != MASP_HIP_QUOTIENT_COEFFICIENT)) return MASP_HIP_E_INVALID_ARG;
+    auto set = [&](masp_hip_ctx* c) {
+        std::unique_lock<std::shared_mutex> lock(c->mu);
+        c->quotient_form = form;
+    };
+    set(ctx);
+    for (masp_hip_ctx* c : ctx->children) set(c);
+    return MASP_HIP_OK;
+}
+int masp_hip_ctx_get_quotient_form(const masp_hip_ctx* ctx, int32_t* out) {
+    if (!ctx || !out) return MASP_HIP_E_INVALID_ARG;
+    *out = (ctx->children.empty() ? ctx : ctx->children[0])->quotient_form;
+    return MASP_HIP_OK;
+}
+
 int masp_hip_ctx_create(int device, masp_hip_ctx** out) {
     if (!out) return MASP_HIP_E_INVALID_ARG;
     return masp_hip_ctx_create_ex(&device, 1, nullptr, out);
@@ -872,12 +924,12 @@
         const int c_lone = ctx->opt.window_bits_b2_lone;
         if (c_lone > 0 && L.n_b2 && (rc = C->b2_lone.load_host(L.b_g2, L.n_b2, s, eff(L.n_b2), c_lone))) return fail(ctx, rc);
     }
+    const int c_hl = c_h ? c_h : ctx->opt.window_bits_h_lone ? 0 : C->h.g.c;
     {
         const size_t nh = C->m - 1;
         std::vector<uint8_t> cat(96 * (nh + L.n_l));
         memcpy(cat.data(), L.h, 96 * nh);
         memcpy(cat.data() + 96 * nh, L.l, 96 * (size_t)L.n_l);
-        const int c_hl = c_h ? c_h : ctx->opt.window_bits_h_lone ? 0 : C->h.g.c;
         if ((rc = C->hl.load_host(cat.data(), (uint32_t)(nh + L.n_l), s, 0xffffffffu, c_hl, sub_bits, (uint32_t)nh))) return fail(ctx, rc);
     }
     int st = C->h.import_status | C->l.import_status | C->a.import_status | C->b1.import_status | C->b2.import_status;
@@ -898,6 +950,25 @@
         C->g1_endo = outside == 0;
     }
     if ((rc = get_domain(ctx, C->logm, &C->dom))) return fail(ctx, rc);
+    if (ctx->quotient_form == 0) {
+        masp::EvalBases E;
+        if ((rc = build_eval_bases(ctx, *C->dom, L.h, L.l, cs, E))) return fail(ctx, rc);
+        if (E.usable) {
+            const masp::EvalLayout& lay = E.lay;
+            if ((rc = C->hl_eval.load_device(E.d_raw.p, (uint32_t)lay.n(), s, 0xffffffffu, c_hl, sub_bits, (uint32_t)lay.aux_off(), (uint32_t)lay.in_off())))
+                return fail(ctx, rc);
+            if ((rc = C->eval_in_var.upload(lay.used_inputs.data(), lay.used_inputs.size(), s))) return fail(ctx, rc);
+            if (hipStreamSynchronize(s) != hipSuccess) return fail(ctx, MASP_HIP_E_HIP);
+            C->eval_inputs = lay.used_inputs;
+            C->n_eval_in = (uint32_t)lay.used_inputs.size();
+            if (C->hl_eval.import_status) {
+                C->hl_eval.release();
+                C->hl_eval.n = 0;
+                C->eval_inputs.clear();
+                C->n_eval_in = 0;
+            }
+        }
+    }
     ctx->circ[slot] = std::move(C);
     return MASP_HIP_OK;
 }
@@ -908,6 +979,35 @@
     std::shared_lock<std::shared_mutex> lock(const_cast<masp_hip_ctx*>(ctx)->mu);
     if (slot >= MASP_HIP_MAX_CIRCUITS || !ctx->circ[slot]) return MASP_HIP_E_NOT_LOADED;
     *flags = ctx->circ[slot]->g1_endo ? MASP_HIP_CIRCUIT_G1_ENDOMORPHISM : 0u;
+    return MASP_HIP_OK;
+}
+
+int masp_hip_circuit_quotient_form(const masp_hip_ctx* ctx, uint32_t slot, int32_t* form) {
+    if (!ctx || !form) return MASP_HIP_E_INVALID_ARG;
+    if (!ctx->children.empty()) return masp_hip_circuit_quotient_form(ctx->children[0], slot, form);
+    std::shared_lock<std::shared_mutex> lock(const_cast<masp_hip_ctx*>(ctx)->mu);
+    if (slot >= MASP_HIP_MAX_CIRCUITS || !ctx->circ[slot]) return MASP_HIP_E_NOT_LOADED;
+    *form = ctx->circ[slot]->hl_eval.n ? MASP_HIP_QUOTIENT_EVALUATION : MASP_HIP_QUOTIENT_COEFFICIENT;
+    return MASP_HIP_OK;
+}
+int masp_hip_circuit_eval_bases(const masp_hip_ctx* ctx, uint32_t slot, uint8_t* bases, size_t cap_points, size_t* n_points, uint32_t* input_cols,
+                                size_t cap_inputs, size_t* n_input_cols) {
+    if (!ctx || !n_points || !n_input_cols) return MASP_HIP_E_INVALID_ARG;
+    if (!ctx->children.empty()) return masp_hip_circuit_eval_bases(ctx->children[0], slot, bases, cap_points, n_points, input_cols, cap_inputs, n_input_cols);
+    std::shared_lock<std::shared_mutex> lock(const_cast<masp_hip_ctx*>(ctx)->mu);
+    if (slot >= MASP_HIP_MAX_CIRCUITS || !ctx->circ[slot]) return MASP_HIP_E_NOT_LOADED;
+    const Circuit& C = *ctx->circ[slot];
+    *n_points = C.hl_eval.n;
+    *n_input_cols = C.eval_inputs.size();
+    if (!bases && !input_cols) return MASP_HIP_OK;
+    if (!bases || !input_cols || cap_points < *n_points || cap_inputs < *n_input_cols) return MASP_HIP_E_CAPACITY;
+    if (C.hl_eval.n) {
+        std::vector<masp::TabRow<masp::FpOps>> rows(C.hl_eval.n);
+        hipSetDevice(ctx->device);
+        if (hipMemcpy(rows.data(), C.hl_eval.tab, sizeof(rows[0]) * rows.size(), hipMemcpyDeviceToHost) != hipSuccess) return MASP_HIP_E_HIP;
+        for (size_t i = 0; i < rows.size(); ++i) masp::g1_write_uncompressed(rows[i].p, bases + 96 * i);
+    }
+    memcpy(input_cols, C.eval_inputs.data(), 4 * C.eval_inputs.size());
     return MASP_HIP_OK;
 }
 
diff --git a/masp_amd/hip.py b/masp_amd/hip.py
--- a/masp_amd/hip.py
+++ b/masp_amd/hip.py
@@ -46,6 +46,7 @@
 
 assert C.sizeof(JobStruct) == 120 and JobStruct.r.offset == 48 and JobStruct.aux_form.offset == 112
 AUX_CANONICAL, AUX_MONTGOMERY = 0, 1
+QUOTIENT_EVALUATION, QUOTIENT_COEFFICIENT = 0, 1
 
 
 def library_path():
@@ -108,6 +109,11 @@
         L.masp_hip_msm_g2_multi_ex.argtypes = [vp, vp, sz, vp, sz, C.c_int, C.c_int, sz, sz, vp, vp]
         L.masp_hip_ctx_set_boolean_block_bits.argtypes = [vp, C.c_int32]
         L.masp_hip_ctx_get_boolean_block_bits.argtypes = [vp, C.POINTER(C.c_int32)]
+    if hasattr(L, "masp_hip_ctx_set_quotient_form"):
+        L.masp_hip_ctx_set_quotient_form.argtypes = [vp, C.c_int32]
+        L.masp_hip_ctx_get_quotient_form.argtypes = [vp, C.POINTER(C.c_int32)]
+        L.masp_hip_circuit_quotient_form.argtypes = [vp, u32, C.POINTER(C.c_int32)]
+        L.masp_hip_circuit_eval_bases.argtypes = [vp, u32, vp, sz, C.POINTER(sz), vp, sz, C.POINTER(sz)]
     L.masp_hip_quotient_h.argtypes = [vp, vp, vp, vp, sz, u32, vp]
     L.masp_hip_ntt.argtypes = [vp, vp, u32, C.c_int]
     L.masp_hip_vk_prepare.argtypes = [vp, vp, sz, C.POINTER(vp)]
@@ -507,6 +513,29 @@
         self._check(self._L.masp_hip_ctx_get_boolean_block_bits(self._h, C.byref(v)))
         return int(v.value)
 
+    def set_quotient_form(self, form):
+        self._check(self._L.masp_hip_ctx_set_quotient_form(self._h, int(form)))
+
+    @property
+    def quotient_form(self):
+        v = C.c_int32(0)
+        self._check(self._L.masp_hip_ctx_get_quotient_form(self._h, C.byref(v)))
+        return int(v.value)
+
+    def circuit_quotient_form(self, slot):
+        v = C.c_int32(0)
+        self._check(self._L.masp_hip_circuit_quotient_form(self._h, int(slot), C.byref(v)))
+        return int(v.value)
+
+    def circuit_eval_bases(self, slot):
+        n, k = C.c_size_t(0), C.c_size_t(0)
+        self._check(self._L.masp_hip_circuit_eval_bases(self._h, int(slot), None, 0, C.byref(n), None, 0, C.byref(k)))
+        pts = np.zeros((n.value, 96), dtype=np.uint8)
+        cols = np.zeros(max(k.value, 1), dtype=np.uint32)
+        if n.value:
+            self._check(self._L.masp_hip_circuit_eval_bases(self._h, int(slot), _p(pts), n.value, C.byref(n), _p(cols), cols.size, C.byref(k)))
+        return pts, [int(c) for c in cols[:k.value]]
+
     def current_options(self):
         got = OptionsStruct()
         got.struct_size = C.sizeof(OptionsStruct)
```

New measurement: 1459 proofs/s (median of 6 runs). 1.04x the previous value.
